# AgRoboticsResearch/headland_trajectory_planning

Measured on NVIDIA B200. Metric: warm_start_plans_per_sec, higher is better.
Workload: dtype f64

## Files before the change

headland_trajectory_planning_b200/_lib.py:

```python
import ctypes as C
import os
import threading

import numpy as np

HERE = os.path.dirname(os.path.abspath(__file__))
_LIB_NAME = "libheadland_b200.so"

ABI_VERSION = 4
HL_MAX_PRIMS = 16
HL_CAPSULE_VERTS = 66
HL_RS_CANDIDATES = 46
HL_RS_MAX_SEGS = 5

CHECK_OBSTACLES = 1
CHECK_BOUNDARY = 2
CHECK_AUX = 4
CHECK_LANE = 8

STATUS_NAMES = {0: "ok", 1: "start_goal_blocked", 2: "open_empty", 3: "max_nodes",
                4: "capacity", 5: "rs_assert"}


class HeadlandError(RuntimeError):
    pass


class HlEnvHost(C.Structure):
    _fields_ = [
        ("n_obs", C.c_int32), ("obs_xy", C.POINTER(C.c_double)),
        ("n_field", C.c_int32), ("field_xy", C.POINTER(C.c_double)),
        ("n_seg", C.c_int32), ("seg_xy", C.POINTER(C.c_double)),
        ("seg_poly", C.POINTER(C.c_double)), ("seg_len", C.POINTER(C.c_double)),
        ("n_crit", C.c_int32), ("crit_xy", C.POINTER(C.c_double)),
        ("n_guide", C.c_int32), ("guide", C.POINTER(C.c_double)),
        ("default_search_length", C.c_double),
        ("body_ext", C.c_double * 4),
        ("n_aux", C.c_int32), ("aux_ext", C.POINTER(C.c_double)),
    ]


class HlSearchParams(C.Structure):
    _fields_ = [
        ("plan_resolution", C.c_double), ("yaw_resolution", C.c_double),
        ("maxc", C.c_double), ("max_steer", C.c_double), ("wheel_base", C.c_double),
        ("n_prims", C.c_int32),
        ("prim_steer", C.c_double * HL_MAX_PRIMS), ("prim_dir", C.c_double * HL_MAX_PRIMS),
        ("prim_yaw_step", C.c_double * HL_MAX_PRIMS), ("prim_curv", C.c_double * HL_MAX_PRIMS),
        ("prim_steer_eff", C.c_double * HL_MAX_PRIMS),
        ("steps_default", C.c_int32), ("steps_large", C.c_int32),
        ("steer_cost", C.c_double), ("delta_steer_cost", C.c_double),
        ("direction_change_cost", C.c_double), ("reverse_cost", C.c_double),
        ("hybrid_cost", C.c_double), ("min_length_to_goal", C.c_double),
        ("max_nodes", C.c_int32), ("max_path_poses", C.c_int32),
        ("motion_type", C.c_int32), ("dubins_capacity", C.c_int32),
    ]


class HlGridField(C.Structure):
    _fields_ = [
        ("occ_offset", C.c_int64), ("out_offset", C.c_int64),
        ("w", C.c_int32), ("h", C.c_int32), ("gi", C.c_int32), ("gj", C.c_int32),
    ]


SCENARIO_DTYPE = np.dtype([("env_id", "<i4"), ("reserved", "<i4"),
                           ("start", "<f8", (3,)), ("goal", "<f8", (3,))])
RESULT_DTYPE = np.dtype([("status", "<i4"), ("counter", "<i4"), ("n_expanded", "<i4"),
                         ("arrival", "<i4"), ("path_len", "<i4"), ("rs_word", "<i4"),
                         ("path_offset", "<i8"), ("goal_cost", "<f8"),
                         ("n_pose_checks", "<i8"), ("n_exact", "<i8"), ("keys_offset", "<i8"),
                         ("cycles", "<i8"), ("n_pose_checks_ref", "<i8")])
RSWORD_DTYPE = np.dtype([("cand", "<i4"), ("n_seg", "<i4"), ("npts", "<i4"), ("collide", "<i4"),
                         ("L", "<f8"), ("cost", "<f8"), ("len", "<f8", (HL_RS_MAX_SEGS,)),
                         ("nlen", "<f8", (HL_RS_MAX_SEGS,))])
assert SCENARIO_DTYPE.itemsize == 56 and RESULT_DTYPE.itemsize == 80 and RSWORD_DTYPE.itemsize == 112

EXPORTS = [
    "hl_last_error", "hl_abi_version", "hl_ctx_create", "hl_ctx_destroy", "hl_ctx_sm_count", "hl_ctx_device",
    "hl_ctx_set_astar_variant", "hl_env_upload", "hl_env_free", "hl_env_count", "hl_env_device", "hl_collision_check", "hl_path_reduce",
    "hl_rs_all_paths", "hl_rs_sample", "hl_hybrid_astar_batch", "hl_hybrid_astar_workspace_bytes", "hl_astar_phase_cycles",
    "hl_distance_field", "hl_distance_field_batch", "hl_grid_pack", "hl_grid_footprint_check", "hl_measure_fp32_peak", "hl_ypark_paths", "hl_arc_paths", "hl_ref_path_count", "hl_ref_path_fill",
    "hl_dubins_count", "hl_dubins_knots", "hl_dubins_fill", "hl_min_boundary_distance", "hl_corridor_hits",
]



class _Missing:
    def __init__(self, name):
        self._name = name
        self.argtypes = None
        self.restype = None

    def __call__(self, *a, **k):
        raise HeadlandError(f"libheadland_b200.so does not export {self._name}: rebuild the library")


class _Tolerant:

    def __init__(self, cdll):
        self._cdll = cdll
        self._missing = {}

    def __getattr__(self, name):
        try:
            return getattr(self._cdll, name)
        except AttributeError:
            return self._missing.setdefault(name, _Missing(name))


_lib = None
_lock = threading.RLock()
_ctxs = {}


def library_path():
    return os.path.join(HERE, _LIB_NAME)


def load_library():
    global _lib
    with _lock:
        if _lib is not None:
            return _lib
        path = library_path()
        if not os.path.exists(path):
            raise HeadlandError(
                f"{path} is missing: build it with `python -c 'import __graft_entry__ as g; g.build()'` "
                "(there is no CPU fallback)")
        lib = _Tolerant(C.CDLL(path))
        vp, i32, i64, u32, dbl = C.c_void_p, C.c_int32, C.c_int64, C.c_uint32, C.c_double
        lib.hl_last_error.restype = C.c_char_p
        lib.hl_abi_version.restype = C.c_int
        lib.hl_ctx_create.argtypes = [C.POINTER(vp), C.c_int]
        lib.hl_ctx_destroy.argtypes = [vp]
        lib.hl_ctx_destroy.restype = None
        lib.hl_ctx_sm_count.argtypes = [vp]
        lib.hl_ctx_device.argtypes = [vp]
        lib.hl_ctx_set_astar_variant.argtypes = [vp, C.c_int]
        lib.hl_env_device.argtypes = [vp]
        lib.hl_env_upload.argtypes = [vp, C.POINTER(HlEnvHost), i32, C.POINTER(vp)]
        lib.hl_env_free.argtypes = [vp]
        lib.hl_env_free.restype = None
        lib.hl_env_count.argtypes = [vp]
        lib.hl_env_count.restype = i32
        lib.hl_collision_check.argtypes = [vp, vp, vp, vp, vp, i64, u32, vp, vp, vp]
        lib.hl_path_reduce.argtypes = [vp, vp, vp, i64, vp, vp]
        lib.hl_rs_all_paths.argtypes = [vp, vp, vp, vp, i64, dbl, dbl, dbl, u32, vp, vp, vp, vp]
        lib.hl_rs_sample.argtypes = [vp, vp, vp, i64, dbl, dbl, vp, vp, vp, vp, vp, vp, vp]
        lib.hl_hybrid_astar_batch.argtypes = [vp, vp, vp, i32, C.POINTER(HlSearchParams), vp, vp, i64, vp,
                                              vp, vp, vp, vp, vp, i64, vp, vp]
        lib.hl_hybrid_astar_workspace_bytes.argtypes = [vp, C.POINTER(HlSearchParams)]
        lib.hl_hybrid_astar_workspace_bytes.restype = i64
        lib.hl_astar_phase_cycles.argtypes = [vp, C.POINTER(C.c_uint64), i32, i32]
        lib.hl_distance_field.argtypes = [vp, vp, i32, i32, i32, i32, i32, vp, C.POINTER(i32), vp]
        lib.hl_distance_field_batch.argtypes = [vp, vp, i64, C.POINTER(HlGridField), i32, i32, vp, i64, C.POINTER(i32), vp]
        lib.hl_grid_pack.argtypes = [vp, vp, i32, i32, vp, vp]
        lib.hl_grid_footprint_check.argtypes = [vp, vp, i32, i32, dbl, vp, i64, C.POINTER(dbl), vp, vp]
        lib.hl_measure_fp32_peak.argtypes = [vp, C.POINTER(dbl)]
        lib.hl_ypark_paths.argtypes = [vp, vp, vp, i64, dbl, vp, vp]
        lib.hl_arc_paths.argtypes = [vp, vp, vp, i64, dbl, vp, vp]
        lib.hl_ref_path_count.argtypes = [vp, vp, vp, vp, vp, i64, dbl, vp, vp, vp]
        lib.hl_ref_path_fill.argtypes = [vp, vp, vp, vp, vp, vp, vp, i64, dbl, dbl, dbl, vp, vp, vp]
        lib.hl_dubins_count.argtypes = [vp, vp, i64, dbl, dbl, dbl, i32, vp, vp, vp, vp]
        lib.hl_dubins_knots.argtypes = [vp, vp, i64, dbl, dbl, dbl, i32, vp, vp, vp, vp, vp, vp]
        lib.hl_min_boundary_distance.argtypes = [vp, vp, vp, vp, vp, i64, i32, vp, vp]
        lib.hl_corridor_hits.argtypes = [vp, vp, vp, vp, vp, i64, dbl, vp, vp]
        lib.hl_dubins_fill.argtypes = [vp, i64, dbl, vp, vp, vp, vp, vp, vp]
        if lib.hl_abi_version() != ABI_VERSION:
            raise HeadlandError("libheadland_b200.so ABI version mismatch")
        _lib = lib
        return lib


def last_error():
    return load_library().hl_last_error().decode("utf-8", "replace")


def check(rc, what):
    if rc != 0:
        raise HeadlandError(f"{what}: {last_error()}")


def have_gpu():
    try:
        import torch
        return torch.cuda.is_available()
    except Exception:
        return False


def get_ctx(device=None):
    import torch
    lib = load_library()
    if not torch.cuda.is_available():
        raise HeadlandError("no CUDA device: headland_trajectory_planning_b200 has no CPU fallback")
    if device is None:
        device = torch.cuda.current_device()
    device = int(device)
    with _lock:
        if device in _ctxs:
            return _ctxs[device]
        h = C.c_void_p()
        rc = lib.hl_ctx_create(C.byref(h), device)
        msg = lib.hl_last_error().decode("utf-8", "replace") if rc != 0 else ""
        if rc == 0:
            _ctxs[device] = h
    if rc != 0:
        raise HeadlandError(f"hl_ctx_create: {msg}")
    return h


ASTAR_VARIANTS = {"spec": 0, "warp": 1, "level": 2}


def apply_astar_variant(ctx):
    v = os.environ.get("HL_ASTAR_VARIANT", "spec")
    check(load_library().hl_ctx_set_astar_variant(ctx, ASTAR_VARIANTS.get(v, 0)), "hl_ctx_set_astar_variant")


def ptr(t):
    if t is None:
        return None
    assert t.is_cuda and t.is_contiguous()
    return C.c_void_p(t.data_ptr())


def stream_ptr():
# ... 7 lines not shown
```

headland_trajectory_planning_b200/csrc/hl_astar.cu:

```cuda
#include <cstdlib>
#include <cstdio>
#include <mutex>
#include "hl_astar_common.cuh"

#ifndef AW_WARPS
#define AW_WARPS 12
#endif
#ifndef AW_MIN_CTAS
#define AW_MIN_CTAS 1
#endif
#ifndef AW_LOCKSTEP
#define AW_LOCKSTEP 1
#endif
#ifndef AW_MAX_PLANS
#define AW_MAX_PLANS 6
#endif

struct AwSmem {
    double start[3], goal[3];
    long long start_key, goal_key;
    int env, scen, state;
    int n_nodes, heap_n, counter, n_closed;
    int status, arrival, rs_word;
    double goal_cost;
// ... 6 lines not shown
            unsigned char rs_valid[HL_RS_CANDIDATES + 2], rs_accept[HL_RS_CANDIDATES + 2];
            RsPlan plans[AW_MAX_PLANS];
            RsPlan plan_tmp;
        };
        struct {
            double tx[HL_MAX_PRIMS][AS_ROLL], ty[HL_MAX_PRIMS][AS_ROLL], pyaw[HL_MAX_PRIMS][AS_ROLL];
            unsigned char pamb[HL_MAX_PRIMS][AS_ROLL];
            double pg[HL_MAX_PRIMS], pprio[HL_MAX_PRIMS];
            long long pkey[HL_MAX_PRIMS];
            int pkey_ok[HL_MAX_PRIMS], pslot[HL_MAX_PRIMS], ppos[HL_MAX_PRIMS], pneed[HL_MAX_PRIMS];
        };
    };
    RsProblem rs_prob;
    int rs_n, rs_pick;
    int dub_rows;
    int phit[HL_MAX_PRIMS];
    unsigned long long n_checks, n_exact, n_ref;
    long long t_last, t_phase[AS_N_PHASES];
    __align__(16) float envf[AS_ENV_FLOATS];
};

static_assert(sizeof(AwSmem) * AW_WARPS <= 227 * 1024, "per-CTA shared memory exceeds 227 KB");
#define TICK(ph) do { if (lane == 0) { long long _n = clock64(); S.t_phase[ph] += _n - S.t_last; S.t_last = _n; } } while (0)

__device__ __forceinline__ void finalize_scenario(AwSmem& S, const AsWs& W, const AsParams& P, const AsOut& O, int lane) {
    const RsPlan* plan = P.pawn ? nullptr : (S.rs_pick >= 0 && S.rs_pick < AW_MAX_PLANS ? &S.plans[S.rs_pick] : &S.plan_tmp);
    const AsWritten w = write_outputs(W, P, O, S.status, S.n_closed, S.cur, S.arrival, S.start_key, S.goal_key, plan,
                                      S.dub_rows, lane);
    if (lane == 0) {
        S.t_phase[PH_OUTPUT] += clock64() - S.t_last;
        long long tot = 0;
        for (int k = 0; k < AS_N_PHASES; ++k) tot += S.t_phase[k];
        write_record(O, S.scen, w, S.arrival, S.rs_word, S.goal_cost, S.counter, S.n_checks, S.n_exact, S.n_ref, tot);
        for (int k = 0; k < AS_N_PHASES; ++k) atomicAdd(O.phase_cycles + k, (unsigned long long)S.t_phase[k]);
    }
    for (int i = lane; i < S.n_nodes; i += 32) W.hkey[W.nhpos[i]] = KEY_EMPTY;
    __syncwarp();
}

__device__ __noinline__ void setup_scenario(AwSmem& S, const AsWs& W, const AsParams& P, const EnvBatchDev& eb,
                                            const EnvDesc& D, const EnvSmem& E, unsigned FLAGS, int lane) {
    const AsStart st = start_node(W, P, eb, D, E, S.start, S.goal, FLAGS, lane);
    if (lane == 0) {
        S.start_key = st.start_key; S.goal_key = st.goal_key; S.status = st.status;
        if (st.status < 0) { S.n_nodes = 1; heap_set(W, S.heap_n, 0, st.prio); }
    }
    __syncwarp();
}

__device__ __noinline__ void pawn_shot(AwSmem& S, const AsWs& W, const AsParams& P, const EnvBatchDev& eb, const EnvDesc& D,
                                       const EnvSmem& E, unsigned FLAGS, int lane) {
    const int cap = P.dub_cap;
    double* ts = W.dub; double* kx = ts + cap; double* ky = kx + cap; double* ks = ky + cap; double* dx = ks + cap;
    double* dy = dx + cap; double* cp = dy + cap; double* bx = cp + cap; double* by = bx + cap;
    double* rx = by + cap; double* ry = rx + cap; double* ryaw = ry + cap; double* rk = ryaw + cap;
    const double q0[3] = {S.cx, S.cy, S.cyaw};
    DubPath path;
    dub_shortest(q0, S.goal, xdiv(1.0, P.maxc), path);
    if (path.type < 0) { if (lane == 0) S.status = HL_STATUS_RS_ASSERT; __syncwarp(); return; }
    const long long n_s = dub_n_samples(dub_length(path), P.res);
    if (n_s + 1 > cap) { if (lane == 0) S.status = HL_STATUS_CAPACITY; __syncwarp(); return; }
    const int m = dub_course_knots(path, P.res, true, S.goal, n_s, ts, kx, ky, ks, lane);
    if (m < 2) { if (lane == 0) S.status = HL_STATUS_RS_ASSERT; __syncwarp(); return; }
    if (lane == 0) rp_derivs(ks, kx, ky, m, dx, dy, cp, bx, by);
    __syncwarp();
    const long long cnt = rp_count(ks[m - 1], P.res);
    if (cnt > cap) { if (lane == 0) S.status = HL_STATUS_CAPACITY; __syncwarp(); return; }
    for (long long i = lane; i < cnt; i += 32) {
        const double t = xmul((double)i, P.res);
        double x, x1, x2, y, y1, y2;
        rp_eval(ks, kx, dx, m, t, x, x1, x2);
        rp_eval(ks, ky, dy, m, t, y, y1, y2);
        const double q = x1 * x1 + y1 * y1;
        rx[i] = x; ry[i] = y; ryaw[i] = angle_wrap(m_atan2(y1, x1));
        rk[i] = (y2 * x1 - x2 * y1) / (q * sqrt(q));
    }
    __syncwarp();
    if (lane == 0) S.n_ref += (unsigned long long)cnt;
    int infeasible = 0;
    for (long long base = 0; base < cnt && !infeasible; base += 32) {
        const long long i = base + lane;
        int st = HL_FREE;
        unsigned amb = 0;
        if (i < cnt) st = pose_filter(D, E, rx[i], ry[i], ryaw[i], FLAGS, &amb);
        const unsigned livem = __ballot_sync(FULL, i < cnt);
        const unsigned hitm = __ballot_sync(FULL, st == HL_HIT);
        const unsigned ambm = __ballot_sync(FULL, st == HL_AMBIG);
        infeasible = hitm != 0;
        if (!infeasible && ambm) {
            int bad = 0;
            if (st == HL_AMBIG) bad = pose_exact(eb, D, rx[i], ry[i], ryaw[i], amb) ? 1 : 0;
            if (lane == 0) S.n_exact += (unsigned long long)__popc(ambm);
            infeasible = __any_sync(FULL, bad);
        }
        if (lane == 0) S.n_checks += (unsigned long long)__popc(livem);
    }
    if (!infeasible && lane == 0) {
        double len = 0.0, kmin = rk[0], kmax = rk[0];
        for (long long i = 0; i + 1 < cnt; ++i) {
            const double dsl = hypot_cr(xsub(rx[i + 1], rx[i]), xsub(ry[i + 1], ry[i]));
            len = (i == 0) ? dsl : xadd(len, dsl);
        }
        for (long long i = 1; i < cnt; ++i) { kmin = fmin(kmin, rk[i]); kmax = fmax(kmax, rk[i]); }
        if (len < P.min_len_goal) {
            S.arrival = 1; S.rs_word = path.type; S.dub_rows = (int)cnt;
            S.goal_cost = xadd(xadd(S.cg, len), xmul(angle_wrap(xsub(kmax, kmin)), P.steer_cost));
        }
    }
    __syncwarp();
}

__global__ void __launch_bounds__(AW_WARPS * 32, AW_MIN_CTAS)
k_hybrid_astar_w(EnvBatchDev eb, const HlScenario* __restrict__ scen, int n_scen, AsParams P, char* ws_base,
                 size_t ws_stride, unsigned int* work_counter, AsOut O) {
    extern __shared__ __align__(16) unsigned char smem_raw[];
    const int lane = threadIdx.x & 31, wid = threadIdx.x >> 5;
    AwSmem& S = reinterpret_cast<AwSmem*>(smem_raw)[wid];
    const AsWs W = as_carve(ws_base + ((size_t)blockIdx.x * AW_WARPS + wid) * ws_stride, P.cap_nodes, P.hash_size,
                            P.max_nodes, P.dub_cap);
    const int hmask = P.hash_size - 1;
    const unsigned FLAGS = HL_CHECK_OBSTACLES | HL_CHECK_BOUNDARY | HL_CHECK_LANE;

    for (int i = lane; i < P.hash_size; i += 32) W.hkey[i] = KEY_EMPTY;
    if (lane == 0) S.state = ST_IDLE;
    __syncwarp();

    EnvSmem E;
    E.n_obs = E.n_field = E.n_seg = E.all_rect = 0; E.eps = 0.f; E.reach = 0.f; E.obs = E.field = E.seg = nullptr;
    const EnvDesc* Dp = eb.desc;
    int iter = 0;
    (void)iter;

    while (true) {
        while (S.state == ST_IDLE) {
            int sc = 0;
            if (lane == 0) sc = (int)atomicAdd(work_counter, 1u);
            sc = __shfl_sync(FULL, sc, 0);
            if (sc >= n_scen) { if (lane == 0) S.state = ST_DONE; __syncwarp(); break; }
            if (lane == 0) {
                const HlScenario s = scen[sc];
                S.scen = sc; S.env = s.env_id;
                for (int k = 0; k < 3; ++k) { S.start[k] = s.start[k]; S.goal[k] = s.goal[k]; }
                S.n_nodes = 0; S.heap_n = 0; S.counter = 0; S.n_closed = 0;
                S.status = -1; S.arrival = 0; S.rs_word = -1; S.goal_cost = 0.0; S.rs_pick = -1;
                S.n_checks = 0; S.n_exact = 0; S.n_ref = 0;
                for (int k = 0; k < AS_N_PHASES; ++k) S.t_phase[k] = 0;
                S.t_last = clock64();
            }
            __syncwarp();
            Dp = eb.desc + S.env;
            stage_env_warp(eb, *Dp, S.envf, AS_ENV_FLOATS, E, lane);
            setup_scenario(S, W, P, eb, *Dp, E, FLAGS, lane);
            TICK(PH_SETUP);
            if (S.status >= 0) finalize_scenario(S, W, P, O, lane);
            else if (lane == 0) S.state = ST_SEARCH;
            __syncwarp();
        }
#if AW_LOCKSTEP == 3
        {
            if ((iter++ & 1) == 0) { if (__syncthreads_and(S.state == ST_DONE)) break; }
            else if (S.state == ST_DONE) {  }
        }
#elif AW_LOCKSTEP
        if (__syncthreads_and(S.state == ST_DONE)) break;
#else
        if (S.state == ST_DONE) break;
#endif
// ... 20 lines not shown
            __syncwarp();
            TICK(PH_POP);
        }
        if (live && S.status < 0 && P.pawn) {
            pawn_shot(S, W, P, eb, D, E, FLAGS, lane);
            TICK(PH_RS_SAMPLE);
        }
        if (live && S.status < 0 && !P.pawn) {
            const double q0[3] = {S.cx, S.cy, S.cyaw};
            for (int c = lane; c < HL_RS_CANDIDATES; c += 32) {
                double l[HL_RS_MAX_SEGS] = {0, 0, 0, 0, 0};
                bool ok = rs_candidate(c, S.rs_prob, l);
                S.rs_valid[c] = ok ? 1 : 0;
                for (int k = 0; k < HL_RS_MAX_SEGS; ++k) S.rs_lens[c][k] = l[k];
            }
            __syncwarp();
            TICK(PH_RS_CAND);
            if (lane < RS_N_GROUPS) rs_select_group(lane, S.rs_valid, S.rs_lens, S.rs_accept, S.rs_Lc);
            __syncwarp();
            {
                const int a0 = S.rs_accept[lane];
                const int a1 = (lane + 32 < HL_RS_CANDIDATES) ? S.rs_accept[lane + 32] : 0;
                const unsigned b0 = __ballot_sync(FULL, a0 == 1), b1 = __ballot_sync(FULL, a1 == 1);
                const unsigned bad = __ballot_sync(FULL, a0 == 2 || a1 == 2);
                const unsigned lt = (1u << lane) - 1u;
                const int n0 = __popc(b0);
                if (a0 == 1) { int k = __popc(b0 & lt); S.rs_acc[k] = lane; S.rs_L[k] = S.rs_Lc[lane]; }
                if (a1 == 1) { int k = n0 + __popc(b1 & lt); S.rs_acc[k] = lane + 32; S.rs_L[k] = S.rs_Lc[lane + 32]; }
                const int m = bad ? 0 : n0 + __popc(b1);
                __syncwarp();
                for (int k = lane; k < m; k += 32)
                    S.rs_prio[k] = rs_path_cost(S.cg, S.rs_acc[k], S.rs_lens[S.rs_acc[k]], P.max_steer,
                                                P.reverse_cost, P.dir_change_cost, P.steer_cost);
                __syncwarp();
                if (lane == 0) {
                    if (bad) S.status = HL_STATUS_RS_ASSERT;
                    S.rs_n = m;
                    if (m > 0) heapdict_order(S.rs_prio, m, S.rs_order);
                }
            }
            __syncwarp();
            TICK(PH_RS_SELECT);
        }
        if (live && S.status < 0) {
            const double q0[3] = {S.cx, S.cy, S.cyaw};
            const int m = P.pawn ? 0 : S.rs_n;
            const double stepn = xmul(P.res, P.maxc);
            const double cq = m_cos(-q0[2]), sq = m_sin(-q0[2]);
            if (lane < m && lane < AW_MAX_PLANS) {
                int c = S.rs_acc[S.rs_order[lane]];
                rs_make_plan(c, S.rs_lens[c], P.maxc, stepn, S.plans[lane]);
                rs_plan_world32(S.plans[lane], q0, cq, sq, D.origin);
            }
            __syncwarp();
            TICK(PH_RS_PLAN);
            EnvSmem Ers = E;
            Ers.eps = E.eps + 6e-5f;
            const float inv_maxc = (float)(1.0 / P.maxc);
            for (int r = 0; r < m; ++r) {
                const int k = S.rs_order[r];
                const int c = S.rs_acc[k];
                if (r >= AW_MAX_PLANS) {
                    __syncwarp();
                    if (lane == 0) {
                        rs_make_plan(c, S.rs_lens[c], P.maxc, stepn, S.plan_tmp);
                        rs_plan_world32(S.plan_tmp, q0, cq, sq, D.origin);
                    }
                    __syncwarp();
                }
                const RsPlan& plan = (r < AW_MAX_PLANS) ? S.plans[r] : S.plan_tmp;
                const int npts = plan.npts;
                if (lane == 0) S.n_ref += (unsigned long long)npts;
                int infeasible = 0;
                const int passes = (npts + 31) >> 5;
                for (int pass = 0; pass < passes && !infeasible; ++pass) {
                    const int j = lane * passes + pass;
                    int st = HL_FREE;
                    unsigned amb = 0;
                    if (j < npts) {
                        float fx, fy, fc, fs;
                        rs_sample_world32(plan, j, inv_maxc, fx, fy, fc, fs);
                        if (fabsf(fx) > Ers.reach || fabsf(fy) > Ers.reach) st = far_status(FLAGS, Ers.n_seg);
                        else if (!(fx == fx) || !(fy == fy) || !(fc == fc)) { st = HL_AMBIG; amb = FLAGS; }
                        else st = filter_part(Ers, fx, fy, fc, fs, Ers.ext, FLAGS, &amb);
                    }
                    const unsigned livem = __ballot_sync(FULL, j < npts);
                    const unsigned hitm = __ballot_sync(FULL, st == HL_HIT);
                    const unsigned ambm = __ballot_sync(FULL, st == HL_AMBIG);
                    infeasible = hitm != 0;
                    if (!infeasible && ambm) {
                        int bad = 0;
                        if (st == HL_AMBIG) {
                            double lx, ly, lyaw, wx, wy, wyaw;
                            int cs, dir;
                            rs_sample_local(plan, j, P.maxc, lx, ly, lyaw, cs, dir);
                            rs_to_world(q0, cq, sq, lx, ly, lyaw, wx, wy, wyaw);
                            bad = pose_exact(eb, D, wx, wy, wyaw, amb) ? 1 : 0;
                        }
                        if (lane == 0) S.n_exact += (unsigned long long)__popc(ambm);
                        infeasible = __any_sync(FULL, bad);
                    }
                    if (lane == 0) S.n_checks += (unsigned long long)__popc(livem);
                }
                const bool short_enough = xdiv(S.rs_L[k], P.maxc) < P.min_len_goal;
                if (!infeasible && short_enough) {
                    if (lane == 0) { S.rs_pick = r; S.arrival = 1; S.rs_word = c; S.goal_cost = S.rs_prio[k]; }
                    break;
                }
            }
            __syncwarp();
            TICK(PH_RS_SAMPLE);
            if (lane == 0) {
                double xd = fabs(xsub(S.cx, S.goal[0])), yd = fabs(xsub(S.cy, S.goal[1]));
                double wd = fabs(angle_wrap(xsub(S.cyaw, S.goal[2])));
                if (xd < P.res && yd < P.res && wd < P.yaw_res) { S.arrival = 2; S.goal_cost = S.cg; S.rs_word = -1; }
                if (S.arrival) S.status = HL_STATUS_OK;
                else {
                    int seg = exact_search_segment(eb, D, S.cx, S.cy);
                    double len = seg < 0 ? D.default_len : eb.seg_len[D.seg_off + seg];
                    S.nsteps = (int)rint(xdiv(len, P.res));
                    if (S.nsteps + 1 > HL_MAX_ROLLOUT || S.nsteps < 1) S.status = HL_STATUS_CAPACITY;
                }
            }
            if (lane < HL_MAX_PRIMS) S.phit[lane] = 0;
            __syncwarp();
            TICK(PH_ARRIVE);
        }
#if AW_LOCKSTEP == 1
        __syncthreads();
#endif
        if (live && S.status < 0) {
            const int n = S.nsteps, np1 = n + 1;
            const int total = P.n_prims * np1;
            for (int idx = lane; idx < total; idx += 32) {
                const int p = idx / np1, i = idx - p * np1;
                const double ys = P.yaw_step[p];
                const double init_yaw = angle_wrap(xadd(S.cyaw, ys));
                const double stop = xadd(init_yaw, xmul(ys, (double)(n + 1)));
                const double delta = xsub(stop, init_yaw);
                const double step = xdiv(delta, (double)(n + 1));
                const double yw = rollout_yaw(init_yaw, stop, step, delta, n + 1, i);
                S.tx[p][i] = xmul(xmul(P.res, m_cos(yw)), P.dir[p]);
                S.ty[p][i] = xmul(xmul(P.res, m_sin(yw)), P.dir[p]);
                S.pyaw[p][i] = rollout_yaw(init_yaw, stop, step, delta, n + 1, i + 1);
            }
            __syncwarp();
            if (lane < P.n_prims) {
                double ax = 0.0, ay = 0.0;
                for (int i = 0; i < np1; ++i) {
                    ax = (i == 0) ? S.tx[lane][0] : xadd(ax, S.tx[lane][i]);
                    ay = (i == 0) ? S.ty[lane][0] : xadd(ay, S.ty[lane][i]);
                    S.tx[lane][i] = xadd(S.cx, ax);
                    S.ty[lane][i] = xadd(S.cy, ay);
                }
            }
            __syncwarp();
            TICK(PH_ROLLOUT);
            for (int idx = lane; idx < total; idx += 32) {
                const int p = idx / np1, j = idx - p * np1;
                unsigned amb = 0;
                int st = pose_filter(D, E, S.tx[p][j], S.ty[p][j], S.pyaw[p][j], FLAGS, &amb);
                S.pamb[p][j] = (st == HL_AMBIG) ? (unsigned char)amb : 0;
                if (st == HL_HIT) atomicOr(&S.phit[p], 1);
            }
            if (lane == 0) { S.n_checks += (unsigned long long)total; S.n_ref += (unsigned long long)total; }
            __syncwarp();
            TICK(PH_FILTER);
            for (int idx = lane; idx < total; idx += 32) {
                const int p = idx / np1, j = idx - p * np1;
                if (S.pamb[p][j] && !S.phit[p]) {
                    atomicAdd(&S.n_exact, 1ULL);
                    if (pose_exact(eb, D, S.tx[p][j], S.ty[p][j], S.pyaw[p][j], S.pamb[p][j])) atomicOr(&S.phit[p], 2);
                }
            }
            __syncwarp();
            TICK(PH_EXACT);
            if (lane < HL_MAX_PRIMS) S.pneed[lane] = 1;
            __syncwarp();
            if (lane < P.n_prims && !S.phit[lane]) {
                const int p = lane;
                double len = 0.0;
                for (int i = 0; i + 1 < np1; ++i) {
                    double ds = hypot_cr(xsub(S.tx[p][i + 1], S.tx[p][i]), xsub(S.ty[p][i + 1], S.ty[p][i]));
                    len = (i == 0) ? ds : xadd(len, ds);
                }
                double cost = xadd(S.cg, len);
                if (P.dir[p] == -1.0) cost = xadd(cost, P.reverse_cost);
                cost = xadd(cost, xmul(P.steer[p], P.steer_cost));
                const double parent_steer = S.cprim < 0 ? 0.0 : P.steer_eff[S.cprim];
                cost = xadd(cost, xmul(fabs(xsub(P.steer[p], parent_steer)), P.delta_steer_cost));
                const double parent_dir = S.cprim < 0 ? 1.0 : P.dir[S.cprim];
                if (parent_dir != P.dir[p]) cost = xadd(cost, P.dir_change_cost);
                S.pg[p] = cost;
                int ix, iy, iw;
                long long key = 0;
                S.pkey_ok[p] = make_key(S.tx[p][n], S.ty[p][n], S.pyaw[p][n], P.res, P.yaw_res, ix, iy, iw, key) ? 1 : 0;
                S.pkey[p] = key;
                int pos = -1;
                const int slot = S.pkey_ok[p] ? hash_find(W, hmask, key, &pos) : -1;
                S.pslot[p] = slot;
                S.ppos[p] = pos;
                if (slot >= 0 && (W.nstate[slot] == 1 || !(cost < W.ng[slot]))) S.pneed[p] = 0;
            }
            __syncwarp();
            for (int p = 0; p < P.n_prims; ++p) {
                if (!S.phit[p] && S.pneed[p]) {
                    double h = warp_state_cost(eb, D, S.tx[p][n], S.ty[p][n], S.pyaw[p][n], lane);
                    if (lane == 0) S.pprio[p] = xmul(P.hybrid_cost, h);
                }
            }
            __syncwarp();
            TICK(PH_COST_HEUR);
            if (lane == 0) {
                for (int p = 0; p < P.n_prims; ++p) {
                    if (S.phit[p]) continue;
                    if (!S.pkey_ok[p]) { S.status = HL_STATUS_CAPACITY; break; }
                    int pos = S.ppos[p];
                    int slot = S.pslot[p];
                    if (slot < 0 ? (W.hkey[pos] != KEY_EMPTY) : false) slot = hash_find(W, hmask, S.pkey[p], &pos);
                    const double g = S.pg[p];
                    const double prio = (S.pprio[p] > g) ? S.pprio[p] : g;
                    if (slot >= 0) {
                        if (W.nstate[slot] == 1) continue;
                        if (!(g < W.ng[slot])) continue;
                        if (!S.pneed[p]) { S.status = HL_STATUS_CAPACITY; break; }
                    } else {
                        if (S.n_nodes >= P.cap_nodes) { S.status = HL_STATUS_CAPACITY; break; }
                        slot = S.n_nodes++;
                        W.hkey[pos] = S.pkey[p]; W.hval[pos] = slot; W.nhpos[slot] = pos;
                        W.nkey[slot] = S.pkey[p]; W.nstate[slot] = 0; W.nheap[slot] = -1;
                    }
                    W.nx[slot] = S.tx[p][n]; W.ny[slot] = S.ty[p][n]; W.nyaw[slot] = S.pyaw[p][n];
                    W.ng[slot] = g; W.nparent[slot] = S.cur; W.nprim[slot] = (signed char)p;
                    W.nsteps[slot] = (signed char)n;
                    heap_set(W, S.heap_n, slot, prio);
                }
            }
            __syncwarp();
            TICK(PH_MERGE);
        }
        if (live && S.status >= 0) {
            finalize_scenario(S, W, P, O, lane);
            if (lane == 0) S.state = ST_IDLE;
            __syncwarp();
// ... 313 lines not shown
```

headland_trajectory_planning_b200/csrc/hl_astar_common.cuh:

```cuda
#define HL_SHARED_CODE 1
#pragma once
#include <cstring>
#include "hl_geom.cuh"
#include "hl_rs.cuh"
#include "hl_dubins.cuh"

#define AS_ROLL (HL_MAX_ROLLOUT + 1)
#define AS_ENV_FLOATS 512
#define KEY_EMPTY (-1LL)
#define FULL 0xffffffffu
enum { ST_IDLE = 0, ST_SEARCH = 1, ST_DONE = 2 };
enum { PH_POP = 0, PH_RS_CAND, PH_RS_SELECT, PH_RS_PLAN, PH_RS_SAMPLE, PH_ARRIVE, PH_ROLLOUT, PH_FILTER, PH_EXACT,
       PH_COST_HEUR, PH_MERGE, PH_SETUP, PH_OUTPUT, AS_N_PHASES };

struct AsParams {
    double res, yaw_res, maxc, max_steer, wheel_base;
    int n_prims;
    double steer[HL_MAX_PRIMS], dir[HL_MAX_PRIMS], yaw_step[HL_MAX_PRIMS], curv[HL_MAX_PRIMS], steer_eff[HL_MAX_PRIMS];
    double steer_cost, delta_steer_cost, dir_change_cost, reverse_cost, hybrid_cost, min_len_goal;
    int max_nodes, max_path_poses;
    int cap_nodes, hash_size;
    int pawn;
    int dub_cap;
};
// ... 75 lines not shown
}

__device__ __forceinline__ unsigned hash_key(long long k) {
    unsigned long long z = (unsigned long long)k * 0x9E3779B97F4A7C15ULL;
    return (unsigned)(z >> 40);
}

__device__ __noinline__ int hash_find(const AsWs& w, int hmask, long long key, int* pos) {
    unsigned h = hash_key(key) & hmask;
    while (true) {
        long long k = w.hkey[h];
        if (k == key) { *pos = (int)h; return w.hval[h]; }
        if (k == KEY_EMPTY) { *pos = (int)h; return -1; }
        h = (h + 1) & hmask;
    }
}

template <int HS> struct HeapRef {
    const AsWs& w; double* sp; int* ss;
    __device__ __forceinline__ double prio(int i) const { return (HS > 0 && i < HS) ? sp[i] : w.hprio[i]; }
    __device__ __forceinline__ int slot(int i) const { return (HS > 0 && i < HS) ? ss[i] : w.hslot[i]; }
    __device__ __forceinline__ void put(int i, double p, int s) const {
        if (HS > 0 && i < HS) { sp[i] = p; ss[i] = s; } else { w.hprio[i] = p; w.hslot[i] = s; }
        w.nheap[s] = i;
    }
};

template <int HS> __device__ __forceinline__ void heap_up_t(const HeapRef<HS>& H, int i, double prio, int slot, bool always) {
    while (i) {
        const int parent = (i - 1) >> 1;
        const double pp = H.prio(parent);
        if (!always && pp < prio) break;
        H.put(i, pp, H.slot(parent));
        i = parent;
    }
    H.put(i, prio, slot);
}

template <int HS> __device__ __forceinline__ int heap_popitem_t(const HeapRef<HS>& H, int& n) {
    const int top = H.slot(0);
    --n;
    if (n > 0) {
        const double prio = H.prio(n);
        const int slot = H.slot(n);
        int i = 0;
        while (true) {
            const int l = (i << 1) + 1, r = l + 1;
            int low = i;
            double lowp = prio;
            if (l < n) {
                const double pl = H.prio(l);
                const double pr = (r < n) ? H.prio(r) : 0.0;
                if (pl < lowp) { low = l; lowp = pl; }
                if (r < n && pr < lowp) { low = r; lowp = pr; }
            }
            if (low == i) break;
            H.put(i, lowp, H.slot(low));
            i = low;
        }
        H.put(i, prio, slot);
    }
    H.w.nheap[top] = -1;
    return top;
}

template <int HS> __device__ __forceinline__ void heap_set_t(const HeapRef<HS>& H, int& n, int slot, double prio) {
    const int at = H.w.nheap[slot];
    if (at >= 0) {
        heap_up_t<HS>(H, at, 0.0, slot, true);
        heap_popitem_t<HS>(H, n);
    }
    heap_up_t<HS>(H, n++, prio, slot, false);
}

__device__ __noinline__ int heap_popitem(const AsWs& w, int& n) {
    const HeapRef<0> H{w, nullptr, nullptr};
    return heap_popitem_t<0>(H, n);
}
__device__ __noinline__ void heap_set(const AsWs& w, int& n, int slot, double prio) {
    const HeapRef<0> H{w, nullptr, nullptr};
    heap_set_t<0>(H, n, slot, prio);
}

__device__ HL_CODE int pose_filter(const EnvDesc& D, const EnvSmem& E, double x, double y, double yaw,
                                           unsigned flags, unsigned* amb) {
    float px = (float)(x - D.origin[0]), py = (float)(y - D.origin[1]);
    if (fabsf(px) > E.reach || fabsf(py) > E.reach) return far_status(flags, E.n_seg);
    if (!(fabs(yaw) < 1e6) || !(px == px) || !(py == py)) { *amb = flags; return HL_AMBIG; }
    float sf, cf;
    sincosf((float)yaw, &sf, &cf);
    return filter_part(E, px, py, cf, sf, E.ext, flags, amb);
}

__device__ __noinline__ bool pose_exact(const EnvBatchDev& eb, const EnvDesc& D, double x, double y, double yaw,
                                           unsigned amb) {
    Pose64 p;
    p.x = x; p.y = y; p.c = m_cos(yaw); p.s = m_sin(yaw);
    return exact_part_check(p, D.body_ext, eb, D, amb);
}

__device__ __noinline__ void stage_env_warp(const EnvBatchDev& eb, const EnvDesc& D, float* sm, int cap_floats,
                                            EnvSmem& E, int lane) {
    const int n_o = D.n_obs * HL_OBS32_STRIDE, n_f = D.n_field * HL_FIELD32_STRIDE, n_s = D.n_seg * 4;
    E.n_obs = D.n_obs; E.n_field = D.n_field; E.n_seg = D.n_seg; E.all_rect = D.all_rect;
    E.eps = D.eps; E.reach = D.reach;
    for (int k = 0; k < 4; ++k) E.ext[k] = (float)D.body_ext[k];
    const float* g_obs = eb.obs32 + (size_t)HL_OBS32_STRIDE * D.obs_off;
    const float* g_field = eb.field32 + HL_FIELD32_STRIDE * (size_t)D.field_off;
    const float* g_seg = eb.seg32 + 4 * (size_t)D.seg_off;
    if (n_o + n_f + n_s <= cap_floats) {
        float* s_obs = sm;
        float* s_field = s_obs + n_o;
        float* s_seg = s_field + n_f;
        for (int i = lane; i < n_o; i += 32) s_obs[i] = g_obs[i];
        for (int i = lane; i < n_f; i += 32) s_field[i] = g_field[i];
        for (int i = lane; i < n_s; i += 32) s_seg[i] = g_seg[i];
        E.obs = s_obs; E.field = s_field; E.seg = s_seg;
    } else {
        E.obs = g_obs; E.field = g_field; E.seg = g_seg;
    }
    __syncwarp();
}

__device__ __noinline__ double warp_state_cost(const EnvBatchDev& eb, const EnvDesc& D, double x, double y, double yaw, int lane) {
    const double* gx = eb.guide_x + D.guide_off;
    const double* gy = eb.guide_y + D.guide_off;
    const int n = D.n_guide;
    if (n <= 0) return 0.0;
    double best = INFINITY;
#pragma unroll 1
    for (int i = lane; i < n; i += 32) {
        double dx = gx[i] - x, dy = gy[i] - y;
        best = fmin(best, dx * dx + dy * dy);
    }
    for (int o = 16; o; o >>= 1) best = fmin(best, __shfl_xor_sync(0xffffffffu, best, o));
    const double thr = best * (1.0 + 1e-9) + 1e-300;
    double bh = INFINITY;
    int bi = 0x7fffffff;
#pragma unroll 1
    for (int i = lane; i < n; i += 32) {
        double dx = xsub(gx[i], x), dy = xsub(gy[i], y);
        if (dx * dx + dy * dy <= thr) {
            double h = hypot_cr(dx, dy);
            if (h < bh || (h == bh && i < bi)) { bh = h; bi = i; }
        }
    }
    for (int o = 16; o; o >>= 1) {
        double oh = __shfl_xor_sync(0xffffffffu, bh, o);
        int oi = __shfl_xor_sync(0xffffffffu, bi, o);
        if (oh < bh || (oh == bh && oi < bi)) { bh = oh; bi = oi; }
    }
    double dist = xmul(bh, 100.0);
    double yaw_diff = fabs(angle_wrap(xsub(eb.guide_yaw[D.guide_off + bi], yaw)));
    if (dist > 2.0) dist = 100.0;
    double to_goal = xsub(eb.guide_s[D.guide_off + n - 1], eb.guide_s[D.guide_off + bi]);
    return xadd(xadd(dist, xmul(yaw_diff, 0.2)), xmul(to_goal, 5.0));
}

__device__ HL_TINY double rollout_yaw(double init_yaw, double stop, double step, double delta, int div, int i) {
    double v;
    if (i == div) v = stop;
    else if (step != 0.0) v = xadd(xmul((double)i, step), init_yaw);
    else v = xadd(xmul(xdiv((double)i, (double)div), delta), init_yaw);
    return angle_wrap(v);
}



struct AsStart { int status; long long start_key, goal_key; double prio; };

__device__ __forceinline__ AsStart start_node(const AsWs& W, const AsParams& P, const EnvBatchDev& eb, const EnvDesc& D,
                                           const EnvSmem& E, const double* start, const double* goal, unsigned flags,
                                           int lane) {
    int bad = 0;
    if (lane < 2) {
        const double* q = lane == 0 ? start : goal;
        unsigned amb = flags;
        int r = pose_filter(D, E, q[0], q[1], q[2], flags, &amb);
        bad = (r == HL_HIT) || (r == HL_AMBIG && pose_exact(eb, D, q[0], q[1], q[2], amb));
    }
    bad = __any_sync(FULL, bad);
    const double h = warp_state_cost(eb, D, start[0], start[1], start[2], lane);
    AsStart s;
    s.status = -1; s.start_key = 0; s.goal_key = 0; s.prio = 0.0;
    if (lane == 0) {
        int ix, iy, iw;
        bool ok = make_key(start[0], start[1], start[2], P.res, P.yaw_res, ix, iy, iw, s.start_key);
        ok = make_key(goal[0], goal[1], goal[2], P.res, P.yaw_res, ix, iy, iw, s.goal_key) && ok;
        if (!ok) s.status = HL_STATUS_CAPACITY;
        else if (bad) s.status = HL_STATUS_START_GOAL_BLOCKED;
        else {
            W.nx[0] = start[0]; W.ny[0] = start[1]; W.nyaw[0] = start[2]; W.ng[0] = 0.0;
            W.nkey[0] = s.start_key; W.nparent[0] = 0; W.nprim[0] = -1; W.nsteps[0] = 0; W.nstate[0] = 0;
            W.nheap[0] = -1;
            int pos;
            hash_find(W, P.hash_size - 1, s.start_key, &pos);
            W.hkey[pos] = s.start_key; W.hval[pos] = 0; W.nhpos[0] = pos;
            s.prio = xmul(P.hybrid_cost, h);
            s.prio = (s.prio > 0.0) ? s.prio : 0.0;
        }
    }
    return s;
}

struct AsWritten { int status, n_keys; long long keys_off; int path_len; long long path_off; };

__device__ __noinline__ AsWritten write_outputs(const AsWs& W, const AsParams& P, const AsOut& O, int status, int n_closed,
                                                int end, int arrival, long long start_key, long long goal_key,
                                                const RsPlan* plan, int dub_rows, int lane) {
    AsWritten w;
    long long koff = 0;
    if (lane == 0 && n_closed > 0) {
        koff = (long long)atomicAdd(O.keys_cursor, (unsigned long long)n_closed);
        if (koff + n_closed > O.keys_capacity) koff = -1;
    }
    koff = __shfl_sync(FULL, koff, 0);
    w.n_keys = n_closed;
    if (koff < 0) { status = HL_STATUS_CAPACITY; w.n_keys = 0; koff = 0; }
    w.keys_off = koff;
    int32_t* ek = O.expanded_keys + (size_t)koff * 3;
    for (int i = lane; i < w.n_keys; i += 32) {
        int ix, iy, iw;
        unpack_key(W.nkey[W.corder[i]], ix, iy, iw);
        ek[3 * i] = ix; ek[3 * i + 1] = iy; ek[3 * i + 2] = iw;
    }
    const int ext_rows = arrival != 1 ? 0 : (plan ? plan->npts : dub_rows);
    int len = 0, path_len = 0;
    long long path_off = 0;
    if (lane == 0 && status == HL_STATUS_OK) {
        int poses = 0;
        bool ok = true;
        if (goal_key != start_key) {
            for (int node = end; node != 0; node = W.nparent[node]) {
                if (len >= P.cap_nodes) { ok = false; break; }
                W.hslot[len++] = node;
                poses += W.nsteps[node] + 1;
            }
            poses += ext_rows;
        }
        path_len = poses;
        if (!ok || path_len > P.max_path_poses) { status = HL_STATUS_CAPACITY; path_len = 0; }
        else if (path_len > 0) {
            unsigned long long off = atomicAdd(O.path_cursor, (unsigned long long)path_len);
            if ((long long)(off + path_len) > O.path_capacity) { status = HL_STATUS_CAPACITY; path_len = 0; }
            path_off = (long long)off;
        }
    }
    __syncwarp();
    w.status = __shfl_sync(FULL, status, 0);
    w.path_len = __shfl_sync(FULL, path_len, 0);
    w.path_off = __shfl_sync(FULL, path_off, 0);
    len = __shfl_sync(FULL, len, 0);
    if (w.status == HL_STATUS_OK && w.path_len > 0) {
        for (int c = lane; c < len; c += 32) {
            const int node = W.hslot[len - 1 - c];
            long long off = w.path_off;
            for (int q = 0; q < c; ++q) off += W.nsteps[W.hslot[len - 1 - q]] + 1;
            const int par = W.nparent[node];
            const int p = W.nprim[node], n = W.nsteps[node];
            const double ys = P.yaw_step[p];
            const double init_yaw = angle_wrap(xadd(W.nyaw[par], ys));
// ... 64 lines not shown
```

headland_trajectory_planning_b200/csrc/hl_astar_level.cuh:

```cuda
#pragma once
#include "hl_astar_common.cuh"

#define LS_ROLL_STRIDE (AS_ROLL + 1)
#define LS_MAX_BATCH 8192
#define LS_CHUNK 32
#define LS_GRID_MULT 4
#define LS_THREADS 256

struct LsScn {
    double start[3], goal[3];
    long long start_key, goal_key;
    int env, status, arrival, has_cur;
    int n_nodes, heap_n, counter, n_closed;
    int cur, cprim, nsteps, rs_n;
    double cx, cy, cyaw, cg;
    double goal_cost;
    int rs_pick, rs_word, rs_bad, pad0;
    RsProblem rs_prob;
    unsigned long long checks, exact, ref;
};

struct LsPrim {
    double dtx[AS_ROLL], dty[AS_ROLL];
    double tx[AS_ROLL], ty[AS_ROLL], pyaw[AS_ROLL];
// ... 202 lines not shown
    const int n_act = C.n_act[parity];
    const int* act = C.act[parity];
    for (int a = warp; a < n_act; a += n_warps) {
        const int sc = act[a];
        LsScn& S = C.scn[sc];
        LsShot& T = C.shot[sc];
        if (lane < RS_N_GROUPS) rs_select_group(lane, T.rs_valid, T.rs_lens, T.rs_accept, T.rs_Lc);
        __syncwarp();
        const int a0 = T.rs_accept[lane];
        const int a1 = (lane + 32 < HL_RS_CANDIDATES) ? T.rs_accept[lane + 32] : 0;
        const unsigned b0 = __ballot_sync(FULL, a0 == 1), b1 = __ballot_sync(FULL, a1 == 1);
        const unsigned bad = __ballot_sync(FULL, a0 == 2 || a1 == 2);
        const unsigned lt = (1u << lane) - 1u;
        const int n0 = __popc(b0);
        if (a0 == 1) { int k = __popc(b0 & lt); T.rs_acc[k] = lane; T.rs_L[k] = T.rs_Lc[lane]; }
        if (a1 == 1) { int k = n0 + __popc(b1 & lt); T.rs_acc[k] = lane + 32; T.rs_L[k] = T.rs_Lc[lane + 32]; }
        const int m = bad ? 0 : n0 + __popc(b1);
        __syncwarp();
        const double sg = S.cg;
        for (int k = lane; k < m; k += 32)
            T.rs_prio[k] = rs_path_cost(sg, T.rs_acc[k], T.rs_lens[T.rs_acc[k]], P.max_steer, P.reverse_cost,
                                        P.dir_change_cost, P.steer_cost);
        __syncwarp();
        int base = 0;
        if (lane == 0) {
            S.rs_n = m; S.rs_bad = bad ? 1 : 0;
            if (m > 0) {
                double prio[HL_RS_CANDIDATES];
                int order[HL_RS_CANDIDATES];
                for (int k = 0; k < m; ++k) prio[k] = T.rs_prio[k];
                heapdict_order(prio, m, order);
                for (int k = 0; k < m; ++k) T.rs_order[k] = order[k];
                base = atomicAdd(C.n_words, m);
            }
        }
        base = __shfl_sync(FULL, base, 0);
        for (int r = lane; r < m; r += 32) { C.words[base + r] = make_int2(sc, r); T.word_bad[r] = 1; }
        __syncwarp();
    }
}

__global__ void __launch_bounds__(LS_THREADS) ls_sample(const LsCall* __restrict__ Cp) {
    __shared__ RsPlan s_plan[LS_THREADS / 32];
    const LsCall& C = *Cp;
    const int lane = threadIdx.x & 31, wib = threadIdx.x >> 5;
    const int warp = (blockIdx.x * blockDim.x + threadIdx.x) >> 5, n_warps = (gridDim.x * blockDim.x) >> 5;
    const AsParams& P = C.P;
    const int n_words = *C.n_words;
    const float inv_maxc = (float)(1.0 / P.maxc);
    const double stepn = xmul(P.res, P.maxc);
    RsPlan& plan = s_plan[wib];
    for (int w = warp; w < n_words; w += n_warps) {
        const int2 item = C.words[w];
        const int sc = item.x, r = item.y;
        LsScn& S = C.scn[sc];
        LsShot& T = C.shot[sc];
        const EnvDesc& D = C.eb.desc[S.env];
        EnvSmem E;
        global_env(C.eb, D, E);
        E.eps += 6e-5f;
        const int k = T.rs_order[r];
        const int c = T.rs_acc[k];
        const double q0[3] = {S.cx, S.cy, S.cyaw};
        const double cq = m_cos(-q0[2]), sq = m_sin(-q0[2]);
        __syncwarp();
        if (lane == 0) {
            rs_make_plan(c, T.rs_lens[c], P.maxc, stepn, plan);
            rs_plan_world32(plan, q0, cq, sq, D.origin);
        }
        __syncwarp();
        const int npts = plan.npts;
        int infeasible = 0;
        const int passes = (npts + 31) >> 5;
        unsigned long long checks = 0, exact = 0;
        for (int pass = 0; pass < passes && !infeasible; ++pass) {
            const int j = lane * passes + pass;
            int st2 = HL_FREE;
            unsigned amb = 0;
            if (j < npts) {
                float fx, fy, fc, fs;
                rs_sample_world32(plan, j, inv_maxc, fx, fy, fc, fs);
                if (fabsf(fx) > E.reach || fabsf(fy) > E.reach) st2 = far_status(LS_FLAGS, E.n_seg);
                else if (!(fx == fx) || !(fy == fy) || !(fc == fc)) { st2 = HL_AMBIG; amb = LS_FLAGS; }
                else st2 = filter_part(E, fx, fy, fc, fs, E.ext, LS_FLAGS, &amb);
            }
            const unsigned livem = __ballot_sync(FULL, j < npts);
            const unsigned hitm = __ballot_sync(FULL, st2 == HL_HIT);
            const unsigned ambm = __ballot_sync(FULL, st2 == HL_AMBIG);
            infeasible = hitm != 0;
            if (!infeasible && ambm) {
                int bad2 = 0;
                if (st2 == HL_AMBIG) {
                    double lx, ly, lyaw, wx, wy, wyaw;
                    int cs, dir;
                    rs_sample_local(plan, j, P.maxc, lx, ly, lyaw, cs, dir);
                    rs_to_world(q0, cq, sq, lx, ly, lyaw, wx, wy, wyaw);
                    bad2 = pose_exact(C.eb, D, wx, wy, wyaw, amb) ? 1 : 0;
                }
                exact += (unsigned long long)__popc(ambm);
                infeasible = __any_sync(FULL, bad2);
            }
            checks += (unsigned long long)__popc(livem);
        }
        if (lane == 0) {
            T.word_npts[r] = npts;
            T.word_bad[r] = infeasible ? 1 : 0;
            atomicAdd(&S.checks, checks);
            if (exact) atomicAdd(&S.exact, exact);
        }
        __syncwarp();
    }
}

__global__ void __launch_bounds__(LS_THREADS) ls_rollout(const LsCall* __restrict__ Cp, int parity) {
    const LsCall& C = *Cp;
    const AsParams& P = C.P;
    const int per_scn = P.n_prims * LS_ROLL_STRIDE;
    const int n_items = C.n_act[parity] * per_scn;
    const int* act = C.act[parity];
    if (blockIdx.x == 0 && threadIdx.x == 0) C.n_act[parity ^ 1] = 0;
    for (int it = blockIdx.x * blockDim.x + threadIdx.x; it < n_items; it += gridDim.x * blockDim.x) {
        const int a = it / per_scn, rem = it - a * per_scn;
        const int p = rem / LS_ROLL_STRIDE, i = rem - p * LS_ROLL_STRIDE;
        const int sc = act[a];
        const LsScn& S = C.scn[sc];
        const int n = S.nsteps, np1 = n + 1;
        if (i > np1) continue;
        LsPrim& R = C.prim[(size_t)sc * P.n_prims + p];
        const double ys = P.yaw_step[p];
        const double init_yaw = angle_wrap(xadd(S.cyaw, ys));
        const double stop = xadd(init_yaw, xmul(ys, (double)(n + 1)));
        const double delta = xsub(stop, init_yaw);
        const double step = xdiv(delta, (double)(n + 1));
        const double yw = rollout_yaw(init_yaw, stop, step, delta, n + 1, i);
        if (i >= 1) R.pyaw[i - 1] = yw;
        if (i <= n) {
            double sn, cs;
            m_sincos(yw, &sn, &cs);
            R.dtx[i] = xmul(xmul(P.res, cs), P.dir[p]);
            R.dty[i] = xmul(xmul(P.res, sn), P.dir[p]);
        }
        if (i == 0) { R.phit = 0; R.pneed = 1; }
    }
}

__global__ void __launch_bounds__(LS_THREADS) ls_filter(const LsCall* __restrict__ Cp, int parity) {
    const LsCall& C = *Cp;
    const AsParams& P = C.P;
    const int per_scn = P.n_prims * AS_ROLL;
    const int n_items = C.n_act[parity] * per_scn;
    const int* act = C.act[parity];
    for (int it = blockIdx.x * blockDim.x + threadIdx.x; it < n_items; it += gridDim.x * blockDim.x) {
        const int a = it / per_scn, rem = it - a * per_scn;
        const int p = rem / AS_ROLL, j = rem - p * AS_ROLL;
        const int sc = act[a];
        LsScn& S = C.scn[sc];
        const int np1 = S.nsteps + 1;
        if (j >= np1) continue;
        LsPrim& R = C.prim[(size_t)sc * P.n_prims + p];
        double ax = R.dtx[0], ay = R.dty[0];
        for (int i = 1; i <= j; ++i) { ax = xadd(ax, R.dtx[i]); ay = xadd(ay, R.dty[i]); }
        const double x = xadd(S.cx, ax), y = xadd(S.cy, ay);
        R.tx[j] = x; R.ty[j] = y;
        const EnvDesc& D = C.eb.desc[S.env];
        EnvSmem E;
        global_env(C.eb, D, E);
        unsigned amb = 0;
        const int st = pose_filter(D, E, x, y, R.pyaw[j], LS_FLAGS, &amb);
        R.pamb[j] = (st == HL_AMBIG) ? (unsigned char)amb : 0;
        if (st == HL_HIT) atomicOr(&R.phit, 1);
        if (j == 0 && p == 0) atomicAdd(&S.checks, (unsigned long long)(P.n_prims * np1));
    }
}

__global__ void __launch_bounds__(LS_THREADS) ls_cost(const LsCall* __restrict__ Cp, int parity) {
    const LsCall& C = *Cp;
    const int lane = threadIdx.x & 31;
    const int warp = (blockIdx.x * blockDim.x + threadIdx.x) >> 5, n_warps = (gridDim.x * blockDim.x) >> 5;
    const AsParams& P = C.P;
    const int hmask = P.hash_size - 1;
    const int n_items = C.n_act[parity] * P.n_prims;
    const int* act = C.act[parity];
    for (int it = warp; it < n_items; it += n_warps) {
        const int a = it / P.n_prims, p = it - a * P.n_prims;
        const int sc = act[a];
        LsScn& S = C.scn[sc];
        LsPrim& R = C.prim[(size_t)sc * P.n_prims + p];
        const EnvDesc& D = C.eb.desc[S.env];
        const int n = S.nsteps, np1 = n + 1;
        int hit = R.phit;
        if (!hit) {
            int bad = 0;
            const int am = lane < np1 ? R.pamb[lane] : 0;
            if (am) bad = pose_exact(C.eb, D, R.tx[lane], R.ty[lane], R.pyaw[lane], am) ? 1 : 0;
            const unsigned ambm = __ballot_sync(FULL, am != 0);
            if (ambm && lane == 0) atomicAdd(&S.exact, (unsigned long long)__popc(ambm));
            if (__any_sync(FULL, bad)) hit = 2;
        }
        if (hit) { if (lane == 0) R.phit = hit; __syncwarp(); continue; }
        double ds = 0.0;
        if (lane < n) ds = hypot_cr(xsub(R.tx[lane + 1], R.tx[lane]), xsub(R.ty[lane + 1], R.ty[lane]));
        double len = __shfl_sync(FULL, ds, 0);
        for (int i = 1; i < n; ++i) len = xadd(len, __shfl_sync(FULL, ds, i));
        if (n < 1) len = 0.0;
        int need = 1, key_ok = 0;
        if (lane == 0) {
            const AsWs W = ls_ws(C, sc);
            double cost = xadd(S.cg, len);
            if (P.dir[p] == -1.0) cost = xadd(cost, P.reverse_cost);
            cost = xadd(cost, xmul(P.steer[p], P.steer_cost));
            const int cprim = S.cprim;
            const double parent_steer = cprim < 0 ? 0.0 : P.steer_eff[cprim];
            cost = xadd(cost, xmul(fabs(xsub(P.steer[p], parent_steer)), P.delta_steer_cost));
            const double parent_dir = cprim < 0 ? 1.0 : P.dir[cprim];
            if (parent_dir != P.dir[p]) cost = xadd(cost, P.dir_change_cost);
            R.pg = cost;
            int ix, iy, iw;
            long long key = 0;
            key_ok = make_key(R.tx[n], R.ty[n], R.pyaw[n], P.res, P.yaw_res, ix, iy, iw, key) ? 1 : 0;
            R.pkey_ok = key_ok;
            R.pkey = key;
            int pos = -1;
            const int slot2 = key_ok ? hash_find(W, hmask, key, &pos) : -1;
            R.pslot = slot2;
            R.ppos = pos;
            if (slot2 >= 0 && (W.nstate[slot2] == 1 || !(cost < W.ng[slot2]))) need = 0;
            R.pneed = need;
            R.phit = 0;
        }
        need = __shfl_sync(FULL, need, 0);
        key_ok = __shfl_sync(FULL, key_ok, 0);
        if (need && key_ok) {
            const double h = warp_state_cost(C.eb, D, R.tx[n], R.ty[n], R.pyaw[n], lane);
            if (lane == 0) R.pprio = xmul(P.hybrid_cost, h);
        }
        __syncwarp();
    }
}

__global__ void __launch_bounds__(LS_THREADS) ls_finalize(const LsCall* __restrict__ Cp) {
    __shared__ RsPlan s_plan[LS_THREADS / 32];
    const LsCall& C = *Cp;
    const int lane = threadIdx.x & 31, wib = threadIdx.x >> 5;
    const int warp = (blockIdx.x * blockDim.x + threadIdx.x) >> 5, n_warps = (gridDim.x * blockDim.x) >> 5;
    const AsParams& P = C.P;
    RsPlan& plan = s_plan[wib];
    for (int sc = warp; sc < C.n_scen; sc += n_warps) {
        const LsScn& S = C.scn[sc];
        const AsWs W = ls_ws(C, sc);
        const int status = S.status < 0 ? HL_STATUS_CAPACITY : S.status;
        if (lane == 0 && S.arrival == 1)
// ... 11 lines not shown
```

headland_trajectory_planning_b200/csrc/hl_astar_spec.cuh:

```cuda
#pragma once
#include "hl_astar_common.cuh"

#ifndef AQ_EXPANDERS
#define AQ_EXPANDERS 2
#endif
#ifndef AQ_SLOTS
#define AQ_SLOTS (AQ_EXPANDERS > 1 ? 5 : 6)
#endif
#define AQ_MAX_PLANS 6
#ifndef AQ_SHOOTERS
#define AQ_SHOOTERS 1
#endif
#define AQ_WARPS_PER_SLOT (AQ_EXPANDERS + AQ_SHOOTERS)
#ifndef AQ_HEAP_SM
#define AQ_HEAP_SM 1023
#endif
#ifndef AQ_GUIDE_CAP
#define AQ_GUIDE_CAP 192
#endif
#ifndef AQ_GD_UNROLL
#define AQ_GD_UNROLL 4
#endif
#define AQ_PRAGMA_(x) _Pragma(#x)
#define AQ_PRAGMA_UNROLL(n) AQ_PRAGMA_(unroll n)
// ... 139 lines not shown
    const HeapRef<AQ_HEAP_SM> H{w, S.hp_prio, S.hp_slot};
#else
    const HeapRef<0> H{w, nullptr, nullptr};
#endif
    const int i = S.heap_n;
    const int depth = 31 - __clz(i + 1);
    const bool mine = lane >= 1 && lane <= depth;
    const int a = ((i + 1) >> lane) - 1;
    double ap = 0.0;
    int as = 0;
    if (mine) { ap = H.prio(a); as = H.slot(a); }
    const unsigned stopm = __ballot_sync(FULL, mine && ap < prio);
    const int stop = stopm ? (__ffs(stopm) - 1) : depth + 1;
    __syncwarp();
    if (mine && lane < stop) H.put(((i + 1) >> (lane - 1)) - 1, ap, as);
    if (lane == 0) { H.put(((i + 1) >> (stop - 1)) - 1, prio, slot); S.heap_n = i + 1; }
    __syncwarp();
}

__device__ __noinline__ void team_state_costs(AqSmem& S, const EnvBatchDev& eb, const EnvDesc& D, const AsParams& P,
                                              int nst, int tl, int lane) {
    const unsigned needm = __ballot_sync(FULL, lane < P.n_prims && !S.phit[lane] && S.pneed[lane]);
    const int slot = tl / AQ_SUB, sub = tl - slot * AQ_SUB;
    const int p = slot < __popc(needm) ? (int)__fns(needm, 0, slot + 1) : -1;
    const int n = D.n_guide;
    const double* gx = S.gx;
    const double* gy = S.gy;
    const double x = p >= 0 ? S.tx[p][nst] : 0.0, y = p >= 0 ? S.ty[p][nst] : 0.0;
    double best = INFINITY;
AQ_PRAGMA_UNROLL(AQ_GD_UNROLL)
    for (int i = sub; i < n; i += AQ_SUB) {
        const double dx = gx[i] - x, dy = gy[i] - y;
        const double d2 = dx * dx + dy * dy;
        best = d2 < best ? d2 : best;
    }
#pragma unroll
    for (int o = AQ_SUB / 2; o; o >>= 1) best = fmin(best, __shfl_xor_sync(FULL, best, o));
    const double thr = best * (1.0 + 1e-9) + 1e-300;
    double bh = INFINITY;
    int bi = 0x7fffffff;
#pragma unroll 1
    for (int i = sub; i < n; i += AQ_SUB) {
        const double dx = xsub(gx[i], x), dy = xsub(gy[i], y);
        if (dx * dx + dy * dy <= thr) {
            const double h = hypot_cr(dx, dy);
            if (h < bh || (h == bh && i < bi)) { bh = h; bi = i; }
        }
    }
#pragma unroll
    for (int o = AQ_SUB / 2; o; o >>= 1) {
        const double oh = __shfl_xor_sync(FULL, bh, o);
        const int oi = __shfl_xor_sync(FULL, bi, o);
        if (oh < bh || (oh == bh && oi < bi)) { bh = oh; bi = oi; }
    }
    if (p >= 0 && sub == 0) {
        double h = 0.0;
        if (n > 0) {
            double dist = xmul(bh, 100.0);
            const double yaw_diff = fabs(angle_wrap(xsub(S.gyaw[bi], S.pyaw[p][nst])));
            if (dist > 2.0) dist = 100.0;
            const double to_goal = xsub(S.gs[n - 1], S.gs[bi]);
            h = xadd(xadd(dist, xmul(yaw_diff, 0.2)), xmul(to_goal, 5.0));
        }
        S.pprio[p] = xmul(P.hybrid_cost, h);
    }
}

__device__ __noinline__ bool aq_word_collides(const EnvSmem& Ers, const EnvBatchDev& eb, const EnvDesc& D, const RsPlan& plan,
                                              const double* q0, double cq, double sq, double maxc, float inv_maxc,
                                              unsigned FLAGS, AqShot& T, int lane) {
    const int npts = plan.npts;
    int infeasible = 0;
    const int passes = (npts + 31) >> 5;
#pragma unroll 1
    for (int pass = 0; pass < passes && !infeasible; ++pass) {
        const int j = lane * passes + pass;
        int st2 = HL_FREE;
        unsigned amb = 0;
        if (j < npts) {
            float fx, fy, fc, fs;
            rs_sample_world32(plan, j, inv_maxc, fx, fy, fc, fs);
            if (fabsf(fx) > Ers.reach || fabsf(fy) > Ers.reach) st2 = far_status(FLAGS, Ers.n_seg);
            else if (!(fx == fx) || !(fy == fy) || !(fc == fc)) { st2 = HL_AMBIG; amb = FLAGS; }
            else st2 = filter_part(Ers, fx, fy, fc, fs, Ers.ext, FLAGS, &amb);
        }
        const unsigned livem = __ballot_sync(FULL, j < npts);
        const unsigned hitm = __ballot_sync(FULL, st2 == HL_HIT);
        const unsigned ambm = __ballot_sync(FULL, st2 == HL_AMBIG);
        infeasible = hitm != 0;
        if (!infeasible && ambm) {
            int bad2 = 0;
            if (st2 == HL_AMBIG) {
                double lx, ly, lyaw, wx, wy, wyaw;
                int cs, dir;
                rs_sample_local(plan, j, maxc, lx, ly, lyaw, cs, dir);
                rs_to_world(q0, cq, sq, lx, ly, lyaw, wx, wy, wyaw);
                bad2 = pose_exact(eb, D, wx, wy, wyaw, amb) ? 1 : 0;
            }
            if (lane == 0) T.s_exact += (unsigned long long)__popc(ambm);
            infeasible = __any_sync(FULL, bad2);
        }
        if (lane == 0) T.s_checks += (unsigned long long)__popc(livem);
    }
    return infeasible != 0;
}

__device__ __forceinline__ void finalize_spec(AqSmem& S, const AsWs& W, const AsParams& P, const AsOut& O, int lane) {
    const int n_closed = S.fin_closed;
    const int end = (n_closed > 0) ? W.corder[n_closed - 1] : 0;
    const AqShot& T = S.sh[S.win];
    const AsWritten w = write_outputs(W, P, O, S.status, n_closed, end, S.arrival, S.start_key, S.goal_key, &T.plan_tmp,
                                      0, lane);
    if (lane == 0) {
        unsigned long long checks = S.e_checks, exact = S.e_exact, ref = 0;
        for (int k = 0; k < AQ_SHOOTERS; ++k) { checks += S.sh[k].s_checks; exact += S.sh[k].s_exact; ref += S.sh[k].s_ref; }
        const bool shot_won = (S.arrival == 1) || (w.status == HL_STATUS_RS_ASSERT);
        ref += (shot_won && n_closed > 0) ? (unsigned long long)W.cref[n_closed - 1] : S.e_ref;
        write_record(O, S.scen, w, S.arrival, T.rs_word, S.goal_cost, S.fin_counter, checks, exact, ref, clock64() - S.t0);
        for (int k = 0; k < AS_N_PHASES; ++k) {
            const long long v = S.te[k] + S.ts[k];
            if (v) atomicAdd(O.phase_cycles + k, (unsigned long long)v);
        }
    }
    for (int i = lane; i < S.n_nodes; i += 32) W.hkey[W.nhpos[i]] = KEY_EMPTY;
    __syncwarp();
}

__global__ void __launch_bounds__(AQ_SLOTS * AQ_WARPS_PER_SLOT * 32, 1)
k_hybrid_astar_s(EnvBatchDev eb, const HlScenario* __restrict__ scen, int n_scen, AsParams P, char* ws_base,
                 size_t ws_stride, unsigned int* work_counter, AsOut O) {
    extern __shared__ __align__(16) unsigned char smem_raw[];
    const int lane = threadIdx.x & 31, wid = threadIdx.x >> 5;
#if AQ_WARP_MAP == 1 && AQ_SLOTS == 5 && AQ_WARPS_PER_SLOT == 3
    const int slot = (wid & 3) == 3 ? 4 : wid >> 2;
    const int wrole = (wid & 3) == 3 ? (wid == 3 ? 2 : (wid == 7 ? 0 : 1)) : ((wid & 3) == 0 ? 2 : (wid & 3) - 1);
#else
    const int slot = wid / AQ_WARPS_PER_SLOT;
    const int wrole = wid % AQ_WARPS_PER_SLOT;
#endif
    const int ew = wrole;
    const int role = wrole < AQ_EXPANDERS ? 0 : wrole - AQ_EXPANDERS + 1;
    const int tl = ew * 32 + lane;
    AqSmem& S = reinterpret_cast<AqSmem*>(smem_raw)[slot];
    const AsWs W = as_carve(ws_base + ((size_t)blockIdx.x * AQ_SLOTS + slot) * ws_stride, P.cap_nodes, P.hash_size,
                            P.max_nodes);
    const int hmask = P.hash_size - 1;
    const unsigned FLAGS = HL_CHECK_OBSTACLES | HL_CHECK_BOUNDARY | HL_CHECK_LANE;
    if (role == 0 && ew == 0) {
#pragma unroll 1
        for (int i = lane; i < P.hash_size; i += 32) W.hkey[i] = KEY_EMPTY;
        if (lane == 0) {
            S.x_expanding = 0; S.x_finished = 0; S.need_seg = 0;
            S.state = ST_IDLE; S.epoch = 0; S.popped = 0; S.ew_done = 0; S.shot_best = AQ_NO_HIT;
            for (int k = 0; k < AQ_SHOOTERS; ++k) S.sh[k].done_epoch = 0;
        }
    }
    __syncthreads();

    EnvSmem E;
    E.n_obs = E.n_field = E.n_seg = E.all_rect = 0; E.eps = 0.f; E.reach = 0.f; E.obs = E.field = E.seg = nullptr;

    if (role >= 1) {
        const int shooter = role - 1;
        AqShot& T = S.sh[shooter];
        int my_epoch = 0;
        int i = 0;
        bool active = false;
// ... 55 lines not shown
                    break;
                }
                if (!have) { __nanosleep(100); break; }
                __threadfence_block();
                if (lane == 0) {
                    const int cur = W.corder[i];
                    T.s_cur = cur; T.sx = W.nx[cur]; T.sy = W.ny[cur]; T.syaw = W.nyaw[cur]; T.sg = W.ng[cur];
                }
                __syncwarp();
                q0[0] = T.sx; q0[1] = T.sy; q0[2] = T.syaw;
                {
                    const double phi = xsub(S.goal[2], q0[2]);
                    double sn, cs;
                    m_sincos(lane == 1 ? phi : q0[2], &sn, &cs);
                    const double c0 = __shfl_sync(FULL, cs, 0), s0 = __shfl_sync(FULL, sn, 0);
                    const double cp = __shfl_sync(FULL, cs, 1), sp = __shfl_sync(FULL, sn, 1);
                    cq = c0; sq = -s0;
                    if (lane == 0) {
                        RsProblem Pr;
                        const double dx = xsub(S.goal[0], q0[0]), dy = xsub(S.goal[1], q0[1]);
                        Pr.phi = phi;
                        Pr.x = xmul(xadd(xmul(c0, dx), xmul(s0, dy)), P.maxc);
                        Pr.y = xmul(xadd(xmul(-s0, dx), xmul(c0, dy)), P.maxc);
                        Pr.sp = sp; Pr.cp = cp;
                        Pr.xb = xadd(xmul(Pr.x, cp), xmul(Pr.y, sp));
                        Pr.yb = xsub(xmul(Pr.x, sp), xmul(Pr.y, cp));
                        T.rs_prob = Pr;
                    }
                    __syncwarp();
                }
                rs_candidates_warp(T.rs_prob, T.rs_valid, T.rs_lens, lane);
                STICK(PH_RS_CAND);
                if (lane < RS_N_GROUPS) rs_select_group(lane, T.rs_valid, T.rs_lens, T.rs_accept, T.rs_Lc);
                __syncwarp();
                {
                    const int a0 = T.rs_accept[lane];
                    const int a1 = (lane + 32 < HL_RS_CANDIDATES) ? T.rs_accept[lane + 32] : 0;
                    const unsigned b0 = __ballot_sync(FULL, a0 == 1), b1 = __ballot_sync(FULL, a1 == 1);
                    const unsigned bad = __ballot_sync(FULL, a0 == 2 || a1 == 2);
                    const unsigned lt = (1u << lane) - 1u;
                    const int n0 = __popc(b0);
                    if (a0 == 1) { int k = __popc(b0 & lt); T.rs_acc[k] = lane; T.rs_L[k] = T.rs_Lc[lane]; }
                    if (a1 == 1) { int k = n0 + __popc(b1 & lt); T.rs_acc[k] = lane + 32; T.rs_L[k] = T.rs_Lc[lane + 32]; }
                    m = bad ? 0 : n0 + __popc(b1);
                    __syncwarp();
                    if (lane == 0) { if (bad) T.rs_assert = 1; T.rs_n = m; }
                    __syncwarp();
                    if (bad) success = true;
                }
                STICK(PH_RS_SELECT);
                shooting = true;
            }
            } while (0);
#if AQ_MID >= 1
            role_sync(1, AQ_SLOTS * AQ_SHOOTERS * 32);
            if (shooting) STICK(PH_OUTPUT);
#endif
            if (!shooting) continue;
            const EnvDesc& D = *Dp;
            {
                int first_free = -1;
                unsigned long long ref_all = 0;
#pragma unroll 1
                for (int k0 = 0; k0 < m && first_free < 0; k0 += AQ_MAX_PLANS) {
                    const int nw = (m - k0) < AQ_MAX_PLANS ? (m - k0) : AQ_MAX_PLANS;
                    rs_make_plans_warp(T.rs_acc, T.rs_lens, T.rs_npts, k0, nw, T.plans, q0, cq, sq, D.origin, P.maxc, stepn, lane);
                    STICK(PH_RS_PLAN);
                    unsigned dead = 0;
#if AQ_COARSE
                    if (nw >= 2) {
                        const int per = 32 / nw;
                        const int r = lane / per, q = lane - r * per;
                        int st2 = HL_FREE;
                        if (r < nw) {
                            const RsPlan& plan = T.plans[r];
                            const int npts = plan.npts;
                            const int j = (int)(((long long)(2 * q + 1) * npts) / (2 * per));
                            if (j < npts) {
                                float fx, fy, fc, fs;
                                unsigned amb = 0;
                                rs_sample_world32(plan, j, inv_maxc, fx, fy, fc, fs);
                                if (fabsf(fx) > Ers.reach || fabsf(fy) > Ers.reach) st2 = far_status(FLAGS, Ers.n_seg);
                                else if (!(fx == fx) || !(fy == fy) || !(fc == fc)) st2 = HL_AMBIG;
                                else st2 = filter_part(Ers, fx, fy, fc, fs, Ers.ext, FLAGS, &amb);
                            }
                        }
                        const unsigned hitm = __ballot_sync(FULL, st2 == HL_HIT);
                        const unsigned livem = __ballot_sync(FULL, r < nw);
                        for (int w = 0; w < nw; ++w)
                            if (hitm & (((per >= 32) ? 0xffffffffu : ((1u << per) - 1u)) << (w * per))) dead |= 1u << w;
                        if (lane == 0) T.s_checks += (unsigned long long)__popc(livem);
                    }
#endif
#pragma unroll 1
                    for (int w = 0; w < nw; ++w) {
                        const RsPlan& plan = T.plans[w];
                        ref_all += (unsigned long long)plan.npts;
                        if (dead & (1u << w)) continue;
                        const bool hit = aq_word_collides(Ers, eb, D, plan, q0, cq, sq, P.maxc, inv_maxc, FLAGS, T, lane);
                        if (!hit && xdiv(T.rs_L[k0 + w], P.maxc) < P.min_len_goal) { first_free = k0 + w; break; }
                    }
                    STICK(PH_RS_SAMPLE);
                }
                if (first_free < 0) {
                    if (lane == 0) T.s_ref += ref_all;
                } else {
                    __syncwarp();
#pragma unroll 1
                    for (int k = lane; k < m; k += 32)
                        T.rs_prio[k] = rs_path_cost(T.sg, T.rs_acc[k], T.rs_lens[T.rs_acc[k]], P.max_steer,
                                                    P.reverse_cost, P.dir_change_cost, P.steer_cost);
                    __syncwarp();
                    if (lane == 0) heapdict_order(T.rs_prio, m, T.rs_order);
                    __syncwarp();
                    unsigned long long tally = 0;
                    int winner = -1;
#pragma unroll 1
                    for (int r = 0; r < m && winner < 0; ++r) {
                        const int k = T.rs_order[r];
                        if (k < first_free) { tally += (unsigned long long)T.rs_npts[k]; continue; }
                        if (k == first_free) { tally += (unsigned long long)T.rs_npts[k]; winner = k; break; }
                        rs_make_plans_warp(T.rs_acc, T.rs_lens, T.rs_npts, k, 1, &T.plan_tmp, q0, cq, sq, D.origin, P.maxc, stepn, lane);
                        const RsPlan& plan = T.plan_tmp;
                        tally += (unsigned long long)plan.npts;
                        const bool hit = aq_word_collides(Ers, eb, D, plan, q0, cq, sq, P.maxc, inv_maxc, FLAGS, T, lane);
                        if (!hit && xdiv(T.rs_L[k], P.maxc) < P.min_len_goal) winner = k;
                    }
                    __syncwarp();
                    rs_make_plans_warp(T.rs_acc, T.rs_lens, T.rs_npts, winner, 1, &T.plan_tmp, q0, cq, sq, D.origin, P.maxc, stepn, lane);
                    if (lane == 0) {
                        T.s_ref += tally;
                        T.rs_word = T.rs_acc[winner]; T.rs_goal_cost = T.rs_prio[winner];
                    }
                    success = true;
                }
                __syncwarp();
                STICK(PH_RS_SAMPLE);
            }
            if (success) {
                if (lane == 0) { __threadfence_block(); atomicMin(&S.shot_best, i); __threadfence_block(); T.done_epoch = my_epoch; }
                __syncwarp();
                active = false;
            } else i += AQ_SHOOTERS;
        }
        return;
    }

    int mode = 0;
    bool finished = false;
    int my_epoch = 0;
    const EnvDesc* Dp = eb.desc;
    unsigned e_iter = 0;
    int helper_epoch = 0;
    while (true) {
        if ((e_iter++ % AQ_EVERY_E) == 0 && role_barrier_all(2, AQ_SLOTS * AQ_TEAM, finished)) break;
        bool expanding = false;
        if (ew == 0) {
        do {
        if (finished) break;
        ETICK(PH_SETUP);
        if (mode == 0) {
        int sc = 0;
        if (lane == 0) {
            sc = (int)atomicAdd(work_counter, 1u);
            const int n_eff = O.order_count ? *O.order_count : n_scen;
            sc = sc < n_eff ? (O.order ? O.order[sc] : sc) : -1;
        }
// ... 81 lines not shown
                if (lane == 0) {
                    const int seg = inm ? 31 - __clz(inm) : -1;
                    const double len = seg < 0 ? D.default_len : eb.seg_len[D.seg_off + seg];
                    S.nsteps = (int)rint(xdiv(len, P.res));
                    if (S.nsteps + 1 > HL_MAX_ROLLOUT || S.nsteps < 1) S.ew_status = HL_STATUS_CAPACITY;
                    S.need_seg = 0;
                }
            }
            if (lane < HL_MAX_PRIMS) { S.phit[lane] = 0; S.pneed[lane] = 1; }
            __syncwarp();
            if (O.first_only && S.ew_status < 0) {
                if (lane == 0) S.ew_status = AQ_STATUS_DEFER;
                __syncwarp();
            }
            ETICK(PH_POP);
            if (S.ew_status >= 0) mode = 2; else expanding = true;
        }
        } while (0);
        }
#if AQ_EXPANDERS > 1
        if (ew == 0 && lane == 0) { S.x_expanding = expanding ? 1 : 0; S.x_finished = finished ? 1 : 0; }
        team_sync(slot);
        if (ew != 0) {
            expanding = S.x_expanding != 0; finished = S.x_finished != 0;
            const int ep = S.epoch;
            if (expanding && ep != helper_epoch) {
                helper_epoch = ep;
                Dp = eb.desc + S.env;
                const EnvDesc& D0 = *Dp;
                const int n_o = D0.n_obs * HL_OBS32_STRIDE, n_f = D0.n_field * HL_FIELD32_STRIDE, n_s = D0.n_seg * 4;
                E.n_obs = D0.n_obs; E.n_field = D0.n_field; E.n_seg = D0.n_seg; E.all_rect = D0.all_rect;
                E.eps = D0.eps; E.reach = D0.reach;
                for (int k = 0; k < 4; ++k) E.ext[k] = (float)D0.body_ext[k];
                if (n_o + n_f + n_s <= AS_ENV_FLOATS) { E.obs = S.envf; E.field = S.envf + n_o; E.seg = S.envf + n_o + n_f; }
                else {
                    E.obs = eb.obs32 + (size_t)HL_OBS32_STRIDE * D0.obs_off;
                    E.field = eb.field32 + HL_FIELD32_STRIDE * (size_t)D0.field_off;
                    E.seg = eb.seg32 + 4 * (size_t)D0.seg_off;
                }
            }
        }
#endif
        const EnvDesc& D = *Dp;
        if (expanding) {
            {
            const int n = S.nsteps, np1 = n + 1;
            const int total = P.n_prims * np1;
#pragma unroll 1
            for (int idx = tl; idx < P.n_prims * (np1 + 1); idx += AQ_TEAM) {
                const int p = idx / (np1 + 1), i = idx - p * (np1 + 1);
                const double ys = P.yaw_step[p];
                const double init_yaw = angle_wrap(xadd(S.cyaw, ys));
                const double stop = xadd(init_yaw, xmul(ys, (double)(n + 1)));
                const double delta = xsub(stop, init_yaw);
                const double step = xdiv(delta, (double)(n + 1));
                const double yw = rollout_yaw(init_yaw, stop, step, delta, n + 1, i);
                if (i >= 1) S.pyaw[p][i - 1] = yw;
                if (i <= n) {
                    double sn, cs;
                    m_sincos(yw, &sn, &cs);
                    S.tx[p][i] = xmul(xmul(P.res, cs), P.dir[p]);
                    S.ty[p][i] = xmul(xmul(P.res, sn), P.dir[p]);
                }
            }
            team_sync(slot);
            if (tl < P.n_prims) {
                double ax = 0.0, ay = 0.0;
#pragma unroll 1
                for (int i = 0; i < np1; ++i) {
                    ax = (i == 0) ? S.tx[lane][0] : xadd(ax, S.tx[lane][i]);
                    ay = (i == 0) ? S.ty[lane][0] : xadd(ay, S.ty[lane][i]);
                    S.tx[lane][i] = xadd(S.cx, ax);
                    S.ty[lane][i] = xadd(S.cy, ay);
                }
            }
            team_sync(slot);
            if (ew == 0) ETICK(PH_ROLLOUT);
            {
                const int far_cnt = np1 < AQ_FAR ? np1 : AQ_FAR;
#pragma unroll 1
                for (int idx = tl; idx < P.n_prims * far_cnt; idx += AQ_TEAM) {
                    const int p = idx / far_cnt, j = n - (idx - p * far_cnt);
                    unsigned amb = 0;
                    int st = pose_filter(D, E, S.tx[p][j], S.ty[p][j], S.pyaw[p][j], FLAGS, &amb);
                    S.pamb[p][j] = (st == HL_AMBIG) ? (unsigned char)amb : 0;
                    if (st == HL_HIT) atomicOr(&S.phit[p], 1);
                }
                team_sync(slot);
                const unsigned live = __ballot_sync(FULL, lane < P.n_prims && S.phit[lane] == 0);
                const int rem = np1 - far_cnt;
                const int total2 = __popc(live) * rem;
#pragma unroll 1
                for (int idx = tl; idx < total2; idx += AQ_TEAM) {
                    const int q = idx / rem, j = idx - q * rem;
                    const int p = __fns(live, 0, q + 1);
                    unsigned amb = 0;
                    int st = pose_filter(D, E, S.tx[p][j], S.ty[p][j], S.pyaw[p][j], FLAGS, &amb);
                    S.pamb[p][j] = (st == HL_AMBIG) ? (unsigned char)amb : 0;
                    if (st == HL_HIT) atomicOr(&S.phit[p], 1);
                }
                if (tl == 0) { S.e_checks += (unsigned long long)(P.n_prims * far_cnt + total2); S.e_ref += (unsigned long long)total; }
            }
            team_sync(slot);
            if (ew == 0) ETICK(PH_FILTER);
#pragma unroll 1
            for (int idx = tl; idx < total; idx += AQ_TEAM) {
                const int p = idx / np1, j = idx - p * np1;
                if (S.pamb[p][j] && !S.phit[p]) {
                    atomicAdd(&S.e_exact, 1ULL);
                    if (pose_exact(eb, D, S.tx[p][j], S.ty[p][j], S.pyaw[p][j], S.pamb[p][j])) atomicOr(&S.phit[p], 2);
                }
            }
            team_sync(slot);
            if (ew == 0) ETICK(PH_EXACT);
            }
        }
        if (expanding) {
            {
            const int n = S.nsteps, np1 = n + 1;
#pragma unroll 1
            for (int idx = tl; idx < P.n_prims * n; idx += AQ_TEAM) {
                const int p = idx / n, i = idx - p * n;
                if (!S.phit[p]) S.pds[p][i] = hypot_cr(xsub(S.tx[p][i + 1], S.tx[p][i]), xsub(S.ty[p][i + 1], S.ty[p][i]));
            }
            team_sync(slot);
            if (tl < P.n_prims && !S.phit[lane]) {
                const int p = lane;
                double len = 0.0;
#pragma unroll 1
                for (int i = 0; i + 1 < np1; ++i) len = (i == 0) ? S.pds[p][0] : xadd(len, S.pds[p][i]);
                double cost = xadd(S.cg, len);
                if (P.dir[p] == -1.0) cost = xadd(cost, P.reverse_cost);
                cost = xadd(cost, xmul(P.steer[p], P.steer_cost));
                const double parent_steer = S.cprim < 0 ? 0.0 : P.steer_eff[S.cprim];
                cost = xadd(cost, xmul(fabs(xsub(P.steer[p], parent_steer)), P.delta_steer_cost));
                const double parent_dir = S.cprim < 0 ? 1.0 : P.dir[S.cprim];
                if (parent_dir != P.dir[p]) cost = xadd(cost, P.dir_change_cost);
                S.pg[p] = cost;
                int ix, iy, iw;
                long long key = 0;
                S.pkey_ok[p] = make_key(S.tx[p][n], S.ty[p][n], S.pyaw[p][n], P.res, P.yaw_res, ix, iy, iw, key) ? 1 : 0;
                S.pkey[p] = key;
                int pos = -1;
                const int slot2 = S.pkey_ok[p] ? hash_find(W, hmask, key, &pos) : -1;
                S.pslot[p] = slot2;
                S.ppos[p] = pos;
                if (slot2 >= 0 && (W.nstate[slot2] == 1 || !(cost < W.ng[slot2]))) S.pneed[p] = 0;
            }
            team_sync(slot);
            if (ew == 0) ETICK(PH_ARRIVE);
            if (S.guide_staged) team_state_costs(S, eb, D, P, n, tl, lane);
            else {
                int q = 0;
#pragma unroll 1
                for (int p = 0; p < P.n_prims; ++p) {
                    if (!S.phit[p] && S.pneed[p]) {
                        if ((q % AQ_EXPANDERS) == ew) {
                            const double h = warp_state_cost(eb, D, S.tx[p][n], S.ty[p][n], S.pyaw[p][n], lane);
                            if (lane == 0) S.pprio[p] = xmul(P.hybrid_cost, h);
                        }
                        ++q;
                    }
                }
            }
            team_sync(slot);
            if (ew == 0) ETICK(PH_COST_HEUR);
            if (ew == 0) {
                const bool live = lane < P.n_prims && !S.phit[lane];
                const int my_pos = live ? S.ppos[lane] : -1, my_slot = live ? S.pslot[lane] : -1;
                bool meet = live && !S.pkey_ok[lane];
                if (live) {
#pragma unroll 1
                    for (int q = 0; q < lane; ++q) {
                        if (S.phit[q]) continue;
                        if (my_slot < 0 ? (S.pslot[q] < 0 && S.ppos[q] == my_pos) : (S.pslot[q] == my_slot)) meet = true;
                    }
                }
                const unsigned newm = __ballot_sync(FULL, live && my_slot < 0);
                const bool slow = __any_sync(FULL, meet) || S.n_nodes + __popc(newm) > P.cap_nodes;
                unsigned todo = __ballot_sync(FULL, live);
// ... 123 lines not shown
```

headland_trajectory_planning_b200/csrc/hl_collision.cu:

```cuda
#include "hl_geom.cuh"

#ifndef K1_WARPS
#define K1_WARPS 8
#endif
#define K1_THREADS (K1_WARPS * 32)
#define K1_TILE (K1_WARPS * 128)
#define K1_PER_THREAD (K1_TILE / K1_THREADS)
#define K1_SLICE (K1_TILE / K1_WARPS)
#define K1_ENV_FLOATS 1024
#define K1_PAIR_CAP 2048
#define K1_QBITS 11
#ifndef K1_MIN_CTAS
#define K1_MIN_CTAS 4
#endif
#ifndef K1_UNROLL_OBS
#define K1_UNROLL_OBS 2
#endif
#ifndef K1_UNROLL_FLD
#define K1_UNROLL_FLD 2
#endif
#define K1_PRAGMA(x) _Pragma(#x)
#define K1_UNROLL(n) K1_PRAGMA(unroll n)

__device__ __forceinline__ unsigned smem_u32(const void* p) { return (unsigned)__cvta_generic_to_shared(p); }
// ... 264 lines not shown
        const float delta = fabsf(q - (k + 0.5f) * step);
        g = g * cosf(delta) * 1.0012061467251643f;
    }
    if (g <= (float)HL_LANE_R - eps) return 1;
    if (g > (float)HL_LANE_R + eps) return 0;
    return 2;
}

__device__ __forceinline__ int k1_lane_corners(const K1Env& E, const K1Rect& R, float4 P) {
    const float eps = E.eps;
    const float px = P.x, py = P.y, c = P.z, s = P.w;
    const float rin = (float)HL_LANE_RIN - eps;
    float rx[4], ry[4];
    const float lx[4] = {R.x0, R.x0, R.x1, R.x1};
    const float ly[4] = {R.y1, R.y0, R.y0, R.y1};
#pragma unroll
    for (int j = 0; j < 4; ++j) {
        rx[j] = fmaf(c, lx[j], fmaf(-s, ly[j], px));
        ry[j] = fmaf(s, lx[j], fmaf(c, ly[j], py));
    }
    bool one_holds_all = false;
    unsigned maybe = 0;
#pragma unroll 1
    for (int i = 0; i < E.n_seg; ++i) {
        const float4 sg = lds4(E.seg_a + 4 * i), sd = lds4(E.segd_a + 4 * i);
        bool all_in = true;
#pragma unroll
        for (int j = 0; j < 4; ++j) {
            const int st = k1_corner_in_capsule(sg, sd, rx[j], ry[j], eps);
            all_in = all_in && (st == 1);
            if (st != 0) maybe |= 1u << j;
        }
        if (all_in) one_holds_all = true;
    }
    if (one_holds_all) return HL_FREE;
    if (maybe != 0xFu) return HL_HIT;
    unsigned prev = 0;
    bool covered = true;
#pragma unroll 1
    for (int q = 0; q <= 4 && covered; ++q) {
        const float lxq = R.x0 + 0.25f * (float)q * (R.x1 - R.x0);
        unsigned m = 0xFFFFu;
#pragma unroll
        for (int side = 0; side < 2; ++side) {
            const float lyq = side ? R.y1 : R.y0;
            const float wx = fmaf(c, lxq, fmaf(-s, lyq, px)), wy = fmaf(s, lxq, fmaf(c, lyq, py));
            unsigned in = 0;
            for (int i = 0; i < E.n_seg; ++i) {
                const float4 sg = lds4(E.seg_a + 4 * i), sd = lds4(E.segd_a + 4 * i);
                const float qx = wx - sg.x, qy = wy - sg.y;
                const float t = fminf(fmaxf(fmaf(qx, sd.x, qy * sd.y) * sd.z, 0.f), 1.f);
                const float ddx = fmaf(-t, sd.x, qx), ddy = fmaf(-t, sd.y, qy);
                if (fmaf(ddx, ddx, ddy * ddy) <= rin * rin) in |= 1u << i;
            }
            m &= in;
        }
        if (q > 0 && (prev & m) == 0) covered = false;
        prev = m;
    }
    return covered ? HL_FREE : HL_AMBIG;
}

__device__ __noinline__ void k1_slow_slice(const EnvBatchDev& eb, const int32_t* env_id, const double* poses,
                                           const int32_t* pose_idx, long long n, long long base, unsigned flags,
                                           uint8_t* out, unsigned long long* n_exact, int lane) {
    for (int j = 0; j < (K1_SLICE / 32); ++j) {
        const long long i = base + j * 32 + lane;
        const bool active = i < n;
        const int e = active ? (env_id ? env_id[i] : 0) : 0;
        const EnvDesc& D = eb.desc[e];
        EnvSmem E;
        global_env(eb, D, E);
        double x = 0.0, y = 0.0, yaw = 0.0;
        if (active) { x = poses[3 * i]; y = poses[3 * i + 1]; yaw = poses[3 * i + 2]; }
        const bool with_aux = active && (pose_idx ? ((pose_idx[i] & 1) == 0) : true);
        const float px = (float)(x - D.origin[0]), py = (float)(y - D.origin[1]);
        const bool beyond = fabsf(px) > E.reach || fabsf(py) > E.reach;
        const bool far = !beyond && (!(fabs(yaw) < 1e6) || !(px == px) || !(py == py));
        float sf, cf;
        sincosf((float)yaw, &sf, &cf);
        bool bad = false;
        unsigned amb = flags;
        int r = HL_FREE;
        if (active) r = beyond ? far_status(flags, E.n_seg) : (far ? HL_AMBIG : filter_part(E, px, py, cf, sf, E.ext, flags, &amb));
        if (r == HL_HIT) bad = true;
        warp_resolve(r == HL_AMBIG, x, y, yaw, e, D.body_ext, amb, bad, eb, n_exact, lane);
        if (flags & HL_CHECK_AUX) {
            const unsigned aflags = flags & (HL_CHECK_OBSTACLES | HL_CHECK_BOUNDARY);
            const int na = (active && with_aux && !beyond) ? D.n_aux : 0;
            int na_max = na;
            for (int o = 16; o; o >>= 1) na_max = max(na_max, __shfl_xor_sync(0xffffffffu, na_max, o));
            for (int a = 0; a < na_max; ++a) {
                const bool mine = a < na && !bad;
                const double* ext64 = eb.aux64 + 4 * (size_t)(D.aux_off + (a < D.n_aux ? a : 0));
                unsigned amb2 = aflags;
                int r2 = HL_FREE;
                if (mine) {
                    float ext32[4] = {(float)ext64[0], (float)ext64[1], (float)ext64[2], (float)ext64[3]};
                    r2 = far ? HL_AMBIG : filter_part(E, px, py, cf, sf, ext32, aflags, &amb2);
                    if (r2 == HL_HIT) bad = true;
                }
                bool bad2 = false;
                warp_resolve(r2 == HL_AMBIG, x, y, yaw, e, D.n_aux > 0 ? ext64 : D.body_ext, amb2, bad2, eb, n_exact, lane);
                bad = bad || bad2;
            }
        }
        if (active) out[i] = bad ? 1 : 0;
    }
}

__global__ void __launch_bounds__(K1_THREADS, K1_MIN_CTAS)
k_collision(EnvBatchDev eb, const int32_t* __restrict__ env_id, const double* __restrict__ poses,
            const int32_t* __restrict__ pose_idx, long long n, unsigned flags,
            uint8_t* __restrict__ out, unsigned long long* n_exact, int use_tma) {
    extern __shared__ __align__(16) unsigned char k1_smem[];
    K1Cta& S = *reinterpret_cast<K1Cta*>(k1_smem);
    const int tid = threadIdx.x, lane = tid & 31, warp = tid >> 5;
    const unsigned rbar = smem_u32(&S.bar_raw), ebar = smem_u32(&S.bar_env);
    const long long n_tiles = (n + K1_TILE - 1) / K1_TILE;
    if (tid == 0) { mbar_init(rbar, 1); mbar_init(ebar, 1); S.dq_cnt = 0; }
    asm volatile("fence.mbarrier_init.release.cluster;" ::: "memory");
    __syncthreads();
    unsigned rphase = 0, ephase = 0;
    int staged_env = -1;
    bool env_ok = false;
    K1Env E;
    E.obs_a = E.field_a = E.seg_a = S.env; E.segd_a = reinterpret_cast<const float*>(S.segd);
    E.fld_a = reinterpret_cast<const float*>(S.fld);
    E.n_obs = E.n_field = E.n_seg = 0; E.eps = 0.f;

    auto tile_tma = [&](long long tile) -> bool { return use_tma && tile < n_tiles && (tile + 1) * K1_TILE <= n; };
    auto issue_tile = [&](long long tile) {
        if (tid == 0 && tile_tma(tile)) {
            mbar_expect_tx(rbar, K1_TILE * 24);
            bulk_g2s(smem_u32(S.raw), poses + 3 * tile * K1_TILE, K1_TILE * 24, rbar);
        }
    };
    auto drain_queue = [&]() {
        const int nq = min(S.dq_cnt, K1_DEFER_CAP);
#pragma unroll 1
        for (int e = warp; e < nq; e += K1_WARPS) {
            const K1Defer d = S.dq[e];
            const EnvDesc& D = eb.desc[d.env];
            const double* ext64 = d.rect == 0 ? D.body_ext : eb.aux64 + 4 * (size_t)(D.aux_off + d.rect - 1);
            Pose64 p;
            p.x = poses[3 * d.i]; p.y = poses[3 * d.i + 1];
            const double yaw = poses[3 * d.i + 2];
            p.c = cos(yaw); p.s = sin(yaw);
            double e4[4];
#pragma unroll
            for (int k = 0; k < 4; ++k) e4[k] = ext64[k];
            const bool res = warp_exact_part_check(p, e4, eb, D, d.amb, lane);
            if (lane == 0) {
                if (res) out[d.i] = 1;
                if (n_exact) atomicAdd(n_exact, 1ULL);
            }
        }
    };
    issue_tile(blockIdx.x);

    for (long long tile = blockIdx.x; tile < n_tiles; tile += gridDim.x) {
        const long long base = tile * K1_TILE;
        const int e0 = env_id ? env_id[base] : 0;
        if (e0 != staged_env) {
            __syncthreads();
            const EnvDesc& D0 = eb.desc[e0];
            const int n_o = D0.n_obs * HL_OBS32_STRIDE, n_f = D0.n_field * HL_FIELD32_STRIDE, n_s = D0.n_seg * 4;
// ... 355 lines not shown
```

headland_trajectory_planning_b200/csrc/hl_common.cuh:

```cuda
#pragma once
#include <cuda_runtime.h>
#include <stdint.h>
#include <math.h>
#include "../../include/headland_b200.h"

#define HL_MAX_SEGS 16
#define HL_OBS32_STRIDE 28
#define HL_FIELD32_STRIDE 12
#define HL_PI 3.141592653589793

struct EnvDesc {
    int n_obs, obs_off;
    int n_field, field_off;
    int n_seg, seg_off;
    int n_crit, crit_off;
    int n_guide, guide_off;
    int n_aux, aux_off;
    int all_rect, pad0;
    float eps;
    float reach;
    double origin[2];
    double default_len;
    double body_ext[4];
};

struct EnvBatchDev {
    const EnvDesc* desc;
    const float* obs32;
    const double* obs64;
    const float* field32;
    const double* field64;
    const float* seg32;
    const double* seg64;
    const double* seg_len;
    const double* seg_poly;
    const double* crit64;
    const double* guide_x;
    const double* guide_y;
    const double* guide_yaw;
    const double* guide_s;
    const double* aux64;
    int n_env;
};

struct hl_ctx;
struct hl_env_batch {
    EnvBatchDev dev;
    void* allocs[20];
    int n_allocs;
    int device;
    hl_ctx* owner;
    size_t block_bytes;
};

struct hl_ctx {
    int device;
    int sm_count;
    int max_smem_optin;
    void* astar_ws;
    size_t astar_ws_bytes;
    unsigned int* d_counters;
    void* stage;
    size_t stage_bytes;
    void* env_cache[2];
    size_t env_cache_bytes[2];
    void* copy_stream;
    void* mu;
    void* ws_mu;
    void* ls_state;
    void (*ls_free)(void*);
    int* astar_defer;
    size_t astar_defer_cap;
    int astar_variant;
    void* astar_done;
};
#define HL_ASTAR_SPEC 0
#define HL_ASTAR_WARP 1
#define HL_ASTAR_LEVEL 2

void hl_set_error(const char* fmt, ...);
int hl_enter(const hl_ctx* ctx, const hl_env_batch* envs, const void* probe, const char* what);
#define HL_CUDA_OK(call)                                                            \
    do {                                                                            \
        cudaError_t _e = (call);                                                    \
        if (_e != cudaSuccess) {                                                    \
            hl_set_error("%s failed: %s (%s:%d)", #call, cudaGetErrorString(_e),    \
                         __FILE__, __LINE__);                                       \
            return 1;                                                               \
        }                                                                           \
    } while (0)

#ifdef __CUDACC__
#ifdef HL_SHARED_CODE
#define HL_LOOP _Pragma("unroll 1")
#else
#define HL_LOOP
#endif
#ifndef HL_TINY
#define HL_TINY __forceinline__
#endif
#ifdef HL_SHARED_CODE
#define HL_CODE __noinline__
#else
#define HL_CODE __forceinline__
#endif
static __device__ HL_CODE double m_sin(double x) { return sin(x); }
static __device__ HL_CODE double m_cos(double x) { return cos(x); }
static __device__ HL_CODE double m_tan(double x) { return tan(x); }
static __device__ HL_CODE double m_atan2(double y, double x) { return atan2(y, x); }
static __device__ HL_CODE double m_asin(double x) { return asin(x); }
static __device__ HL_CODE double m_acos(double x) { return acos(x); }
static __device__ HL_CODE double m_fmod(double a, double b) { return fmod(a, b); }
static __device__ HL_CODE void m_sincos(double x, double* s, double* c) { sincos(x, s, c); }
static __device__ HL_CODE double m_fmod_pos(double a, double m) {
    const double aa = fabs(a);
    if (aa < m) return a;
    if (aa < 2.0 * m) return (a > 0.0) ? __dadd_rn(a, -m) : __dadd_rn(a, m);
    return fmod(a, m);
}
__device__ __forceinline__ double xmul(double a, double b) { return __dmul_rn(a, b); }
__device__ __forceinline__ double xadd(double a, double b) { return __dadd_rn(a, b); }
__device__ __forceinline__ double xsub(double a, double b) { return __dadd_rn(a, -b); }
static __device__ HL_TINY double xdiv(double a, double b) { return __ddiv_rn(a, b); }

// ... 39 lines not shown
```

headland_trajectory_planning_b200/csrc/hl_ctx.cu:

```cuda
#include <cstdarg>
#include <cstdio>
#include <cstring>
#include <vector>
#include <cstdlib>
#include <thread>
#include <mutex>
#include <cmath>
#include "hl_common.cuh"

static thread_local char g_err[512] = "";

void hl_set_error(const char* fmt, ...) {
    va_list ap;
    va_start(ap, fmt);
    vsnprintf(g_err, sizeof(g_err), fmt, ap);
    va_end(ap);
}

extern "C" const char* hl_last_error(void) { return g_err; }
extern "C" int hl_abi_version(void) { return HL_ABI_VERSION; }

extern "C" int hl_ctx_create(hl_ctx** out, int device) {
    if (!out) { hl_set_error("hl_ctx_create: out is NULL"); return 1; }
    int n = 0;
    cudaError_t e = cudaGetDeviceCount(&n);
    if (e != cudaSuccess || n == 0) {
        hl_set_error("hl_ctx_create: no CUDA device (%s); this library has no CPU fallback",
                     e == cudaSuccess ? "device count 0" : cudaGetErrorString(e));
        return 1;
    }
    if (device < 0 || device >= n) { hl_set_error("hl_ctx_create: bad device %d of %d", device, n); return 1; }
    HL_CUDA_OK(cudaSetDevice(device));
    cudaDeviceProp prop;
    HL_CUDA_OK(cudaGetDeviceProperties(&prop, device));
    if (prop.major != 10) {
        hl_set_error("hl_ctx_create: device %d is sm_%d%d; this library is built for sm_100a only",
                     device, prop.major, prop.minor);
        return 1;
    }
    hl_ctx* c = new hl_ctx();
    c->device = device;
    c->sm_count = prop.multiProcessorCount;
    c->max_smem_optin = (int)prop.sharedMemPerBlockOptin;
    c->astar_ws = nullptr;
    c->astar_ws_bytes = 0;
    c->astar_defer = nullptr;
    c->astar_defer_cap = 0;
    c->d_counters = nullptr;
    c->stage = nullptr;
    c->stage_bytes = 0;
    c->env_cache[0] = c->env_cache[1] = nullptr;
    c->env_cache_bytes[0] = c->env_cache_bytes[1] = 0;
    c->ls_state = nullptr;
    c->ls_free = nullptr;
    c->copy_stream = nullptr;
    c->mu = new std::recursive_mutex();
    c->ws_mu = new std::recursive_mutex();
    {
        cudaStream_t cs = nullptr;
        if (cudaStreamCreateWithFlags(&cs, cudaStreamNonBlocking) == cudaSuccess) c->copy_stream = cs;
    }
    c->astar_variant = HL_ASTAR_SPEC;
    if (const char* var = getenv("HL_ASTAR_VARIANT")) {
        if (strcmp(var, "warp") == 0) c->astar_variant = HL_ASTAR_WARP;
        else if (strcmp(var, "level") == 0) c->astar_variant = HL_ASTAR_LEVEL;
    }
    c->astar_done = nullptr;
    {
        cudaEvent_t ev = nullptr;
        if (cudaEventCreateWithFlags(&ev, cudaEventDisableTiming) == cudaSuccess) c->astar_done = ev;
    }
    if (!c->astar_done || cudaMalloc(&c->d_counters, 256 * sizeof(unsigned int)) != cudaSuccess) {
        hl_set_error("hl_ctx_create: cudaMalloc / cudaEventCreate failed: %s", cudaGetErrorString(cudaGetLastError()));
        if (c->astar_done) cudaEventDestroy((cudaEvent_t)c->astar_done);
        if (c->copy_stream) cudaStreamDestroy((cudaStream_t)c->copy_stream);
        delete (std::recursive_mutex*)c->mu;
        delete (std::recursive_mutex*)c->ws_mu;
        delete c;
        return 1;
    }
    cudaMemset(c->d_counters, 0, 256 * sizeof(unsigned int));
    *out = c;
    return 0;
}

extern "C" int hl_ctx_device(const hl_ctx* ctx) { return ctx ? ctx->device : -1; }
extern "C" int hl_env_device(const hl_env_batch* envs) { return envs ? envs->device : -1; }

extern "C" int hl_ctx_set_astar_variant(hl_ctx* ctx, int variant) {
    if (!ctx || variant < HL_ASTAR_SPEC || variant > HL_ASTAR_LEVEL) { hl_set_error("hl_ctx_set_astar_variant: bad arguments"); return 1; }
    std::lock_guard<std::recursive_mutex> lock(*(std::recursive_mutex*)ctx->ws_mu);
    ctx->astar_variant = variant;
    return 0;
}

int hl_enter(const hl_ctx* ctx, const hl_env_batch* envs, const void* probe, const char* what) {
    if (!ctx) { hl_set_error("%s: ctx is NULL", what); return 1; }
    if (envs && envs->device != ctx->device) {
        hl_set_error("%s: the environment batch lives on device %d but the context is for device %d "
                     "(upload it through the context of the device that runs the kernels)", what, envs->device, ctx->device);
        return 1;
    }
    if (envs && envs->owner != ctx) { hl_set_error("%s: the environment batch belongs to another context", what); return 1; }
    cudaError_t e = cudaSetDevice(ctx->device);
    if (e != cudaSuccess) { hl_set_error("%s: cudaSetDevice(%d) failed: %s", what, ctx->device, cudaGetErrorString(e)); return 1; }
    if (probe) {
        cudaPointerAttributes a;
        e = cudaPointerGetAttributes(&a, probe);
        if (e != cudaSuccess) { cudaGetLastError(); hl_set_error("%s: cudaPointerGetAttributes failed: %s", what, cudaGetErrorString(e)); return 1; }
        if (a.type != cudaMemoryTypeDevice && a.type != cudaMemoryTypeManaged) {
            hl_set_error("%s: a d_* argument is not device memory (host pointer passed?)", what); return 1;
        }
        if (a.type == cudaMemoryTypeDevice && a.device != ctx->device) {
            hl_set_error("%s: a d_* argument lives on device %d but the context is for device %d", what, a.device, ctx->device);
            return 1;
        }
    }
    return 0;
}

extern "C" void hl_ctx_destroy(hl_ctx* ctx) {
    if (!ctx) return;
    cudaSetDevice(ctx->device);
    if (ctx->astar_ws) cudaFree(ctx->astar_ws);
    if (ctx->astar_defer) cudaFree(ctx->astar_defer);
    if (ctx->d_counters) cudaFree(ctx->d_counters);
    if (ctx->stage) cudaFreeHost(ctx->stage);
    for (int k = 0; k < 2; ++k) if (ctx->env_cache[k]) cudaFree(ctx->env_cache[k]);
    if (ctx->ls_state && ctx->ls_free) ctx->ls_free(ctx->ls_state);
    if (ctx->copy_stream) cudaStreamDestroy((cudaStream_t)ctx->copy_stream);
    if (ctx->astar_done) cudaEventDestroy((cudaEvent_t)ctx->astar_done);
    delete (std::recursive_mutex*)ctx->mu;
    delete (std::recursive_mutex*)ctx->ws_mu;
    delete ctx;
}

extern "C" int hl_ctx_sm_count(const hl_ctx* ctx) { return ctx ? ctx->sm_count : 0; }

extern "C" void hl_env_free(hl_env_batch* envs) {
    if (!envs) return;
    cudaSetDevice(envs->device);
    hl_ctx* c = envs->owner;
    std::unique_lock<std::recursive_mutex> lock;
    if (c && c->mu) lock = std::unique_lock<std::recursive_mutex>(*(std::recursive_mutex*)c->mu);
    for (int i = 0; i < envs->n_allocs; ++i) {
        int slot = -1;
        if (i == 0 && c) {
            if (!c->env_cache[0]) slot = 0;
            else if (!c->env_cache[1]) slot = 1;
            else {
                const int small = c->env_cache_bytes[0] <= c->env_cache_bytes[1] ? 0 : 1;
                if (envs->block_bytes > c->env_cache_bytes[small]) slot = small;
            }
        }
        if (slot >= 0) {
            cudaDeviceSynchronize();
            if (c->env_cache[slot]) cudaFree(c->env_cache[slot]);
            c->env_cache[slot] = envs->allocs[0]; c->env_cache_bytes[slot] = envs->block_bytes;
        } else cudaFree(envs->allocs[i]);
    }
    delete envs;
}

extern "C" int32_t hl_env_count(const hl_env_batch* envs) { return envs ? envs->dev.n_env : 0; }

enum { P_DESC = 0, P_OBS64, P_FIELD64, P_SEG64, P_SEGLEN, P_SEGPOLY, P_CRIT64, P_AUX64, P_GUIDE_AOS,
       P_OBS32, P_FIELD32, P_SEG32, P_GX, P_GY, P_GYAW, P_GS, P_COUNT };
#define P_HOST_POOLS P_OBS32
struct PoolLayout {
    size_t off[P_COUNT];
    size_t host_bytes;
    size_t total;
};
static inline size_t al256(size_t x) { return (x + 255) & ~(size_t)255; }

struct EnvDerive {
    EnvDesc* desc;
    const double* obs64; const double* field64; const double* seg64; const double* aux64; const double* guide_aos;
    float* obs32; float* field32; float* seg32;
    double* gx; double* gy; double* gyaw; double* gs;
};

__global__ void __launch_bounds__(128) k_env_derive(EnvDerive A, int n_env) {
    const int e = blockIdx.x;
    if (e >= n_env) return;
    EnvDesc& D = A.desc[e];
    const int t = threadIdx.x, nt = blockDim.x;
    __shared__ double s_lo[2][128], s_hi[2][128];
    __shared__ double s_origin[2], s_orient;
    __shared__ int s_all_rect;
    const double* obs = A.obs64 + 8 * (size_t)D.obs_off;
    const double* fld = A.field64 + 2 * (size_t)D.field_off;
    const double* seg = A.seg64 + 4 * (size_t)D.seg_off;
    double lo[2] = {1e300, 1e300}, hi[2] = {-1e300, -1e300};
    for (int i = t; i < 4 * D.n_obs; i += nt)
        for (int c = 0; c < 2; ++c) { lo[c] = fmin(lo[c], obs[2 * i + c]); hi[c] = fmax(hi[c], obs[2 * i + c]); }
    for (int i = t; i < D.n_field; i += nt)
        for (int c = 0; c < 2; ++c) { lo[c] = fmin(lo[c], fld[2 * i + c]); hi[c] = fmax(hi[c], fld[2 * i + c]); }
    for (int i = t; i < 2 * D.n_seg; i += nt)
        for (int c = 0; c < 2; ++c) { lo[c] = fmin(lo[c], seg[2 * i + c]); hi[c] = fmax(hi[c], seg[2 * i + c]); }
    for (int c = 0; c < 2; ++c) { s_lo[c][t] = lo[c]; s_hi[c][t] = hi[c]; }
    if (t == 0) s_all_rect = 1;
    __syncthreads();
    for (int w = nt / 2; w > 0; w >>= 1) {
        if (t < w)
            for (int c = 0; c < 2; ++c) { s_lo[c][t] = fmin(s_lo[c][t], s_lo[c][t + w]); s_hi[c][t] = fmax(s_hi[c][t], s_hi[c][t + w]); }
        __syncthreads();
    }
    if (t == 0) {
        double l0 = s_lo[0][0], l1 = s_lo[1][0], h0 = s_hi[0][0], h1 = s_hi[1][0];
        if (l0 > h0) { l0 = l1 = h0 = h1 = 0.0; }
        const double ox = xmul(0.5, xadd(l0, h0)), oy = xmul(0.5, xadd(l1, h1));
        s_origin[0] = ox; s_origin[1] = oy;
        D.origin[0] = ox; D.origin[1] = oy;
        const double extent = xmul(xmul(0.5, fmax(xsub(h0, l0), xsub(h1, l1))), 1.4142135623730951);
        double foot = hypot_cr(fmax(fabs(D.body_ext[0]), fabs(D.body_ext[1])), fmax(fabs(D.body_ext[2]), fabs(D.body_ext[3])));
        for (int a = 0; a < D.n_aux; ++a) {
            const double* x = A.aux64 + 4 * (size_t)(D.aux_off + a);
            foot = fmax(foot, hypot_cr(fmax(fabs(x[0]), fabs(x[1])), fmax(fabs(x[2]), fabs(x[3]))));
        }
        const double reach = xadd(xadd(xadd(extent, 6.0), foot), 4.0);
        D.reach = (float)reach;
        D.eps = (float)xmul(xmul(32.0, 1.1920929e-07), fmax(reach, 8.0));
        double area2 = 0.0;
        for (int i = 0; i < D.n_field; ++i) {
            const int j = (i + 1 == D.n_field) ? 0 : i + 1;
            area2 = xadd(area2, xsub(xmul(fld[2 * i], fld[2 * j + 1]), xmul(fld[2 * j], fld[2 * i + 1])));
        }
        s_orient = area2 < 0 ? -1.0 : 1.0;
    }
    __syncthreads();
    const double ox = s_origin[0], oy = s_origin[1];
    for (int k = t; k < D.n_obs; k += nt) {
        const double* V = obs + 8 * k;
        float* o = A.obs32 + HL_OBS32_STRIDE * (size_t)(D.obs_off + k);
        for (int i = 0; i < 4; ++i) {
            o[2 * i] = (float)xsub(V[2 * i], ox);
            o[2 * i + 1] = (float)xsub(V[2 * i + 1], oy);
        }
        for (int i = 0; i < 4; ++i) {
            const int j = (i + 1) & 3;
            const double ex = xsub(V[2 * j], V[2 * i]), ey = xsub(V[2 * j + 1], V[2 * i + 1]);
            const double ln = sqrt(xadd(xmul(ex, ex), xmul(ey, ey)));
            const double nx = ln > 0 ? xdiv(ey, ln) : 0.0, ny = ln > 0 ? xdiv(-ex, ln) : 0.0;
            const double cc = xadd(xmul(nx, xsub(V[2 * i], ox)), xmul(ny, xsub(V[2 * i + 1], oy)));
            o[8 + 3 * i] = (float)nx; o[9 + 3 * i] = (float)ny; o[10 + 3 * i] = (float)cc;
        }
        const double e0x = xsub(V[2], V[0]), e0y = xsub(V[3], V[1]), e1x = xsub(V[4], V[2]), e1y = xsub(V[5], V[3]);
        const double e2x = xsub(V[6], V[4]), e2y = xsub(V[7], V[5]), e3x = xsub(V[0], V[6]), e3y = xsub(V[1], V[7]);
        const double l0 = sqrt(xadd(xmul(e0x, e0x), xmul(e0y, e0y))), l1 = sqrt(xadd(xmul(e1x, e1x), xmul(e1y, e1y)));
        const double scale = fmax(l0, l1);
        const bool para = xadd(xadd(xadd(fabs(xadd(e0x, e2x)), fabs(xadd(e0y, e2y))), fabs(xadd(e1x, e3x))), fabs(xadd(e1y, e3y))) <= xmul(1e-9, scale);
        const bool perp = l0 > 0 && l1 > 0 && fabs(xadd(xmul(e0x, e1x), xmul(e0y, e1y))) <= xmul(xmul(1e-9, l0), l1);
        const bool is_rect = para && perp;
        if (!is_rect) s_all_rect = 0;
        o[20] = is_rect ? 1.0f : 0.0f;
        o[21] = (float)xsub(xmul(0.25, xadd(xadd(xadd(V[0], V[2]), V[4]), V[6])), ox);
        o[22] = (float)xsub(xmul(0.25, xadd(xadd(xadd(V[1], V[3]), V[5]), V[7])), oy);
        o[23] = (float)(is_rect ? xdiv(e0x, l0) : 1.0); o[24] = (float)(is_rect ? xdiv(e0y, l0) : 0.0);
        o[25] = (float)xmul(0.5, l0); o[26] = (float)xmul(0.5, l1); o[27] = 0.0f;
    }
    {
        const double orient = s_orient;
        for (int i = t; i < D.n_field; i += nt) {
            const int j = (i + 1 == D.n_field) ? 0 : i + 1;
            const double Ax = xsub(fld[2 * i], ox), Ay = xsub(fld[2 * i + 1], oy);
            const double Bx = xsub(fld[2 * j], ox), By = xsub(fld[2 * j + 1], oy);
            const double ex = xsub(Bx, Ax), ey = xsub(By, Ay), ln = sqrt(xadd(xmul(ex, ex), xmul(ey, ey)));
            const double nx = ln > 0 ? xdiv(xmul(orient, ey), ln) : 0.0, ny = ln > 0 ? xdiv(xmul(-orient, ex), ln) : 0.0;
            float* f = A.field32 + HL_FIELD32_STRIDE * (size_t)(D.field_off + i);
            f[0] = (float)Ax; f[1] = (float)Ay; f[2] = (float)xsub(Bx, Ax); f[3] = (float)xsub(By, Ay);
            f[4] = (float)nx; f[5] = (float)ny; f[6] = (float)xadd(xmul(nx, Ax), xmul(ny, Ay));
            f[7] = (float)By;
            f[8] = (float)xadd(xmul(-ny, Ax), xmul(nx, Ay)); f[9] = (float)xadd(xmul(-ny, Bx), xmul(nx, By));
            f[10] = 0.0f; f[11] = 0.0f;
        }
    }
    for (int i = t; i < 4 * D.n_seg; i += nt)
        A.seg32[4 * (size_t)D.seg_off + i] = (float)xsub(seg[i], (i & 1) ? oy : ox);
    {
        const double* g = A.guide_aos + 4 * (size_t)D.guide_off;
        const size_t go = (size_t)D.guide_off;
        for (int i = t; i < D.n_guide; i += nt) {
            A.gx[go + i] = g[4 * i]; A.gy[go + i] = g[4 * i + 1]; A.gyaw[go + i] = g[4 * i + 2]; A.gs[go + i] = g[4 * i + 3];
        }
    }
    __syncthreads();
    if (t == 0) { D.all_rect = s_all_rect; D.pad0 = 0; }
}

extern "C" int hl_env_upload(hl_ctx* ctx, const HlEnvHost* h, int32_t n_env, hl_env_batch** out) {
    if (!ctx || !h || !out || n_env <= 0) { hl_set_error("hl_env_upload: bad arguments"); return 1; }
    if (hl_enter(ctx, nullptr, nullptr, "hl_env_upload")) return 1;
    std::lock_guard<std::recursive_mutex> lock(*(std::recursive_mutex*)ctx->mu);
    size_t n_obs = 0, n_field = 0, n_seg = 0, n_crit = 0, n_guide = 0, n_aux = 0;
    std::vector<size_t> offs(6 * (size_t)n_env);
    for (int e = 0; e < n_env; ++e) {
        const HlEnvHost& E = h[e];
        size_t* o6 = &offs[6 * (size_t)e];
        o6[0] = n_obs; o6[1] = n_field; o6[2] = n_seg; o6[3] = n_crit; o6[4] = n_guide; o6[5] = n_aux;
        if (E.n_seg > HL_MAX_SEGS) { hl_set_error("hl_env_upload: env %d has %d lane segments (max %d)", e, E.n_seg, HL_MAX_SEGS); return 1; }
        if (E.n_obs < 0 || E.n_field < 0 || E.n_seg < 0 || E.n_guide < 0 || E.n_aux < 0 || E.n_crit < 0) {
            hl_set_error("hl_env_upload: env %d has a negative count", e); return 1;
        }
        n_obs += E.n_obs; n_field += E.n_field; n_seg += E.n_seg; n_crit += E.n_crit; n_guide += E.n_guide; n_aux += E.n_aux;
    }
    size_t bytes[P_COUNT];
    bytes[P_DESC] = sizeof(EnvDesc) * (size_t)n_env;
    bytes[P_OBS64] = sizeof(double) * 8 * n_obs;       bytes[P_FIELD64] = sizeof(double) * 2 * n_field;
    bytes[P_SEG64] = sizeof(double) * 4 * n_seg;       bytes[P_SEGLEN] = sizeof(double) * n_seg;
    bytes[P_SEGPOLY] = sizeof(double) * 2 * HL_CAPSULE_VERTS * n_seg;
    bytes[P_CRIT64] = sizeof(double) * 2 * n_crit;     bytes[P_AUX64] = sizeof(double) * 4 * n_aux;
    bytes[P_GUIDE_AOS] = sizeof(double) * 4 * n_guide;
    bytes[P_OBS32] = sizeof(float) * HL_OBS32_STRIDE * n_obs;
    bytes[P_FIELD32] = sizeof(float) * HL_FIELD32_STRIDE * n_field;
    bytes[P_SEG32] = sizeof(float) * 4 * n_seg;
    bytes[P_GX] = bytes[P_GY] = bytes[P_GYAW] = bytes[P_GS] = sizeof(double) * n_guide;
    PoolLayout L;
    L.total = 0;
    for (int k = 0; k < P_COUNT; ++k) {
        if (k == P_HOST_POOLS) L.host_bytes = L.total;
        L.off[k] = L.total; L.total += al256(bytes[k] ? bytes[k] : 1);
    }
    if (L.host_bytes > ctx->stage_bytes) {
        if (ctx->stage) cudaFreeHost(ctx->stage);
        ctx->stage = nullptr; ctx->stage_bytes = 0;
        HL_CUDA_OK(cudaMallocHost(&ctx->stage, L.host_bytes));
        ctx->stage_bytes = L.host_bytes;
    }
    char* S = (char*)ctx->stage;
    EnvDesc* desc = (EnvDesc*)(S + L.off[P_DESC]);
    double* obs64 = (double*)(S + L.off[P_OBS64]);     double* field64 = (double*)(S + L.off[P_FIELD64]);
    double* seg64 = (double*)(S + L.off[P_SEG64]);     double* seg_len = (double*)(S + L.off[P_SEGLEN]);
    double* seg_poly = (double*)(S + L.off[P_SEGPOLY]); double* crit64 = (double*)(S + L.off[P_CRIT64]);
    double* aux64 = (double*)(S + L.off[P_AUX64]);     double* guide = (double*)(S + L.off[P_GUIDE_AOS]);
    auto fill = [&](int e_lo, int e_hi) {
    for (int e = e_lo; e < e_hi; ++e) {
        const HlEnvHost& E = h[e];
        EnvDesc& D = desc[e];
        const size_t* o6 = &offs[6 * (size_t)e];
        const size_t c_obs = o6[0], c_field = o6[1], c_seg = o6[2], c_crit = o6[3], c_guide = o6[4], c_aux = o6[5];
        D.n_obs = E.n_obs;     D.obs_off = (int)c_obs;
        D.n_field = E.n_field; D.field_off = (int)c_field;
        D.n_seg = E.n_seg;     D.seg_off = (int)c_seg;
        D.n_crit = E.n_crit;   D.crit_off = (int)c_crit;
        D.n_guide = E.n_guide; D.guide_off = (int)c_guide;
        D.n_aux = E.n_aux;     D.aux_off = (int)c_aux;
        D.default_len = E.default_search_length;
        for (int k = 0; k < 4; ++k) D.body_ext[k] = E.body_ext[k];
        D.origin[0] = D.origin[1] = 0.0; D.reach = 0.f; D.eps = 0.f; D.all_rect = 1; D.pad0 = 0;
        if (E.n_obs) memcpy(obs64 + 8 * c_obs, E.obs_xy, sizeof(double) * 8 * E.n_obs);
        if (E.n_field) memcpy(field64 + 2 * c_field, E.field_xy, sizeof(double) * 2 * E.n_field);
        if (E.n_seg) {
            memcpy(seg64 + 4 * c_seg, E.seg_xy, sizeof(double) * 4 * E.n_seg);
            memcpy(seg_len + c_seg, E.seg_len, sizeof(double) * E.n_seg);
            memcpy(seg_poly + 2 * HL_CAPSULE_VERTS * c_seg, E.seg_poly, sizeof(double) * 2 * HL_CAPSULE_VERTS * E.n_seg);
        }
        if (E.n_crit) memcpy(crit64 + 2 * c_crit, E.crit_xy, sizeof(double) * 2 * E.n_crit);
        if (E.n_guide) memcpy(guide + 4 * c_guide, E.guide, sizeof(double) * 4 * E.n_guide);
        if (E.n_aux) memcpy(aux64 + 4 * c_aux, E.aux_ext, sizeof(double) * 4 * E.n_aux);
    }
    };
    {
        int nt = (int)std::thread::hardware_concurrency();
        const char* lws = getenv("LOCAL_WORLD_SIZE");
        const int ranks = lws ? atoi(lws) : 1;
        if (ranks > 1) nt /= ranks;
        nt = nt < 1 ? 1 : (nt > 4 ? 4 : nt);
        if (n_env < 1024) nt = 1;
        std::vector<std::thread> th;
        for (int t = 1; t < nt; ++t) th.emplace_back(fill, (int)((long long)n_env * t / nt), (int)((long long)n_env * (t + 1) / nt));
        fill(0, (int)((long long)n_env / nt));
        for (auto& x : th) x.join();
    }
    hl_env_batch* b = new hl_env_batch();
    b->n_allocs = 0;
    b->device = ctx->device;
    b->dev.n_env = n_env;
    char* d = nullptr;
    b->owner = ctx;
    b->block_bytes = L.total;
    int pick = -1;
    for (int k = 0; k < 2; ++k)
        if (ctx->env_cache[k] && ctx->env_cache_bytes[k] >= L.total &&
            (pick < 0 || ctx->env_cache_bytes[k] < ctx->env_cache_bytes[pick])) pick = k;
    if (pick >= 0) {
        d = (char*)ctx->env_cache[pick]; b->block_bytes = ctx->env_cache_bytes[pick];
        ctx->env_cache[pick] = nullptr; ctx->env_cache_bytes[pick] = 0;
    } else if (cudaMalloc(&d, L.total) != cudaSuccess) { delete b; hl_set_error("hl_env_upload: cudaMalloc(%zu) failed", L.total); return 1; }
    b->allocs[b->n_allocs++] = d;
    cudaStream_t cs = (cudaStream_t)ctx->copy_stream;
    EnvDerive A;
    A.desc = (EnvDesc*)(d + L.off[P_DESC]);
    A.obs64 = (const double*)(d + L.off[P_OBS64]);     A.field64 = (const double*)(d + L.off[P_FIELD64]);
    A.seg64 = (const double*)(d + L.off[P_SEG64]);     A.aux64 = (const double*)(d + L.off[P_AUX64]);
    A.guide_aos = (const double*)(d + L.off[P_GUIDE_AOS]);
    A.obs32 = (float*)(d + L.off[P_OBS32]); A.field32 = (float*)(d + L.off[P_FIELD32]); A.seg32 = (float*)(d + L.off[P_SEG32]);
    A.gx = (double*)(d + L.off[P_GX]); A.gy = (double*)(d + L.off[P_GY]); A.gyaw = (double*)(d + L.off[P_GYAW]); A.gs = (double*)(d + L.off[P_GS]);
    cudaError_t ce = cudaMemcpyAsync(d, S, L.host_bytes, cudaMemcpyHostToDevice, cs);
    if (ce == cudaSuccess) {
        k_env_derive<<<n_env, 128, 0, cs>>>(A, n_env);
        ce = cudaGetLastError();
    }
    if (ce == cudaSuccess) ce = cudaStreamSynchronize(cs);
    if (ce != cudaSuccess) {
        hl_env_free(b); hl_set_error("hl_env_upload: copy / k_env_derive failed: %s", cudaGetErrorString(ce)); return 1;
    }
    b->dev.desc = A.desc;
    b->dev.obs32 = A.obs32;     b->dev.obs64 = A.obs64;
    b->dev.field32 = A.field32; b->dev.field64 = A.field64;
    b->dev.seg32 = A.seg32;     b->dev.seg64 = A.seg64;
    b->dev.seg_len = (const double*)(d + L.off[P_SEGLEN]); b->dev.seg_poly = (const double*)(d + L.off[P_SEGPOLY]);
    b->dev.crit64 = (const double*)(d + L.off[P_CRIT64]);
    b->dev.guide_x = A.gx; b->dev.guide_y = A.gy; b->dev.guide_yaw = A.gyaw; b->dev.guide_s = A.gs;
    b->dev.aux64 = A.aux64;
    *out = b;
    return 0;
}
```

headland_trajectory_planning_b200/csrc/hl_geom.cuh:

```cuda
#pragma once
#include "hl_common.cuh"

enum { HL_FREE = 0, HL_HIT = 1, HL_AMBIG = 2 };

__device__ __forceinline__ int far_status(unsigned flags, int n_seg) {
    return ((flags & HL_CHECK_BOUNDARY) || ((flags & HL_CHECK_LANE) && n_seg > 0)) ? HL_HIT : HL_FREE;
}

#define HL_LANE_R 6.0
#define HL_LANE_RIN 5.992771509254837
#define HL_BAND_IN (HL_LANE_RIN - 1e-6)
#define HL_BAND_OUT (HL_LANE_R + 1e-6)

struct Pose64 {
    double x, y, c, s;
};

__device__ __forceinline__ void exact_corners(const Pose64& p, const double* ext, double* cx, double* cy) {
    const double lx[4] = {ext[0], ext[0], ext[1], ext[1]};
    const double ly[4] = {ext[3], ext[2], ext[2], ext[3]};
#pragma unroll
    for (int k = 0; k < 4; ++k) {
        cx[k] = xadd(xsub(xmul(p.c, lx[k]), xmul(p.s, ly[k])), p.x);
        cy[k] = xadd(xadd(xmul(p.s, lx[k]), xmul(p.c, ly[k])), p.y);
// ... 243 lines not shown
                const double tc = xdiv(g0, xsub(g0, g1));
                if (g0 > 0.0) lo = fmax(lo, tc); else hi = fmin(hi, tc);
            }
            dead = __any_sync(0xffffffffu, dead);
            lo = warp_max(lo);
            hi = warp_min(hi);
            if (!dead && lo <= hi) {
                int q = ni++;
                while (q > 0 && (lo_s[q - 1] > lo || (lo_s[q - 1] == lo && hi_s[q - 1] > hi))) {
                    lo_s[q] = lo_s[q - 1]; hi_s[q] = hi_s[q - 1]; --q;
                }
                lo_s[q] = lo; hi_s[q] = hi;
            }
        }
        double cover = 0.0;
        for (int q = 0; q < ni; ++q) {
            if (lo_s[q] > cover) return false;
            cover = fmax(cover, hi_s[q]);
        }
        if (cover < 1.0) return false;
    }
    const double* crit = eb.crit64 + 2 * (size_t)e.crit_off;
    int inside = 0;
    for (int q = lane; q < e.n_crit; q += 32) {
        double u, w;
        exact_local(p, crit[2 * q], crit[2 * q + 1], u, w);
        if (u > ext[0] && u < ext[1] && w > ext[2] && w < ext[3]) inside = 1;
    }
    return !__any_sync(0xffffffffu, inside);
}

static __device__ __noinline__ bool warp_exact_part_check(const Pose64& p, const double* ext, const EnvBatchDev& eb,
                                                          const EnvDesc& e, unsigned flags, int lane) {
    double cx[4], cy[4];
    exact_corners(p, ext, cx, cy);
    if (flags & HL_CHECK_OBSTACLES) {
        const double* V = eb.obs64 + 8 * (size_t)e.obs_off;
        int hit = 0;
        for (int k = lane; k < e.n_obs; k += 32)
            if (exact_rect_hits_quad(p, ext, cx, cy, V + 8 * k)) hit = 1;
        if (__any_sync(0xffffffffu, hit)) return true;
    }
    if (flags & HL_CHECK_BOUNDARY) {
        const double* poly = eb.field64 + 2 * (size_t)e.field_off;
        const int n = e.n_field;
        unsigned par = 0, on = 0;
        int cut = 0;
        for (int i = lane; i < n; i += 32) {
            const int j = (i + 1 == n) ? 0 : i + 1;
            const double ax = poly[2 * i], ay = poly[2 * i + 1], bx = poly[2 * j], by = poly[2 * j + 1];
#pragma unroll
            for (int k = 0; k < 4; ++k) {
                const double px = cx[k], py = cy[k];
                const double cross = xsub(xmul(xsub(bx, ax), xsub(py, ay)), xmul(xsub(by, ay), xsub(px, ax)));
                if (cross == 0.0 && px >= fmin(ax, bx) && px <= fmax(ax, bx) && py >= fmin(ay, by) && py <= fmax(ay, by))
                    on |= 1u << k;
                if ((ay > py) != (by > py)) {
                    const double xint = xadd(xdiv(xmul(xsub(bx, ax), xsub(py, ay)), xsub(by, ay)), ax);
                    if (px < xint) par ^= 1u << k;
                }
            }
            double ua, wa, ub, wb;
            exact_local(p, ax, ay, ua, wa);
            exact_local(p, bx, by, ub, wb);
            if (exact_seg_meets_open_rect(ua, wa, ub, wb, ext)) cut = 1;
        }
        for (int o = 16; o; o >>= 1) { par ^= __shfl_xor_sync(0xffffffffu, par, o); on |= __shfl_xor_sync(0xffffffffu, on, o); }
        if (((par | on) & 0xFu) != 0xFu) return true;
        if (__any_sync(0xffffffffu, cut)) return true;
    }
    if ((flags & HL_CHECK_LANE) && e.n_seg > 0)
        if (!warp_exact_rect_in_lane(p, ext, cx, cy, eb, e, lane)) return true;
    return false;
}

struct EnvSmem {
    int n_obs, n_field, n_seg, all_rect;
    float eps, reach;
    float ext[4];
    const float* obs;
    const float* field;
    const float* seg;
};

__device__ __forceinline__ float f_rcp(float x) { return __fdividef(1.0f, x); }
__device__ __forceinline__ float f_sqrt(float x) { return x > 0.0f ? x * rsqrtf(x) : 0.0f; }

static __device__ HL_CODE int corner_in_capsule(const float* sg, float wx, float wy, float eps) {
    const float ex = sg[2] - sg[0], ey = sg[3] - sg[1];
    const float len2 = fmaf(ex, ex, ey * ey);
    const float qx = wx - sg[0], qy = wy - sg[1];
    const float tt = fmaf(qx, ex, qy * ey) * f_rcp(len2);
    const float t = fminf(fmaxf(tt, 0.f), 1.f);
    const float ddx = fmaf(-t, ex, qx), ddy = fmaf(-t, ey, qy);
    const float d2 = fmaf(ddx, ddx, ddy * ddy);
    const float rin = (float)HL_LANE_RIN - eps, rout = (float)HL_LANE_R + eps;
    if (d2 <= rin * rin) return 1;
    if (d2 > rout * rout) return 0;
    float g = f_sqrt(d2);
    if (tt < 0.f || tt > 1.f) {
        const float il = rsqrtf(len2);
        const float along = fabsf(fmaf(ddx, ex, ddy * ey)) * il, across = fabsf(fmaf(ddy, ex, -ddx * ey)) * il;
        const float phi = atan2f(across, along);
        const float q = 1.5707963267948966f - phi;
        const float step = 0.09817477042468103f;
        const float k = floorf(q / step);
        const float delta = fabsf(q - (k + 0.5f) * step);
        g = g * cosf(delta) * 1.0012061467251643f;
    }
    if (g <= (float)HL_LANE_R - eps) return 1;
    if (g > (float)HL_LANE_R + eps) return 0;
    return 2;
}

struct FiltState {
    unsigned near_mask;
    unsigned amb;
    bool hit, inside, overflow;
};

static __device__ __forceinline__ void filt_stage1(const EnvSmem& E, float px, float py, float c, float s,
                                                   const float* ext, unsigned flags, FiltState& F) {
    const float eps = E.eps;
    const float hx = 0.5f * (ext[1] - ext[0]), hy = 0.5f * (ext[3] - ext[2]);
    const float mx = 0.5f * (ext[1] + ext[0]), my = 0.5f * (ext[3] + ext[2]);
    const float Cx = fmaf(c, mx, fmaf(-s, my, px)), Cy = fmaf(s, mx, fmaf(c, my, py));
    unsigned amb = 0;
    bool hit = false;
    if (flags & HL_CHECK_OBSTACLES) {
        bool a_obs = false;
        if (E.all_rect) {
            HL_LOOP
            for (int k = 0; k < E.n_obs; ++k) {
                const float* o = E.obs + HL_OBS32_STRIDE * k;
                const float4 b0 = *reinterpret_cast<const float4*>(o + 20);
                const float4 b1 = *reinterpret_cast<const float4*>(o + 24);
                const float dx = b0.y - Cx, dy = b0.z - Cy;
                const float ax = b0.w, ay = b1.x, ha = b1.y, hb = b1.z;
                const float p = fabsf(fmaf(ax, c, ay * s)), q = fabsf(fmaf(ay, c, -ax * s));
                const float du = fabsf(fmaf(dx, c, dy * s)), dv = fabsf(fmaf(dy, c, -dx * s));
                const float da = fabsf(fmaf(dx, ax, dy * ay)), db = fabsf(fmaf(dy, ax, -dx * ay));
                const float sep = fmaxf(fmaxf(du - fmaf(ha, p, fmaf(hb, q, hx)), dv - fmaf(ha, q, fmaf(hb, p, hy))),
                                        fmaxf(da - fmaf(hx, p, fmaf(hy, q, ha)), db - fmaf(hx, q, fmaf(hy, p, hb))));
                hit |= sep < -eps;
                a_obs |= fabsf(sep) <= eps;
            }
        } else {
            float rx[4], ry[4];
            const float lx[4] = {ext[0], ext[0], ext[1], ext[1]};
            const float ly[4] = {ext[3], ext[2], ext[2], ext[3]};
#pragma unroll
            for (int j = 0; j < 4; ++j) {
                rx[j] = fmaf(c, lx[j], fmaf(-s, ly[j], px));
                ry[j] = fmaf(s, lx[j], fmaf(c, ly[j], py));
            }
            HL_LOOP
            for (int k = 0; k < E.n_obs; ++k) {
                const float* o = E.obs + HL_OBS32_STRIDE * k;
                float sep = -INFINITY;
#pragma unroll
                for (int i = 0; i < 4; ++i) {
                    float nx = o[8 + 3 * i], ny = o[9 + 3 * i], cc = o[10 + 3 * i];
                    float m = fminf(fminf(fmaf(nx, rx[0], ny * ry[0]), fmaf(nx, rx[1], ny * ry[1])),
                                    fminf(fmaf(nx, rx[2], ny * ry[2]), fmaf(nx, rx[3], ny * ry[3])));
                    sep = fmaxf(sep, m - cc);
                }
                float umin = INFINITY, umax = -INFINITY, wmin = INFINITY, wmax = -INFINITY;
#pragma unroll
                for (int v = 0; v < 4; ++v) {
                    float dx = o[2 * v] - px, dy = o[2 * v + 1] - py;
                    float u = fmaf(c, dx, s * dy), w = fmaf(c, dy, -s * dx);
                    umin = fminf(umin, u); umax = fmaxf(umax, u);
                    wmin = fminf(wmin, w); wmax = fmaxf(wmax, w);
                }
                sep = fmaxf(sep, fmaxf(fmaxf(umin - ext[1], ext[0] - umax), fmaxf(wmin - ext[3], ext[2] - wmax)));
                hit |= sep < -eps;
                a_obs |= fabsf(sep) <= eps;
            }
        }
        if (a_obs) amb |= HL_CHECK_OBSTACLES;
    }
    bool inside = false, overflow = false;
    unsigned near_mask = 0;
    if (flags & HL_CHECK_BOUNDARY) {
        const int n = E.n_field;
        const float rho_eps = sqrtf(fmaf(hx, hx, hy * hy)) + eps;
        HL_LOOP
        for (int i = 0; i < n; ++i) {
            const float* e = E.field + HL_FIELD32_STRIDE * i;
            const float4 r0 = *reinterpret_cast<const float4*>(e);
            const float4 r1 = *reinterpret_cast<const float4*>(e + 4);
            const float dyc = Cy - r0.y;
            const bool straddle = (r0.y > Cy) != (r1.w > Cy);
            const float lhs = (Cx - r0.x) * r0.w, rhs = r0.z * dyc;
            inside ^= straddle && ((r0.w > 0.0f) ? (lhs < rhs) : (lhs > rhs));
            const float sd = fmaf(r1.x, Cx, fmaf(r1.y, Cy, -r1.z));
            if (!(fabsf(sd) > rho_eps)) {
                const float nu = fmaf(r1.x, c, r1.y * s), nv = fmaf(r1.y, c, -r1.x * s);
                const float rn = fmaf(hx, fabsf(nu), hy * fabsf(nv));
                if (!(fabsf(sd) > rn + eps)) { if (i < 32) near_mask |= 1u << i; else overflow = true; }
            }
        }
    }
    F.near_mask = near_mask; F.amb = amb; F.hit = hit; F.inside = inside; F.overflow = overflow;
}

static __device__ __forceinline__ void filt_field2(const EnvSmem& E, float px, float py, float c, float s,
                                                   const float* ext, FiltState& F) {
    const float eps = E.eps;
    const float hx = 0.5f * (ext[1] - ext[0]), hy = 0.5f * (ext[3] - ext[2]);
    const float mx = 0.5f * (ext[1] + ext[0]), my = 0.5f * (ext[3] + ext[2]);
    const float Cx = fmaf(c, mx, fmaf(-s, my, px)), Cy = fmaf(s, mx, fmaf(c, my, py));
    unsigned near_mask = F.near_mask;
    bool all_clear = !F.overflow, cut = false;
    while (near_mask) {
        const int i = __ffs(near_mask) - 1;
        near_mask &= near_mask - 1;
        const float* e = E.field + HL_FIELD32_STRIDE * i;
        const float Ax = e[0], Ay = e[1], Bx = Ax + e[2], By = e[7], nx = e[4], ny = e[5];
        const float nu = fmaf(nx, c, ny * s), nv = fmaf(ny, c, -nx * s);
        const float ct = fmaf(-ny, Cx, nx * Cy);
        const float rt = fmaf(hx, fabsf(nv), hy * fabsf(nu));
        if (ct - rt > fmaxf(e[8], e[9]) + eps || ct + rt < fminf(e[8], e[9]) - eps) continue;
        float dxa = Ax - px, dya = Ay - py, dxb = Bx - px, dyb = By - py;
        float ua = fmaf(c, dxa, s * dya), wa = fmaf(c, dya, -s * dxa);
        float ub = fmaf(c, dxb, s * dyb), wb = fmaf(c, dyb, -s * dxb);
        if ((fminf(ua, ub) > ext[1] + eps) || (fmaxf(ua, ub) < ext[0] - eps) ||
            (fminf(wa, wb) > ext[3] + eps) || (fmaxf(wa, wb) < ext[2] - eps)) continue;
        all_clear = false;
        float t0 = 0.f, t1 = 1.f;
        bool dead = false;
        const float a2[2] = {ua, wa}, d2v[2] = {ub - ua, wb - wa};
        const float lo2[2] = {ext[0] + eps, ext[2] + eps}, hi2[2] = {ext[1] - eps, ext[3] - eps};
#pragma unroll
        for (int ax = 0; ax < 2; ++ax) {
            if (fabsf(d2v[ax]) < 1e-12f) {
                if (a2[ax] <= lo2[ax] || a2[ax] >= hi2[ax]) dead = true;
            } else {
                float inv = f_rcp(d2v[ax]);
                float tl = (lo2[ax] - a2[ax]) * inv, th = (hi2[ax] - a2[ax]) * inv;
                t0 = fmaxf(t0, fminf(tl, th));
                t1 = fminf(t1, fmaxf(tl, th));
            }
        }
        if (!dead && (t1 - t0) * f_sqrt(fmaf(d2v[0], d2v[0], d2v[1] * d2v[1])) > 8.0f * eps) { cut = true; break; }
    }
    if (cut) F.hit = true;
    else if (all_clear) { if (!F.inside) F.hit = true; }
    else F.amb |= HL_CHECK_BOUNDARY;
}

static __device__ __forceinline__ int filt_lane(const EnvSmem& E, float px, float py, float c, float s,
                                                const float* ext, bool* lane_amb) {
    const float eps = E.eps;
    const float hx = 0.5f * (ext[1] - ext[0]), hy = 0.5f * (ext[3] - ext[2]);
    const float mx = 0.5f * (ext[1] + ext[0]), my = 0.5f * (ext[3] + ext[2]);
    const float Cx = fmaf(c, mx, fmaf(-s, my, px)), Cy = fmaf(s, mx, fmaf(c, my, py));
    *lane_amb = false;
    const float rho = sqrtf(fmaf(hx, hx, hy * hy));
    const float rin = (float)HL_LANE_RIN - eps, rout = (float)HL_LANE_R + eps;
    bool accepted = false, need_corners = false;
    HL_LOOP
    for (int i = 0; i < E.n_seg && !accepted; ++i) {
        const float* sg = E.seg + 4 * i;
        float ex = sg[2] - sg[0], ey = sg[3] - sg[1];
        float inv = f_rcp(fmaf(ex, ex, ey * ey));
        float qx = Cx - sg[0], qy = Cy - sg[1];
        float t = fminf(fmaxf(fmaf(qx, ex, qy * ey) * inv, 0.f), 1.f);
        float ddx = fmaf(-t, ex, qx), ddy = fmaf(-t, ey, qy);
        float d = f_sqrt(fmaf(ddx, ddx, ddy * ddy));
        if (d + rho <= rin) accepted = true;
        else if (d - rho <= rout) need_corners = true;
    }
    if (accepted) return HL_FREE;
    if (!need_corners) return HL_HIT;
    float rx[4], ry[4];
    const float lx[4] = {ext[0], ext[0], ext[1], ext[1]};
    const float ly[4] = {ext[3], ext[2], ext[2], ext[3]};
#pragma unroll
    for (int j = 0; j < 4; ++j) {
        rx[j] = fmaf(c, lx[j], fmaf(-s, ly[j], px));
        ry[j] = fmaf(s, lx[j], fmaf(c, ly[j], py));
    }
    bool one_holds_all = false;
    unsigned maybe = 0;
    HL_LOOP
    for (int i = 0; i < E.n_seg; ++i) {
        const float* sg = E.seg + 4 * i;
        bool all_in = true;
#pragma unroll
        for (int j = 0; j < 4; ++j) {
            const int st = corner_in_capsule(sg, rx[j], ry[j], eps);
            all_in = all_in && (st == 1);
            if (st != 0) maybe |= 1u << j;
        }
        if (all_in) one_holds_all = true;
    }
    if (one_holds_all) return HL_FREE;
    if (maybe != 0xFu) return HL_HIT;
    unsigned prev = 0;
    bool covered = true;
#pragma unroll 1
    for (int q = 0; q <= 4 && covered; ++q) {
        const float lxq = ext[0] + 0.25f * (float)q * (ext[1] - ext[0]);
        unsigned m = 0xFFFFu;
#pragma unroll
        for (int side = 0; side < 2; ++side) {
            const float lyq = side ? ext[3] : ext[2];
            const float wx = fmaf(c, lxq, fmaf(-s, lyq, px)), wy = fmaf(s, lxq, fmaf(c, lyq, py));
            unsigned in = 0;
            HL_LOOP
            for (int i = 0; i < E.n_seg; ++i) {
                const float* sg = E.seg + 4 * i;
                float ex = sg[2] - sg[0], ey = sg[3] - sg[1];
                float inv = f_rcp(fmaf(ex, ex, ey * ey));
                float qx = wx - sg[0], qy = wy - sg[1];
                float t = fminf(fmaxf(fmaf(qx, ex, qy * ey) * inv, 0.f), 1.f);
                float ddx = fmaf(-t, ex, qx), ddy = fmaf(-t, ey, qy);
                if (fmaf(ddx, ddx, ddy * ddy) <= rin * rin) in |= 1u << i;
            }
            m &= in;
        }
        if (q > 0 && (prev & m) == 0) covered = false;
        prev = m;
    }
    if (!covered) *lane_amb = true;
    return HL_FREE;
}

static __device__ HL_CODE int filter_part(const EnvSmem& E, float px, float py, float c, float s,
                                           const float* ext, unsigned flags, unsigned* which_ambig) {
    FiltState F;
    filt_stage1(E, px, py, c, s, ext, flags, F);
    if (flags & HL_CHECK_BOUNDARY) filt_field2(E, px, py, c, s, ext, F);
    if (F.hit) return HL_HIT;
    unsigned amb = F.amb;
    if ((flags & HL_CHECK_LANE) && E.n_seg > 0) {
        bool lane_amb;
        if (filt_lane(E, px, py, c, s, ext, &lane_amb) == HL_HIT) return HL_HIT;
        if (lane_amb) amb |= HL_CHECK_LANE;
    }
    if (amb) { if (which_ambig) *which_ambig = amb; return HL_AMBIG; }
    return HL_FREE;
}

static __device__ bool pose_infeasible(const EnvBatchDev& eb, const EnvDesc& D, const EnvSmem& E,
                                double x, double y, double yaw, bool with_aux, unsigned flags,
                                unsigned long long* n_exact) {
    float px = (float)(x - D.origin[0]), py = (float)(y - D.origin[1]);
    if (fabsf(px) > E.reach || fabsf(py) > E.reach) return far_status(flags, E.n_seg) == HL_HIT;
    bool far = !(fabs(yaw) < 1e6) || !(px == px) || !(py == py);
    float sf, cf;
    sincosf((float)yaw, &sf, &cf);
    unsigned amb = flags;
    int r = far ? HL_AMBIG : filter_part(E, px, py, cf, sf, E.ext, flags, &amb);
    if (r == HL_HIT) return true;
    bool bad = false;
    Pose64 p;
    bool have64 = false;
    if (r == HL_AMBIG) {
        p.x = x; p.y = y; p.c = m_cos(yaw); p.s = m_sin(yaw);
        have64 = true;
        if (n_exact) atomicAdd(n_exact, 1ULL);
        bad = exact_part_check(p, D.body_ext, eb, D, amb);
        if (bad) return true;
    }
    if (with_aux && (flags & HL_CHECK_AUX)) {
        unsigned aflags = flags & (HL_CHECK_OBSTACLES | HL_CHECK_BOUNDARY);
        for (int a = 0; a < D.n_aux; ++a) {
            const double* ext64 = eb.aux64 + 4 * (size_t)(D.aux_off + a);
            float ext32[4] = {(float)ext64[0], (float)ext64[1], (float)ext64[2], (float)ext64[3]};
            unsigned amb2 = aflags;
            int r2 = far ? HL_AMBIG : filter_part(E, px, py, cf, sf, ext32, aflags, &amb2);
            if (r2 == HL_HIT) return true;
            if (r2 == HL_AMBIG) {
                if (!have64) { p.x = x; p.y = y; p.c = m_cos(yaw); p.s = m_sin(yaw); have64 = true; }
                if (n_exact) atomicAdd(n_exact, 1ULL);
                if (exact_part_check(p, ext64, eb, D, amb2)) return true;
            }
        }
    }
    return false;
}

__device__ __forceinline__ void global_env(const EnvBatchDev& eb, const EnvDesc& D, EnvSmem& E) {
    E.n_obs = D.n_obs; E.n_field = D.n_field; E.n_seg = D.n_seg; E.all_rect = D.all_rect;
    E.eps = D.eps; E.reach = D.reach;
    for (int k = 0; k < 4; ++k) E.ext[k] = (float)D.body_ext[k];
    E.obs = eb.obs32 + (size_t)HL_OBS32_STRIDE * D.obs_off;
    E.field = eb.field32 + HL_FIELD32_STRIDE * (size_t)D.field_off;
    E.seg = eb.seg32 + 4 * (size_t)D.seg_off;
}
```

headland_trajectory_planning_b200/csrc/hl_rs.cu:

```cuda
#define HL_SHARED_CODE 1
#include <cstring>
#include "hl_geom.cuh"
#include "hl_rs.cuh"

#define RS_WARPS 4
#define RS_PLANS 6

struct RsWarpSmem {
    double lens[HL_RS_CANDIDATES][HL_RS_MAX_SEGS];
    double L[HL_RS_CANDIDATES], Lc[HL_RS_CANDIDATES];
    double prio[HL_RS_CANDIDATES];
    int acc[HL_RS_CANDIDATES];
    int order[HL_RS_CANDIDATES];
    unsigned char valid[HL_RS_CANDIDATES + 2], accept[HL_RS_CANDIDATES + 2];
    RsProblem prob;
    RsPlan plans[RS_PLANS];
};

__global__ void __launch_bounds__(RS_WARPS * 32)
k_rs_all_paths(EnvBatchDev eb, int have_env, const int32_t* __restrict__ env_id,
               const double* __restrict__ sg, long long n, double maxc, double step, double max_steer,
               unsigned flags, HlRsWord* __restrict__ words, int32_t* __restrict__ count,
               int32_t* __restrict__ order_out) {
    extern __shared__ __align__(16) unsigned char rs_smem_raw[];
    RsWarpSmem* sm = reinterpret_cast<RsWarpSmem*>(rs_smem_raw);
    const int lane = threadIdx.x & 31, wid = threadIdx.x >> 5;
    RsWarpSmem& W = sm[wid];
    const long long n_warps = (long long)gridDim.x * RS_WARPS;
    const double stepn = xmul(step, maxc);
    const float inv_maxc = (float)(1.0 / maxc);
    const bool body_only = !(flags & HL_CHECK_AUX);
    for (long long i = (long long)blockIdx.x * RS_WARPS + wid; i < n; i += n_warps) {
        double q0[3] = {sg[6 * i], sg[6 * i + 1], sg[6 * i + 2]};
        double q1[3] = {sg[6 * i + 3], sg[6 * i + 4], sg[6 * i + 5]};
        double cq, sq;
        {
            const double phi = xsub(q1[2], q0[2]);
            double sn, cs;
            m_sincos(lane == 1 ? phi : q0[2], &sn, &cs);
            const double c0 = __shfl_sync(0xffffffffu, cs, 0), s0 = __shfl_sync(0xffffffffu, sn, 0);
            const double cp = __shfl_sync(0xffffffffu, cs, 1), sp = __shfl_sync(0xffffffffu, sn, 1);
            cq = c0; sq = -s0;
            if (lane == 0) {
                RsProblem Pr;
                const double dx = xsub(q1[0], q0[0]), dy = xsub(q1[1], q0[1]);
                Pr.phi = phi;
                Pr.x = xmul(xadd(xmul(c0, dx), xmul(s0, dy)), maxc);
                Pr.y = xmul(xadd(xmul(-s0, dx), xmul(c0, dy)), maxc);
                Pr.sp = sp; Pr.cp = cp;
                Pr.xb = xadd(xmul(Pr.x, cp), xmul(Pr.y, sp));
                Pr.yb = xsub(xmul(Pr.x, sp), xmul(Pr.y, cp));
                W.prob = Pr;
            }
            __syncwarp();
        }
        rs_candidates_warp(W.prob, W.valid, W.lens, lane);
        if (lane < RS_N_GROUPS) rs_select_group(lane, W.valid, W.lens, W.accept, W.Lc);
        __syncwarp();
        int m;
        {
            const int a0 = W.accept[lane];
            const int a1 = (lane + 32 < HL_RS_CANDIDATES) ? W.accept[lane + 32] : 0;
            const unsigned b0 = __ballot_sync(0xffffffffu, a0 == 1), b1 = __ballot_sync(0xffffffffu, a1 == 1);
            const unsigned bad = __ballot_sync(0xffffffffu, a0 == 2 || a1 == 2);
            const unsigned lt = (1u << lane) - 1u;
            const int n0 = __popc(b0);
            if (a0 == 1) { int k = __popc(b0 & lt); W.acc[k] = lane; W.L[k] = W.Lc[lane]; }
            if (a1 == 1) { int k = n0 + __popc(b1 & lt); W.acc[k] = lane + 32; W.L[k] = W.Lc[lane + 32]; }
            m = bad ? -1 : n0 + __popc(b1);
        }
        __syncwarp();
        const int mm = m < 0 ? 0 : m;
        for (int k = lane; k < mm; k += 32)
            W.prio[k] = rs_path_cost(0.0, W.acc[k], W.lens[W.acc[k]], max_steer, 5000.0, 1000.0, 1.0);
        __syncwarp();
        if (lane == 0) {
            if (mm > 0) heapdict_order(W.prio, mm, W.order);
            count[i] = m;
        }
        __syncwarp();
        HlRsWord* out = words + (size_t)i * HL_RS_CANDIDATES;
        if (order_out)
            for (int k = lane; k < HL_RS_CANDIDATES; k += 32)
                order_out[(size_t)i * HL_RS_CANDIDATES + k] = (k < mm) ? W.order[k] : -1;
        const int e = (have_env && env_id) ? env_id[i] : 0;
        const EnvDesc* Dp = have_env ? &eb.desc[e] : nullptr;
        EnvSmem E;
        if (have_env && mm > 0) {
            global_env(eb, *Dp, E);
            E.eps += 6e-5f;
        }
        HL_LOOP
        for (int k0 = 0; k0 < mm; k0 += RS_PLANS) {
            const int nk = (mm - k0) < RS_PLANS ? (mm - k0) : RS_PLANS;
            __syncwarp();
            rs_make_plans_warp(W.acc, W.lens, nullptr, k0, nk, W.plans, q0, cq, sq, have_env ? Dp->origin : nullptr, maxc, stepn, lane);
            if (lane < nk) {
                const int k = k0 + lane;
                const int c = W.acc[k];
                const RsPlan& plan = W.plans[lane];
                HlRsWord w;
                w.cand = c; w.n_seg = plan.nseg; w.npts = plan.npts; w.collide = -1;
                w.L = xdiv(W.L[k], maxc);
                w.cost = W.prio[k];
                for (int s = 0; s < HL_RS_MAX_SEGS; ++s) {
                    w.len[s] = (s < plan.nseg) ? xdiv(W.lens[c][s], maxc) : 0.0;
                    w.nlen[s] = (s < plan.nseg) ? W.lens[c][s] : 0.0;
                }
                out[k] = w;
            }
            __syncwarp();
            if (!have_env) continue;
            const EnvDesc& D = *Dp;
            HL_LOOP
            for (int r = 0; r < nk; ++r) {
                const RsPlan& plan = W.plans[r];
                const int npts = plan.npts;
                int hit = 0;
                if (body_only) {
                    const int passes = (npts + 31) >> 5;
                    for (int pass = 0; pass < passes && !hit; ++pass) {
                        const int j = lane * passes + pass;
                        int st = HL_FREE;
                        unsigned amb = 0;
                        if (j < npts) {
                            float fx, fy, fc, fs;
                            rs_sample_world32(plan, j, inv_maxc, fx, fy, fc, fs);
                            if (fabsf(fx) > E.reach || fabsf(fy) > E.reach) st = far_status(flags, E.n_seg);
                            else if (!(fx == fx) || !(fy == fy) || !(fc == fc)) { st = HL_AMBIG; amb = flags; }
                            else st = filter_part(E, fx, fy, fc, fs, E.ext, flags, &amb);
                        }
                        hit = __any_sync(0xffffffffu, st == HL_HIT);
                        if (!hit && __any_sync(0xffffffffu, st == HL_AMBIG)) {
                            int bad = 0;
                            if (st == HL_AMBIG) {
                                double lx, ly, lyaw, wx, wy, wyaw;
                                int cs, dir;
                                rs_sample_local(plan, j, maxc, lx, ly, lyaw, cs, dir);
                                rs_to_world(q0, cq, sq, lx, ly, lyaw, wx, wy, wyaw);
                                Pose64 p64;
                                p64.x = wx; p64.y = wy; p64.c = m_cos(wyaw); p64.s = m_sin(wyaw);
                                bad = exact_part_check(p64, D.body_ext, eb, D, amb) ? 1 : 0;
                            }
                            hit = __any_sync(0xffffffffu, bad);
                        }
                    }
                } else {
                    EnvSmem E0 = E;
                    E0.eps = D.eps;
                    for (int base = 0; base < npts && !hit; base += 32) {
                        const int j = base + lane;
                        int bad = 0;
                        if (j < npts) {
                            double lx, ly, lyaw, wx, wy, wyaw;
                            int cs, dir;
                            rs_sample_local(plan, j, maxc, lx, ly, lyaw, cs, dir);
                            rs_to_world(q0, cq, sq, lx, ly, lyaw, wx, wy, wyaw);
                            bad = pose_infeasible(eb, D, E0, wx, wy, wyaw, (j & 1) == 0, flags, nullptr) ? 1 : 0;
                        }
                        hit = __any_sync(0xffffffffu, bad);
                    }
                }
                if (lane == 0) out[k0 + r].collide = hit ? 1 : 0;
            }
        }
        __syncwarp();
    }
}

__global__ void __launch_bounds__(RS_WARPS * 32)
k_rs_sample(const double* __restrict__ start, const HlRsWord* __restrict__ words, long long m, double maxc,
            double step, const long long* __restrict__ offset, double* __restrict__ ox, double* __restrict__ oy,
            double* __restrict__ oyaw, double* __restrict__ ocs, int8_t* __restrict__ odir) {
    __shared__ RsPlan plans[RS_WARPS];
    const int lane = threadIdx.x & 31, wid = threadIdx.x >> 5;
    const long long n_warps = (long long)gridDim.x * RS_WARPS;
    for (long long i = (long long)blockIdx.x * RS_WARPS + wid; i < m; i += n_warps) {
        const HlRsWord w = words[i];
        double q0[3] = {start[3 * i], start[3 * i + 1], start[3 * i + 2]};
        __syncwarp();
        if (lane == 0) {
            double lens[HL_RS_MAX_SEGS];
            for (int s = 0; s < HL_RS_MAX_SEGS; ++s) lens[s] = w.nlen[s];
            rs_make_plan(w.cand, lens, maxc, xmul(step, maxc), plans[wid]);
        }
        __syncwarp();
        const RsPlan& P = plans[wid];
        const long long o = offset[i];
        const long long cap = offset[i + 1] - o;
        const double cq = cos(-q0[2]), sq = sin(-q0[2]);
        for (int j = lane; j < P.npts && j < cap; j += 32) {
            double lx, ly, lyaw, wx, wy, wyaw;
            int cs, dir;
            rs_sample_local(P, j, maxc, lx, ly, lyaw, cs, dir);
            rs_to_world(q0, cq, sq, lx, ly, lyaw, wx, wy, wyaw);
            ox[o + j] = wx; oy[o + j] = wy; oyaw[o + j] = wyaw;
            ocs[o + j] = cs == 0 ? 0.0 : (cs > 0 ? maxc : -maxc);
            odir[o + j] = (int8_t)dir;
        }
    }
}

extern "C" int hl_rs_all_paths(hl_ctx* ctx, const hl_env_batch* envs, const int32_t* d_env_id,
                               const double* d_start_goal, int64_t n, double maxc, double step,
                               double max_steer, uint32_t flags, HlRsWord* d_words, int32_t* d_count,
                               int32_t* d_order, void* stream) {
    if (!ctx || !d_start_goal || !d_words || !d_count || n < 0) { hl_set_error("hl_rs_all_paths: bad arguments"); return 1; }
    if (n == 0) return 0;
    if (hl_enter(ctx, envs, d_words, "hl_rs_all_paths")) return 1;
    long long blocks = (n + RS_WARPS - 1) / RS_WARPS;
    long long cap = (long long)ctx->sm_count * 8;
    int grid = (int)(blocks < cap ? blocks : cap);
    EnvBatchDev eb;
    memset(&eb, 0, sizeof(eb));
    if (envs) eb = envs->dev;
    k_rs_all_paths<<<grid, RS_WARPS * 32, sizeof(RsWarpSmem) * RS_WARPS, (cudaStream_t)stream>>>(
        eb, envs ? 1 : 0, d_env_id, d_start_goal, (long long)n, maxc, step, max_steer, flags, d_words,
        d_count, d_order);
    HL_CUDA_OK(cudaGetLastError());
    return 0;
}

extern "C" int hl_rs_sample(hl_ctx* ctx, const double* d_start, const HlRsWord* d_words, int64_t m,
                            double maxc, double step, const int64_t* d_offset, double* d_x, double* d_y,
                            double* d_yaw, double* d_cs, int8_t* d_dir, void* stream) {
    if (!ctx || !d_start || !d_words || !d_offset || !d_x || !d_y || !d_yaw || !d_cs || !d_dir || m < 0) {
        hl_set_error("hl_rs_sample: bad arguments"); return 1;
    }
    if (m == 0) return 0;
    if (hl_enter(ctx, nullptr, d_x, "hl_rs_sample")) return 1;
    long long blocks = (m + RS_WARPS - 1) / RS_WARPS;
    long long cap = (long long)ctx->sm_count * 8;
    int grid = (int)(blocks < cap ? blocks : cap);
    k_rs_sample<<<grid, RS_WARPS * 32, 0, (cudaStream_t)stream>>>(
        d_start, d_words, (long long)m, maxc, step, (const long long*)d_offset, d_x, d_y, d_yaw, d_cs, d_dir);
    HL_CUDA_OK(cudaGetLastError());
    return 0;
}
```

headland_trajectory_planning_b200/ops.py:

```python
import ctypes as C

import numpy as np

from . import _lib
from ._lib import CHECK_AUX, CHECK_BOUNDARY, CHECK_LANE, CHECK_OBSTACLES


def _torch():
    import torch
    return torch


def _device(envs=None, *tensors):
    import torch
    if not torch.cuda.is_available():
        raise _lib.HeadlandError("no CUDA device: headland_trajectory_planning_b200 has no CPU fallback")
    cur = torch.cuda.current_device()
    if envs is not None and getattr(envs, "device", cur) != cur:
        raise _lib.HeadlandError(f"environment batch was uploaded to cuda:{envs.device} but the current device of this "
                                 f"thread is cuda:{cur} (torch.cuda.set_device / EnvBatch(device=...))")
    for t in tensors:
        if torch.is_tensor(t) and (not t.is_cuda or t.device.index != cur):
            raise _lib.HeadlandError(f"tensor on {t.device} passed to an op running on cuda:{cur}")
    return torch.device("cuda", cur)


def collision_check(envs, poses, env_id=None, pose_idx=None, flags=CHECK_OBSTACLES | CHECK_BOUNDARY,
                    count_exact=False):
    torch = _torch()
    lib = _lib.load_library()
    dev = _device(envs, poses, env_id, pose_idx)
    if not torch.is_tensor(poses):
        poses = torch.from_numpy(np.ascontiguousarray(np.asarray(poses, dtype=np.float64)[:, :3])).to(dev)
    poses = poses.contiguous()
    n = poses.shape[0]
    if env_id is not None and not torch.is_tensor(env_id):
        env_id = torch.from_numpy(np.ascontiguousarray(env_id, dtype=np.int32)).to(dev)
    if pose_idx is not None and not torch.is_tensor(pose_idx):
        pose_idx = torch.from_numpy(np.ascontiguousarray(pose_idx, dtype=np.int32)).to(dev)
    out = torch.empty(n, dtype=torch.uint8, device=dev)
    n_exact = torch.zeros(1, dtype=torch.int64, device=dev) if count_exact else None
    if n == 0:
        return (out, n_exact) if count_exact else out
    _lib.check(lib.hl_collision_check(envs.ctx, envs.handle, _lib.ptr(env_id), _lib.ptr(poses),
                                      _lib.ptr(pose_idx), n, flags, _lib.ptr(out), _lib.ptr(n_exact),
                                      _lib.stream_ptr()), "hl_collision_check")
    if count_exact:
        return out, n_exact
    return out


def path_reduce(envs, pose_bad, path_start):
    torch = _torch()
    lib = _lib.load_library()
    n_paths = path_start.shape[0] - 1
    out = torch.empty(n_paths, dtype=torch.uint8, device=pose_bad.device)
    _lib.check(lib.hl_path_reduce(envs.ctx, _lib.ptr(pose_bad), _lib.ptr(path_start), n_paths,
                                  _lib.ptr(out), _lib.stream_ptr()), "hl_path_reduce")
    return out


def ypark_paths(cand, step):
    torch = _torch()
    lib = _lib.load_library()
    if torch.is_tensor(cand) and cand.is_cuda:
        dev = _device(None, cand)
        d_cand = cand.to(torch.float64).reshape(-1, 8).contiguous()
        n = d_cand.shape[0]
        counts = (torch.round(d_cand[:, 0] / step) + torch.round(d_cand[:, 1] / step) + 2).to(torch.int64)
        d_off = torch.zeros(n + 1, dtype=torch.int64, device=dev)
        if n:
            d_off[1:] = torch.cumsum(counts, 0)
        total = int(d_off[-1].item()) if n else 0
        poses = torch.empty((total, 3), dtype=torch.float64, device=dev)
        if n:
            _lib.check(lib.hl_ypark_paths(_lib.get_ctx(dev.index), _lib.ptr(d_cand), _lib.ptr(d_off), n, float(step),
                                          _lib.ptr(poses), _lib.stream_ptr()), "hl_ypark_paths")
        return poses, d_off
    dev = _device()
    cand = np.ascontiguousarray(np.asarray(cand, dtype=np.float64).reshape(-1, 8))
    n = cand.shape[0]
    counts = (np.rint(cand[:, 0] / step) + np.rint(cand[:, 1] / step) + 2).astype(np.int64)
    offsets = np.concatenate([[0], np.cumsum(counts)]).astype(np.int64)
    poses = torch.empty((int(offsets[-1]), 3), dtype=torch.float64, device=dev)
    if n == 0:
        return poses, offsets
    d_cand = torch.from_numpy(cand).to(dev)
    d_off = torch.from_numpy(offsets).to(dev)
    _lib.check(lib.hl_ypark_paths(_lib.get_ctx(dev.index), _lib.ptr(d_cand), _lib.ptr(d_off), n, float(step),
                                  _lib.ptr(poses), _lib.stream_ptr()), "hl_ypark_paths")
    return poses, offsets


def arc_paths(cand, step):
    torch = _torch()
    lib = _lib.load_library()
    dev = _device()
    cand = np.ascontiguousarray(np.asarray(cand, dtype=np.float64).reshape(-1, 8))
    n = cand.shape[0]
    counts = (np.rint(cand[:, 5] / step) + 1).astype(np.int64)
    offsets = np.concatenate([[0], np.cumsum(counts)]).astype(np.int64)
    poses = torch.empty((int(offsets[-1]), 3), dtype=torch.float64, device=dev)
    if n == 0:
        return poses, offsets
    d_cand = torch.from_numpy(cand).to(dev)
    d_off = torch.from_numpy(offsets).to(dev)
    _lib.check(lib.hl_arc_paths(_lib.get_ctx(dev.index), _lib.ptr(d_cand), _lib.ptr(d_off), n, float(step),
                                _lib.ptr(poses), _lib.stream_ptr()), "hl_arc_paths")
    return poses, offsets


def ref_path_batch(x, y, direction, in_offsets, wheel_base, desired_v=0.5, ds=0.1):
    torch = _torch()
    lib = _lib.load_library()
    dev = _device()
    def dev_t(a, dt):
        if torch.is_tensor(a):
            return a.to(dev).to(dt).contiguous()
        return torch.from_numpy(np.ascontiguousarray(a)).to(dev).to(dt).contiguous()
    x, y = dev_t(x, torch.float64), dev_t(y, torch.float64)
    direction = dev_t(direction, torch.int8)
    in_off = dev_t(np.asarray(in_offsets, dtype=np.int64), torch.int64)
    n = in_off.numel() - 1
    counts = torch.zeros(max(n, 1), dtype=torch.int64, device=dev)
    status = torch.zeros(max(n, 1), dtype=torch.int32, device=dev)
    ctx = _lib.get_ctx(dev.index)
    if n > 0:
        _lib.check(lib.hl_ref_path_count(ctx, _lib.ptr(x), _lib.ptr(y), _lib.ptr(direction), _lib.ptr(in_off), n, float(ds),
                                         _lib.ptr(counts), _lib.ptr(status), _lib.stream_ptr()), "hl_ref_path_count")
    out_off = torch.zeros(n + 1, dtype=torch.int64, device=dev)
    if n > 0:
        out_off[1:] = torch.cumsum(counts[:n], 0)
# ... 295 lines not shown
```

include/headland_b200.h:

```cpp
#ifndef HEADLAND_B200_H
#define HEADLAND_B200_H

#include <stdint.h>

#ifdef __cplusplus
extern "C" {
#endif

#define HL_ABI_VERSION 4

#define HL_MAX_PRIMS        16
#define HL_MAX_ROLLOUT      16
#define HL_CAPSULE_VERTS    66
#define HL_RS_CANDIDATES    46
#define HL_RS_MAX_SEGS       5

#define HL_CHECK_OBSTACLES  1u
#define HL_CHECK_BOUNDARY   2u
#define HL_CHECK_AUX        4u
#define HL_CHECK_LANE       8u

enum {
    HL_STATUS_OK                 = 0,
    HL_STATUS_START_GOAL_BLOCKED = 1,
    HL_STATUS_OPEN_EMPTY         = 2,
    HL_STATUS_MAX_NODES          = 3,
    HL_STATUS_CAPACITY           = 4,
    HL_STATUS_RS_ASSERT          = 5
};

typedef struct hl_ctx hl_ctx;
typedef struct hl_env_batch hl_env_batch;

typedef struct {
    int32_t n_obs;
    const double* obs_xy;
    int32_t n_field;
    const double* field_xy;
    int32_t n_seg;
    const double* seg_xy;
    const double* seg_poly;
    const double* seg_len;
    int32_t n_crit;
    const double* crit_xy;
    int32_t n_guide;
    const double* guide;
    double default_search_length;
    double body_ext[4];
    int32_t n_aux;
    const double* aux_ext;
} HlEnvHost;

typedef struct {
    double plan_resolution;
    double yaw_resolution;
    double maxc;
    double max_steer;
    double wheel_base;
    int32_t n_prims;
    double prim_steer[HL_MAX_PRIMS];
    double prim_dir[HL_MAX_PRIMS];
    double prim_yaw_step[HL_MAX_PRIMS];
    double prim_curv[HL_MAX_PRIMS];
    double prim_steer_eff[HL_MAX_PRIMS];
    int32_t steps_default;
    int32_t steps_large;
    double steer_cost, delta_steer_cost, direction_change_cost, reverse_cost, hybrid_cost;
    double min_length_to_goal;
    int32_t max_nodes;
    int32_t max_path_poses;
    int32_t motion_type;
    int32_t dubins_capacity;
} HlSearchParams;

typedef struct {
    int32_t env_id;
    int32_t reserved;
    double start[3];
    double goal[3];
} HlScenario;

typedef struct {
    int32_t status;
    int32_t counter;
    int32_t n_expanded;
    int32_t arrival;
    int32_t path_len;
    int32_t rs_word;
    int64_t path_offset;
    double  goal_cost;
    int64_t n_pose_checks;
    int64_t n_exact;
    int64_t keys_offset;
    int64_t cycles;
    int64_t n_pose_checks_ref;
} HlPlanResult;

typedef struct {
    int32_t cand;
    int32_t n_seg;
    int32_t npts;
    int32_t collide;
    double  L;
    double  cost;
    double  len[HL_RS_MAX_SEGS];
    double  nlen[HL_RS_MAX_SEGS];
} HlRsWord;

const char* hl_last_error(void);
int hl_abi_version(void);
int hl_ctx_create(hl_ctx** out, int device);
void hl_ctx_destroy(hl_ctx* ctx);
int hl_ctx_sm_count(const hl_ctx* ctx);
int hl_ctx_device(const hl_ctx* ctx);
int hl_ctx_set_astar_variant(hl_ctx* ctx, int variant);

int hl_env_upload(hl_ctx* ctx, const HlEnvHost* h_envs, int32_t n_env, hl_env_batch** out);
void hl_env_free(hl_env_batch* envs);
int32_t hl_env_count(const hl_env_batch* envs);
int hl_env_device(const hl_env_batch* envs);

int hl_collision_check(hl_ctx* ctx, const hl_env_batch* envs, const int32_t* d_env_id,
                       const double* d_poses, const int32_t* d_pose_idx, int64_t n,
                       uint32_t flags, uint8_t* d_out, unsigned long long* d_n_exact,
                       void* stream);

int hl_path_reduce(hl_ctx* ctx, const uint8_t* d_pose_bad, const int64_t* d_path_start,
                   int64_t n_paths, uint8_t* d_path_bad, void* stream);

int hl_ypark_paths(hl_ctx* ctx, const double* d_cand, const int64_t* d_offsets, int64_t n, double step,
                   double* d_poses, void* stream);

int hl_arc_paths(hl_ctx* ctx, const double* d_cand, const int64_t* d_offsets, int64_t n, double step,
                 double* d_poses, void* stream);

int hl_ref_path_count(hl_ctx* ctx, const double* d_x, const double* d_y, const int8_t* d_dir,
                      const int64_t* d_in_offsets, int64_t n_paths, double ds, int64_t* d_counts,
                      int32_t* d_status, void* stream);
int hl_ref_path_fill(hl_ctx* ctx, const double* d_x, const double* d_y, const int8_t* d_dir,
                     const int64_t* d_in_offsets, const int64_t* d_out_offsets, const int32_t* d_status,
                     int64_t n_paths, double wheel_base, double desired_v, double ds, double* d_workspace,
                     double* d_out, void* stream);

int hl_dubins_count(hl_ctx* ctx, const double* d_pairs, int64_t n, double rho, double step, double ds,
                    int32_t append_goal, int64_t* d_slots, int32_t* d_word, double* d_length, void* stream);
int hl_dubins_knots(hl_ctx* ctx, const double* d_pairs, int64_t n, double rho, double step, double ds,
                    int32_t append_goal, const int64_t* d_slot_offsets, double* d_workspace,
                    int32_t* d_n_knots, int64_t* d_n_rows, double* d_samples , void* stream);
int hl_dubins_fill(hl_ctx* ctx, int64_t n, double ds, const int64_t* d_slot_offsets, const int64_t* d_row_offsets,
                   const int32_t* d_n_knots, double* d_workspace, double* d_out, void* stream);

int hl_min_boundary_distance(hl_ctx* ctx, const hl_env_batch* envs, const int32_t* d_env_id, const double* d_poses,
                             const int64_t* d_path_start, int64_t n_paths, int32_t with_aux, double* d_out, void* stream);

int hl_corridor_hits(hl_ctx* ctx, const hl_env_batch* envs, const int32_t* d_env_id, const double* d_points,
                     const int64_t* d_line_start, int64_t n_lines, double radius, uint8_t* d_out, void* stream);

int hl_rs_all_paths(hl_ctx* ctx, const hl_env_batch* envs, const int32_t* d_env_id,
                    const double* d_start_goal, int64_t n, double maxc, double step,
                    double max_steer, uint32_t flags, HlRsWord* d_words, int32_t* d_count,
                    int32_t* d_order, void* stream);

int hl_rs_sample(hl_ctx* ctx, const double* d_start, const HlRsWord* d_words, int64_t m,
                 double maxc, double step, const int64_t* d_offset, double* d_x, double* d_y,
                 double* d_yaw, double* d_cs, int8_t* d_dir, void* stream);

int hl_hybrid_astar_batch(hl_ctx* ctx, const hl_env_batch* envs, const HlScenario* d_scen,
                          int32_t n_scen, const HlSearchParams* h_params,
                          HlPlanResult* d_results, int32_t* d_expanded_keys, int64_t keys_capacity,
                          unsigned long long* d_keys_cursor, double* d_path_x, double* d_path_y, double* d_path_yaw,
                          double* d_path_k, int8_t* d_path_dir, int64_t path_capacity,
                          unsigned long long* d_path_cursor, void* stream);
int64_t hl_hybrid_astar_workspace_bytes(const hl_ctx* ctx, const HlSearchParams* h_params);
#define HL_ASTAR_N_PHASES 13
int hl_astar_phase_cycles(hl_ctx* ctx, uint64_t* h_out, int32_t n, int32_t reset);

int hl_distance_field(hl_ctx* ctx, const uint8_t* d_occ, int32_t w, int32_t h, int32_t gi,
                      int32_t gj, int32_t motion_type, double* d_out, int32_t* h_sweeps,
                      void* stream);

typedef struct {
    int64_t occ_offset;
    int64_t out_offset;
    int32_t w, h;
    int32_t gi, gj;
} HlGridField;

int hl_distance_field_batch(hl_ctx* ctx, const uint8_t* d_occ, int64_t occ_bytes,
                            const HlGridField* h_fields, int32_t n_fields, int32_t motion_type,
                            double* d_out, int64_t out_elems, int32_t* h_sweeps, void* stream);

int hl_grid_pack(hl_ctx* ctx, const uint8_t* d_occ, int32_t w, int32_t h, uint32_t* d_bits,
                 void* stream);
int hl_grid_footprint_check(hl_ctx* ctx, const uint32_t* d_occ_bits, int32_t w, int32_t h,
                            double res, const double* d_poses, int64_t n,
                            const double body_ext[4], uint8_t* d_out, void* stream);

int hl_measure_fp32_peak(hl_ctx* ctx, double* h_tflops);

#ifdef __cplusplus
}
#endif
#endif
// ... 1 lines not shown
```

Baseline: 204,600.

## Add per-environment uniform cell grid to prune obstacle, field and lane collision tests

```diff
diff --git a/headland_trajectory_planning_b200/_lib.py b/headland_trajectory_planning_b200/_lib.py
--- a/headland_trajectory_planning_b200/_lib.py
+++ b/headland_trajectory_planning_b200/_lib.py
@@ -7,7 +7,7 @@
 HERE = os.path.dirname(os.path.abspath(__file__))
 _LIB_NAME = "libheadland_b200.so"
 
-ABI_VERSION = 4
+ABI_VERSION = 5
 HL_MAX_PRIMS = 16
 HL_CAPSULE_VERTS = 66
 HL_RS_CANDIDATES = 46
@@ -78,7 +78,7 @@
 
 EXPORTS = [
     "hl_last_error", "hl_abi_version", "hl_ctx_create", "hl_ctx_destroy", "hl_ctx_sm_count", "hl_ctx_device",
-    "hl_ctx_set_astar_variant", "hl_env_upload", "hl_env_free", "hl_env_count", "hl_env_device", "hl_collision_check", "hl_path_reduce",
+    "hl_ctx_set_astar_variant", "hl_env_upload", "hl_env_free", "hl_env_count", "hl_env_device", "hl_env_cells", "hl_collision_check", "hl_path_reduce",
     "hl_rs_all_paths", "hl_rs_sample", "hl_hybrid_astar_batch", "hl_hybrid_astar_workspace_bytes", "hl_astar_phase_cycles",
     "hl_distance_field", "hl_distance_field_batch", "hl_grid_pack", "hl_grid_footprint_check", "hl_measure_fp32_peak", "hl_ypark_paths", "hl_arc_paths", "hl_ref_path_count", "hl_ref_path_fill",
     "hl_dubins_count", "hl_dubins_knots", "hl_dubins_fill", "hl_min_boundary_distance", "hl_corridor_hits",
@@ -144,6 +144,7 @@
         lib.hl_env_free.restype = None
         lib.hl_env_count.argtypes = [vp]
         lib.hl_env_count.restype = i32
+        lib.hl_env_cells.argtypes = [vp, i32, vp, vp, vp, i64]
         lib.hl_collision_check.argtypes = [vp, vp, vp, vp, vp, i64, u32, vp, vp, vp]
         lib.hl_path_reduce.argtypes = [vp, vp, vp, i64, vp, vp]
         lib.hl_rs_all_paths.argtypes = [vp, vp, vp, vp, i64, dbl, dbl, dbl, u32, vp, vp, vp, vp]
diff --git a/headland_trajectory_planning_b200/csrc/hl_astar.cu b/headland_trajectory_planning_b200/csrc/hl_astar.cu
--- a/headland_trajectory_planning_b200/csrc/hl_astar.cu
+++ b/headland_trajectory_planning_b200/csrc/hl_astar.cu
@@ -112,7 +112,7 @@
         const long long i = base + lane;
         int st = HL_FREE;
         unsigned amb = 0;
-        if (i < cnt) st = pose_filter(D, E, rx[i], ry[i], ryaw[i], FLAGS, &amb);
+        if (i < cnt) st = pose_filter(eb, D, E, rx[i], ry[i], ryaw[i], FLAGS, &amb);
         const unsigned livem = __ballot_sync(FULL, i < cnt);
         const unsigned hitm = __ballot_sync(FULL, st == HL_HIT);
         const unsigned ambm = __ballot_sync(FULL, st == HL_AMBIG);
@@ -299,7 +299,7 @@
                         rs_sample_world32(plan, j, inv_maxc, fx, fy, fc, fs);
                         if (fabsf(fx) > Ers.reach || fabsf(fy) > Ers.reach) st = far_status(FLAGS, Ers.n_seg);
                         else if (!(fx == fx) || !(fy == fy) || !(fc == fc)) { st = HL_AMBIG; amb = FLAGS; }
-                        else st = filter_part(Ers, fx, fy, fc, fs, Ers.ext, FLAGS, &amb);
+                        else st = filter_body(Ers, env_table(eb, D), fx, fy, fc, fs, FLAGS, &amb);
                     }
                     const unsigned livem = __ballot_sync(FULL, j < npts);
                     const unsigned hitm = __ballot_sync(FULL, st == HL_HIT);
@@ -376,7 +376,7 @@
             for (int idx = lane; idx < total; idx += 32) {
                 const int p = idx / np1, j = idx - p * np1;
                 unsigned amb = 0;
-                int st = pose_filter(D, E, S.tx[p][j], S.ty[p][j], S.pyaw[p][j], FLAGS, &amb);
+                int st = pose_filter(eb, D, E, S.tx[p][j], S.ty[p][j], S.pyaw[p][j], FLAGS, &amb);
                 S.pamb[p][j] = (st == HL_AMBIG) ? (unsigned char)amb : 0;
                 if (st == HL_HIT) atomicOr(&S.phit[p], 1);
             }
diff --git a/headland_trajectory_planning_b200/csrc/hl_astar_common.cuh b/headland_trajectory_planning_b200/csrc/hl_astar_common.cuh
--- a/headland_trajectory_planning_b200/csrc/hl_astar_common.cuh
+++ b/headland_trajectory_planning_b200/csrc/hl_astar_common.cuh
@@ -181,14 +181,14 @@
     heap_set_t<0>(H, n, slot, prio);
 }
 
-__device__ HL_CODE int pose_filter(const EnvDesc& D, const EnvSmem& E, double x, double y, double yaw,
+__device__ HL_CODE int pose_filter(const EnvBatchDev& eb, const EnvDesc& D, const EnvSmem& E, double x, double y, double yaw,
                                            unsigned flags, unsigned* amb) {
     float px = (float)(x - D.origin[0]), py = (float)(y - D.origin[1]);
     if (fabsf(px) > E.reach || fabsf(py) > E.reach) return far_status(flags, E.n_seg);
     if (!(fabs(yaw) < 1e6) || !(px == px) || !(py == py)) { *amb = flags; return HL_AMBIG; }
     float sf, cf;
     sincosf((float)yaw, &sf, &cf);
-    return filter_part(E, px, py, cf, sf, E.ext, flags, amb);
+    return filter_body(E, env_table(eb, D), px, py, cf, sf, flags, amb);
 }
 
 __device__ __noinline__ bool pose_exact(const EnvBatchDev& eb, const EnvDesc& D, double x, double y, double yaw,
@@ -275,7 +275,7 @@
     if (lane < 2) {
         const double* q = lane == 0 ? start : goal;
         unsigned amb = flags;
-        int r = pose_filter(D, E, q[0], q[1], q[2], flags, &amb);
+        int r = pose_filter(eb, D, E, q[0], q[1], q[2], flags, &amb);
         bad = (r == HL_HIT) || (r == HL_AMBIG && pose_exact(eb, D, q[0], q[1], q[2], amb));
     }
     bad = __any_sync(FULL, bad);
diff --git a/headland_trajectory_planning_b200/csrc/hl_astar_level.cuh b/headland_trajectory_planning_b200/csrc/hl_astar_level.cuh
--- a/headland_trajectory_planning_b200/csrc/hl_astar_level.cuh
+++ b/headland_trajectory_planning_b200/csrc/hl_astar_level.cuh
@@ -308,7 +308,7 @@
                 rs_sample_world32(plan, j, inv_maxc, fx, fy, fc, fs);
                 if (fabsf(fx) > E.reach || fabsf(fy) > E.reach) st2 = far_status(LS_FLAGS, E.n_seg);
                 else if (!(fx == fx) || !(fy == fy) || !(fc == fc)) { st2 = HL_AMBIG; amb = LS_FLAGS; }
-                else st2 = filter_part(E, fx, fy, fc, fs, E.ext, LS_FLAGS, &amb);
+                else st2 = filter_body(E, env_table(C.eb, D), fx, fy, fc, fs, LS_FLAGS, &amb);
             }
             const unsigned livem = __ballot_sync(FULL, j < npts);
             const unsigned hitm = __ballot_sync(FULL, st2 == HL_HIT);
@@ -392,7 +392,7 @@
         EnvSmem E;
         global_env(C.eb, D, E);
         unsigned amb = 0;
-        const int st = pose_filter(D, E, x, y, R.pyaw[j], LS_FLAGS, &amb);
+        const int st = pose_filter(C.eb, D, E, x, y, R.pyaw[j], LS_FLAGS, &amb);
         R.pamb[j] = (st == HL_AMBIG) ? (unsigned char)amb : 0;
         if (st == HL_HIT) atomicOr(&R.phit, 1);
         if (j == 0 && p == 0) atomicAdd(&S.checks, (unsigned long long)(P.n_prims * np1));
diff --git a/headland_trajectory_planning_b200/csrc/hl_astar_spec.cuh b/headland_trajectory_planning_b200/csrc/hl_astar_spec.cuh
--- a/headland_trajectory_planning_b200/csrc/hl_astar_spec.cuh
+++ b/headland_trajectory_planning_b200/csrc/hl_astar_spec.cuh
@@ -245,7 +245,7 @@
             rs_sample_world32(plan, j, inv_maxc, fx, fy, fc, fs);
             if (fabsf(fx) > Ers.reach || fabsf(fy) > Ers.reach) st2 = far_status(FLAGS, Ers.n_seg);
             else if (!(fx == fx) || !(fy == fy) || !(fc == fc)) { st2 = HL_AMBIG; amb = FLAGS; }
-            else st2 = filter_part(Ers, fx, fy, fc, fs, Ers.ext, FLAGS, &amb);
+            else st2 = filter_body(Ers, env_table(eb, D), fx, fy, fc, fs, FLAGS, &amb);
         }
         const unsigned livem = __ballot_sync(FULL, j < npts);
         const unsigned hitm = __ballot_sync(FULL, st2 == HL_HIT);
@@ -467,7 +467,7 @@
                                 rs_sample_world32(plan, j, inv_maxc, fx, fy, fc, fs);
                                 if (fabsf(fx) > Ers.reach || fabsf(fy) > Ers.reach) st2 = far_status(FLAGS, Ers.n_seg);
                                 else if (!(fx == fx) || !(fy == fy) || !(fc == fc)) st2 = HL_AMBIG;
-                                else st2 = filter_part(Ers, fx, fy, fc, fs, Ers.ext, FLAGS, &amb);
+                                else st2 = filter_body(Ers, env_table(eb, D), fx, fy, fc, fs, FLAGS, &amb);
                             }
                         }
                         const unsigned hitm = __ballot_sync(FULL, st2 == HL_HIT);
@@ -715,7 +715,7 @@
                 for (int idx = tl; idx < P.n_prims * far_cnt; idx += AQ_TEAM) {
                     const int p = idx / far_cnt, j = n - (idx - p * far_cnt);
                     unsigned amb = 0;
-                    int st = pose_filter(D, E, S.tx[p][j], S.ty[p][j], S.pyaw[p][j], FLAGS, &amb);
+                    int st = pose_filter(eb, D, E, S.tx[p][j], S.ty[p][j], S.pyaw[p][j], FLAGS, &amb);
                     S.pamb[p][j] = (st == HL_AMBIG) ? (unsigned char)amb : 0;
                     if (st == HL_HIT) atomicOr(&S.phit[p], 1);
                 }
@@ -728,7 +728,7 @@
                     const int q = idx / rem, j = idx - q * rem;
                     const int p = __fns(live, 0, q + 1);
                     unsigned amb = 0;
-                    int st = pose_filter(D, E, S.tx[p][j], S.ty[p][j], S.pyaw[p][j], FLAGS, &amb);
+                    int st = pose_filter(eb, D, E, S.tx[p][j], S.ty[p][j], S.pyaw[p][j], FLAGS, &amb);
                     S.pamb[p][j] = (st == HL_AMBIG) ? (unsigned char)amb : 0;
                     if (st == HL_HIT) atomicOr(&S.phit[p], 1);
                 }
diff --git a/headland_trajectory_planning_b200/csrc/hl_collision.cu b/headland_trajectory_planning_b200/csrc/hl_collision.cu
--- a/headland_trajectory_planning_b200/csrc/hl_collision.cu
+++ b/headland_trajectory_planning_b200/csrc/hl_collision.cu
@@ -370,7 +370,7 @@
         bool bad = false;
         unsigned amb = flags;
         int r = HL_FREE;
-        if (active) r = beyond ? far_status(flags, E.n_seg) : (far ? HL_AMBIG : filter_part(E, px, py, cf, sf, E.ext, flags, &amb));
+        if (active) r = beyond ? far_status(flags, E.n_seg) : (far ? HL_AMBIG : filter_body(E, env_table(eb, D), px, py, cf, sf, flags, &amb));
         if (r == HL_HIT) bad = true;
         warp_resolve(r == HL_AMBIG, x, y, yaw, e, D.body_ext, amb, bad, eb, n_exact, lane);
         if (flags & HL_CHECK_AUX) {
diff --git a/headland_trajectory_planning_b200/csrc/hl_common.cuh b/headland_trajectory_planning_b200/csrc/hl_common.cuh
--- a/headland_trajectory_planning_b200/csrc/hl_common.cuh
+++ b/headland_trajectory_planning_b200/csrc/hl_common.cuh
@@ -8,6 +8,10 @@
 #define HL_OBS32_STRIDE 28
 #define HL_FIELD32_STRIDE 12
 #define HL_PI 3.141592653589793
+#define HL_CELL 1.0f
+#define HL_MAX_CELLS 65536
+enum { HL_FC_CROSS = 0, HL_FC_INSIDE_CLEAR = 1, HL_FC_INSIDE_NEAR = 2, HL_FC_OUTSIDE = 3 };
+enum { HL_LC_CHECK = 0, HL_LC_FREE = 1, HL_LC_HIT = 2 };
 
 struct EnvDesc {
     int n_obs, obs_off;
@@ -19,6 +23,10 @@
     int all_rect, pad0;
     float eps;
     float reach;
+    int cell_off;
+    int cell_nx, cell_ny;
+    float cell_x0, cell_y0;
+    int pad1;
     double origin[2];
     double default_len;
     double body_ext[4];
@@ -40,6 +48,7 @@
     const double* guide_yaw;
     const double* guide_s;
     const double* aux64;
+    const uint4* cells;
     int n_env;
 };
 
diff --git a/headland_trajectory_planning_b200/csrc/hl_ctx.cu b/headland_trajectory_planning_b200/csrc/hl_ctx.cu
--- a/headland_trajectory_planning_b200/csrc/hl_ctx.cu
+++ b/headland_trajectory_planning_b200/csrc/hl_ctx.cu
@@ -7,6 +7,7 @@
 #include <mutex>
 #include <cmath>
 #include "hl_common.cuh"
+#include "hl_geom.cuh"
 
 static thread_local char g_err[512] = "";
 
@@ -165,7 +166,7 @@
 extern "C" int32_t hl_env_count(const hl_env_batch* envs) { return envs ? envs->dev.n_env : 0; }
 
 enum { P_DESC = 0, P_OBS64, P_FIELD64, P_SEG64, P_SEGLEN, P_SEGPOLY, P_CRIT64, P_AUX64, P_GUIDE_AOS,
-       P_OBS32, P_FIELD32, P_SEG32, P_GX, P_GY, P_GYAW, P_GS, P_COUNT };
+       P_OBS32, P_FIELD32, P_SEG32, P_GX, P_GY, P_GYAW, P_GS, P_CELLS, P_COUNT };
 #define P_HOST_POOLS P_OBS32
 struct PoolLayout {
     size_t off[P_COUNT];
@@ -289,12 +290,141 @@
     if (t == 0) { D.all_rect = s_all_rect; D.pad0 = 0; }
 }
 
+__device__ __forceinline__ double seg_dist2(double px, double py, double ax, double ay, double bx, double by) {
+    const double ex = bx - ax, ey = by - ay, l2 = ex * ex + ey * ey;
+    const double t = l2 > 0.0 ? fmin(fmax(((px - ax) * ex + (py - ay) * ey) / l2, 0.0), 1.0) : 0.0;
+    const double dx = px - (ax + t * ex), dy = py - (ay + t * ey);
+    return dx * dx + dy * dy;
+}
+__device__ __forceinline__ double box_dist2(double px, double py, double lx, double ly, double hx, double hy) {
+    const double dx = fmax(fmax(lx - px, px - hx), 0.0), dy = fmax(fmax(ly - py, py - hy), 0.0);
+    return dx * dx + dy * dy;
+}
+__device__ double square_seg_dist2(double qx, double qy, double a, double ax, double ay, double bx, double by) {
+    const double p[2] = {ax - qx, ay - qy}, d[2] = {bx - ax, by - ay};
+    double t0 = 0.0, t1 = 1.0;
+    bool meets = true;
+    for (int k = 0; k < 2; ++k) {
+        if (d[k] == 0.0) { if (fabs(p[k]) > a) meets = false; }
+        else {
+            const double ta = (-a - p[k]) / d[k], tb = (a - p[k]) / d[k];
+            t0 = fmax(t0, fmin(ta, tb)); t1 = fmin(t1, fmax(ta, tb));
+        }
+    }
+    if (meets && t0 <= t1) return 0.0;
+    double d2 = fmin(box_dist2(ax, ay, qx - a, qy - a, qx + a, qy + a), box_dist2(bx, by, qx - a, qy - a, qx + a, qy + a));
+    for (int k = 0; k < 4; ++k) d2 = fmin(d2, seg_dist2(qx + ((k & 1) ? a : -a), qy + ((k & 2) ? a : -a), ax, ay, bx, by));
+    return d2;
+}
+
+__global__ void __launch_bounds__(256) k_env_cells(EnvDesc* desc, const double* obs64, const double* field64,
+                                                   const double* seg64, uint4* cells, int n_env) {
+    const int e = blockIdx.x;
+    if (e >= n_env) return;
+    EnvDesc& D = desc[e];
+    const int nx = D.cell_nx, ny = D.cell_ny;
+    const int t = threadIdx.x, nt = blockDim.x;
+    if (nx <= 0 || ny <= 0) {
+        if (t == 0) cells[D.cell_off] = make_uint4(0u, 0u, 0u, 0u);
+        return;
+    }
+    __shared__ double s_obs[32][8], s_fld[32][2], s_seg[HL_MAX_SEGS][4];
+    __shared__ int s_ccw[32];
+    __shared__ double s_x0, s_y0;
+    const double ox = D.origin[0], oy = D.origin[1];
+    const int n_obs = D.n_obs, n_fld = D.n_field, n_seg = D.n_seg;
+    for (int i = t; i < 8 * n_obs; i += nt) s_obs[i >> 3][i & 7] = obs64[8 * (size_t)D.obs_off + i] - ((i & 1) ? oy : ox);
+    for (int i = t; i < 2 * n_fld; i += nt) s_fld[i >> 1][i & 1] = field64[2 * (size_t)D.field_off + i] - ((i & 1) ? oy : ox);
+    for (int i = t; i < 4 * n_seg; i += nt) s_seg[i >> 2][i & 3] = seg64[4 * (size_t)D.seg_off + i] - ((i & 1) ? oy : ox);
+    __syncthreads();
+    const double hx = 0.5 * (D.body_ext[1] - D.body_ext[0]), hy = 0.5 * (D.body_ext[3] - D.body_ext[2]);
+    const double rho = sqrt(hx * hx + hy * hy);
+    if (t < n_obs) {
+        int ccw = 1;
+        for (int i = 0; i < 4; ++i) {
+            const int j = (i + 1) & 3, k = (i + 2) & 3;
+            const double cr = (s_obs[t][2 * j] - s_obs[t][2 * i]) * (s_obs[t][2 * k + 1] - s_obs[t][2 * j + 1]) -
+                              (s_obs[t][2 * j + 1] - s_obs[t][2 * i + 1]) * (s_obs[t][2 * k] - s_obs[t][2 * j]);
+            if (!(cr > 0.0)) ccw = 0;
+        }
+        s_ccw[t] = ccw;
+    }
+    if (t == 0) {
+        double lx = INFINITY, ly = INFINITY;
+        for (int i = 0; i < n_fld; ++i) { lx = fmin(lx, s_fld[i][0]); ly = fmin(ly, s_fld[i][1]); }
+        const float x0 = (float)(lx - rho - (double)HL_CELL), y0 = (float)(ly - rho - (double)HL_CELL);
+        s_x0 = x0; s_y0 = y0;
+        D.cell_x0 = x0; D.cell_y0 = y0;
+        cells[D.cell_off] = make_uint4(__float_as_uint(x0), __float_as_uint(y0), (unsigned)nx, (unsigned)ny);
+    }
+    __syncthreads();
+    const double cell = (double)HL_CELL, a = 0.5 * cell, h = 0.7071067811865476 * cell;
+    const double m = 4.0 * ((double)D.eps + 6e-5);
+    const double r = rho + m, r2 = r * r, rh2 = (r + h) * (r + h);
+    const double lane_in = (double)HL_LANE_RIN - m - rho, lane_out = (double)HL_LANE_R + m + rho;
+    uint4* out = cells + (size_t)D.cell_off + 1;
+    for (int c = t; c < nx * ny; c += nt) {
+        const double qx = s_x0 + ((c % nx) + 0.5) * cell, qy = s_y0 + ((c / nx) + 0.5) * cell;
+        unsigned om = 0;
+        for (int k = 0; k < n_obs; ++k) {
+            const double* V = s_obs[k];
+            if (s_ccw[k]) {
+                const double lx = fmin(fmin(V[0], V[2]), fmin(V[4], V[6])), hx2 = fmax(fmax(V[0], V[2]), fmax(V[4], V[6]));
+                const double ly = fmin(fmin(V[1], V[3]), fmin(V[5], V[7])), hy2 = fmax(fmax(V[1], V[3]), fmax(V[5], V[7]));
+                if (box_dist2(qx, qy, lx, ly, hx2, hy2) > rh2) continue;
+                bool in = true;
+                double d2 = INFINITY;
+                for (int i = 0; i < 4; ++i) {
+                    const int j = (i + 1) & 3;
+                    const double cr = (V[2 * j] - V[2 * i]) * (qy - V[2 * i + 1]) - (V[2 * j + 1] - V[2 * i + 1]) * (qx - V[2 * i]);
+                    if (cr < 0.0) in = false;
+                    d2 = fmin(d2, square_seg_dist2(qx, qy, a, V[2 * i], V[2 * i + 1], V[2 * j], V[2 * j + 1]));
+                }
+                if (!in && d2 > r2) continue;
+            }
+            om |= 1u << k;
+        }
+        unsigned fm = 0, fc = HL_FC_CROSS;
+        {
+            double dmin2 = INFINITY;
+            bool inside = false;
+            for (int i = 0; i < n_fld; ++i) {
+                const int j = (i + 1 == n_fld) ? 0 : i + 1;
+                const double ax = s_fld[i][0], ay = s_fld[i][1], bx = s_fld[j][0], by = s_fld[j][1];
+                if ((ay > qy) != (by > qy) && qx < ax + (bx - ax) * (qy - ay) / (by - ay)) inside = !inside;
+                if (box_dist2(qx, qy, fmin(ax, bx), fmin(ay, by), fmax(ax, bx), fmax(ay, by)) > rh2) continue;
+                const double d2 = square_seg_dist2(qx, qy, a, ax, ay, bx, by);
+                dmin2 = fmin(dmin2, d2);
+                if (d2 <= r2) fm |= 1u << i;
+            }
+            if (dmin2 > m * m) fc = !inside ? HL_FC_OUTSIDE : (fm ? HL_FC_INSIDE_NEAR : HL_FC_INSIDE_CLEAR);
+            if (fc == HL_FC_OUTSIDE) fm = 0;
+            if (fc == HL_FC_CROSS) fm = n_fld >= 32 ? ~0u : (1u << n_fld) - 1u;
+        }
+        unsigned lc = HL_LC_CHECK;
+        if (n_seg > 0) {
+            bool any_in = false, all_out = true;
+            for (int i = 0; i < n_seg; ++i) {
+                const double* g = s_seg[i];
+                double far2 = 0.0;
+                for (int k = 0; k < 4; ++k)
+                    far2 = fmax(far2, seg_dist2(qx + ((k & 1) ? a : -a), qy + ((k & 2) ? a : -a), g[0], g[1], g[2], g[3]));
+                if (lane_in > 0.0 && far2 < lane_in * lane_in) any_in = true;
+                if (!(square_seg_dist2(qx, qy, a, g[0], g[1], g[2], g[3]) > lane_out * lane_out)) all_out = false;
+            }
+            lc = any_in ? HL_LC_FREE : (all_out ? HL_LC_HIT : HL_LC_CHECK);
+        }
+        out[c] = make_uint4(om, fm, fc | (lc << 2), 0u);
+    }
+}
+
 extern "C" int hl_env_upload(hl_ctx* ctx, const HlEnvHost* h, int32_t n_env, hl_env_batch** out) {
     if (!ctx || !h || !out || n_env <= 0) { hl_set_error("hl_env_upload: bad arguments"); return 1; }
     if (hl_enter(ctx, nullptr, nullptr, "hl_env_upload")) return 1;
     std::lock_guard<std::recursive_mutex> lock(*(std::recursive_mutex*)ctx->mu);
-    size_t n_obs = 0, n_field = 0, n_seg = 0, n_crit = 0, n_guide = 0, n_aux = 0;
+    size_t n_obs = 0, n_field = 0, n_seg = 0, n_crit = 0, n_guide = 0, n_aux = 0, n_cells = 0;
     std::vector<size_t> offs(6 * (size_t)n_env);
+    std::vector<int> cell_dims(3 * (size_t)n_env);
     for (int e = 0; e < n_env; ++e) {
         const HlEnvHost& E = h[e];
         size_t* o6 = &offs[6 * (size_t)e];
@@ -304,6 +434,21 @@
             hl_set_error("hl_env_upload: env %d has a negative count", e); return 1;
         }
         n_obs += E.n_obs; n_field += E.n_field; n_seg += E.n_seg; n_crit += E.n_crit; n_guide += E.n_guide; n_aux += E.n_aux;
+        int* cd = &cell_dims[3 * (size_t)e];
+        cd[0] = (int)n_cells; cd[1] = cd[2] = 0;
+        n_cells += 1;
+        if (E.n_obs <= 32 && E.n_field >= 3 && E.n_field <= 32) {
+            double lo[2] = {INFINITY, INFINITY}, hi[2] = {-INFINITY, -INFINITY};
+            for (int i = 0; i < E.n_field; ++i)
+                for (int c = 0; c < 2; ++c) { lo[c] = fmin(lo[c], E.field_xy[2 * i + c]); hi[c] = fmax(hi[c], E.field_xy[2 * i + c]); }
+            const double hx = 0.5 * (E.body_ext[1] - E.body_ext[0]), hy = 0.5 * (E.body_ext[3] - E.body_ext[2]);
+            const double span = 2.0 * (sqrt(hx * hx + hy * hy) + (double)HL_CELL);
+            const double wx = (hi[0] - lo[0] + span) / (double)HL_CELL + 2.0, wy = (hi[1] - lo[1] + span) / (double)HL_CELL + 2.0;
+            if (wx > 0.0 && wy > 0.0 && wx * wy <= (double)HL_MAX_CELLS) {
+                cd[1] = (int)wx; cd[2] = (int)wy;
+                n_cells += (size_t)cd[1] * cd[2];
+            }
+        }
     }
     size_t bytes[P_COUNT];
     bytes[P_DESC] = sizeof(EnvDesc) * (size_t)n_env;
@@ -316,6 +461,8 @@
     bytes[P_FIELD32] = sizeof(float) * HL_FIELD32_STRIDE * n_field;
     bytes[P_SEG32] = sizeof(float) * 4 * n_seg;
     bytes[P_GX] = bytes[P_GY] = bytes[P_GYAW] = bytes[P_GS] = sizeof(double) * n_guide;
+    bytes[P_CELLS] = sizeof(uint4) * n_cells;
+    if (n_cells > (size_t)INT32_MAX) { hl_set_error("hl_env_upload: %zu cells exceed the 32-bit cell offsets", n_cells); return 1; }
     PoolLayout L;
     L.total = 0;
     for (int k = 0; k < P_COUNT; ++k) {
@@ -349,6 +496,9 @@
         D.default_len = E.default_search_length;
         for (int k = 0; k < 4; ++k) D.body_ext[k] = E.body_ext[k];
         D.origin[0] = D.origin[1] = 0.0; D.reach = 0.f; D.eps = 0.f; D.all_rect = 1; D.pad0 = 0;
+        const int* cd = &cell_dims[3 * (size_t)e];
+        D.cell_off = cd[0]; D.cell_nx = cd[1]; D.cell_ny = cd[2];
+        D.cell_x0 = D.cell_y0 = 0.f; D.pad1 = 0;
         if (E.n_obs) memcpy(obs64 + 8 * c_obs, E.obs_xy, sizeof(double) * 8 * E.n_obs);
         if (E.n_field) memcpy(field64 + 2 * c_field, E.field_xy, sizeof(double) * 2 * E.n_field);
         if (E.n_seg) {
@@ -400,6 +550,7 @@
     cudaError_t ce = cudaMemcpyAsync(d, S, L.host_bytes, cudaMemcpyHostToDevice, cs);
     if (ce == cudaSuccess) {
         k_env_derive<<<n_env, 128, 0, cs>>>(A, n_env);
+        k_env_cells<<<n_env, 256, 0, cs>>>(A.desc, A.obs64, A.field64, A.seg64, (uint4*)(d + L.off[P_CELLS]), n_env);
         ce = cudaGetLastError();
     }
     if (ce == cudaSuccess) ce = cudaStreamSynchronize(cs);
@@ -414,6 +565,29 @@
     b->dev.crit64 = (const double*)(d + L.off[P_CRIT64]);
     b->dev.guide_x = A.gx; b->dev.guide_y = A.gy; b->dev.guide_yaw = A.gyaw; b->dev.guide_s = A.gs;
     b->dev.aux64 = A.aux64;
+    b->dev.cells = (const uint4*)(d + L.off[P_CELLS]);
     *out = b;
     return 0;
 }
+
+extern "C" int hl_env_cells(const hl_env_batch* envs, int32_t env, int32_t* dims, double* info, uint32_t* records,
+                            int64_t cap_records) {
+    if (!envs || !dims || !info || env < 0 || env >= envs->dev.n_env) { hl_set_error("hl_env_cells: bad arguments"); return 1; }
+    int prev = 0;
+    HL_CUDA_OK(cudaGetDevice(&prev));
+    HL_CUDA_OK(cudaSetDevice(envs->device));
+    EnvDesc D;
+    cudaError_t ce = cudaMemcpy(&D, envs->dev.desc + env, sizeof(EnvDesc), cudaMemcpyDeviceToHost);
+    const int64_t n = (int64_t)D.cell_nx * D.cell_ny;
+    if (ce == cudaSuccess) {
+        dims[0] = D.cell_nx; dims[1] = D.cell_ny;
+        info[0] = D.origin[0]; info[1] = D.origin[1]; info[2] = D.cell_x0; info[3] = D.cell_y0; info[4] = D.eps;
+        if (records && n > 0) {
+            if (cap_records < n) { cudaSetDevice(prev); hl_set_error("hl_env_cells: %lld records do not fit in %lld", (long long)n, (long long)cap_records); return 1; }
+            ce = cudaMemcpy(records, envs->dev.cells + D.cell_off + 1, sizeof(uint4) * (size_t)n, cudaMemcpyDeviceToHost);
+        }
+    }
+    cudaSetDevice(prev);
+    if (ce != cudaSuccess) { hl_set_error("hl_env_cells: %s", cudaGetErrorString(ce)); return 1; }
+    return 0;
+}
diff --git a/headland_trajectory_planning_b200/csrc/hl_geom.cuh b/headland_trajectory_planning_b200/csrc/hl_geom.cuh
--- a/headland_trajectory_planning_b200/csrc/hl_geom.cuh
+++ b/headland_trajectory_planning_b200/csrc/hl_geom.cuh
@@ -349,6 +349,17 @@
     const float* field;
     const float* seg;
 };
+
+__device__ __forceinline__ const uint4* env_table(const EnvBatchDev& eb, const EnvDesc& D) { return eb.cells + D.cell_off; }
+
+__device__ __forceinline__ uint4 cell_lookup(const uint4* cells, float Cx, float Cy) {
+    const uint4 hd = __ldg(cells);
+    const float gx = (Cx - __uint_as_float(hd.x)) * (1.0f / HL_CELL), gy = (Cy - __uint_as_float(hd.y)) * (1.0f / HL_CELL);
+    if (gx >= 0.f && gy >= 0.f && gx < (float)hd.z && gy < (float)hd.w)
+        return __ldg(cells + 1 + (int)gy * (int)hd.z + (int)gx);
+    return make_uint4(~0u, ~0u, HL_FC_CROSS | (HL_LC_CHECK << 2), 0u);
+}
+__device__ __forceinline__ unsigned low_bits(int n) { return n >= 32 ? ~0u : (1u << n) - 1u; }
 
 __device__ __forceinline__ float f_rcp(float x) { return __fdividef(1.0f, x); }
 __device__ __forceinline__ float f_sqrt(float x) { return x > 0.0f ? x * rsqrtf(x) : 0.0f; }
@@ -387,7 +398,7 @@
 };
 
 static __device__ __forceinline__ void filt_stage1(const EnvSmem& E, float px, float py, float c, float s,
-                                                   const float* ext, unsigned flags, FiltState& F) {
+                                                   const float* ext, unsigned flags, const uint4& cell, FiltState& F) {
     const float eps = E.eps;
     const float hx = 0.5f * (ext[1] - ext[0]), hy = 0.5f * (ext[3] - ext[2]);
     const float mx = 0.5f * (ext[1] + ext[0]), my = 0.5f * (ext[3] + ext[2]);
@@ -398,7 +409,9 @@
         bool a_obs = false;
         if (E.all_rect) {
             HL_LOOP
-            for (int k = 0; k < E.n_obs; ++k) {
+            for (int base = 0; base < E.n_obs; base += 32)
+            for (unsigned bits = cell.x & low_bits(E.n_obs - base); bits; bits &= bits - 1) {
+                const int k = base + __ffs(bits) - 1;
                 const float* o = E.obs + HL_OBS32_STRIDE * k;
                 const float4 b0 = *reinterpret_cast<const float4*>(o + 20);
                 const float4 b1 = *reinterpret_cast<const float4*>(o + 24);
@@ -422,7 +435,9 @@
                 ry[j] = fmaf(s, lx[j], fmaf(c, ly[j], py));
             }
             HL_LOOP
-            for (int k = 0; k < E.n_obs; ++k) {
+            for (int base = 0; base < E.n_obs; base += 32)
+            for (unsigned bits = cell.x & low_bits(E.n_obs - base); bits; bits &= bits - 1) {
+                const int k = base + __ffs(bits) - 1;
                 const float* o = E.obs + HL_OBS32_STRIDE * k;
                 float sep = -INFINITY;
 #pragma unroll
@@ -453,7 +468,9 @@
         const int n = E.n_field;
         const float rho_eps = sqrtf(fmaf(hx, hx, hy * hy)) + eps;
         HL_LOOP
-        for (int i = 0; i < n; ++i) {
+        for (int base = 0; base < n; base += 32)
+        for (unsigned bits = cell.y & low_bits(n - base); bits; bits &= bits - 1) {
+            const int i = base + __ffs(bits) - 1;
             const float* e = E.field + HL_FIELD32_STRIDE * i;
             const float4 r0 = *reinterpret_cast<const float4*>(e);
             const float4 r1 = *reinterpret_cast<const float4*>(e + 4);
@@ -468,6 +485,8 @@
                 if (!(fabsf(sd) > rn + eps)) { if (i < 32) near_mask |= 1u << i; else overflow = true; }
             }
         }
+        const unsigned fc = cell.z & 3u;
+        if (fc != HL_FC_CROSS) inside = fc != HL_FC_OUTSIDE;
     }
     F.near_mask = near_mask; F.amb = amb; F.hit = hit; F.inside = inside; F.overflow = overflow;
 }
@@ -518,12 +537,14 @@
 }
 
 static __device__ __forceinline__ int filt_lane(const EnvSmem& E, float px, float py, float c, float s,
-                                                const float* ext, bool* lane_amb) {
+                                                const float* ext, unsigned lane_cls, bool* lane_amb) {
     const float eps = E.eps;
     const float hx = 0.5f * (ext[1] - ext[0]), hy = 0.5f * (ext[3] - ext[2]);
     const float mx = 0.5f * (ext[1] + ext[0]), my = 0.5f * (ext[3] + ext[2]);
     const float Cx = fmaf(c, mx, fmaf(-s, my, px)), Cy = fmaf(s, mx, fmaf(c, my, py));
     *lane_amb = false;
+    if (lane_cls == HL_LC_FREE) return HL_FREE;
+    if (lane_cls == HL_LC_HIT) return HL_HIT;
     const float rho = sqrtf(fmaf(hx, hx, hy * hy));
     const float rin = (float)HL_LANE_RIN - eps, rout = (float)HL_LANE_R + eps;
     bool accepted = false, need_corners = false;
@@ -595,20 +616,34 @@
     return HL_FREE;
 }
 
-static __device__ HL_CODE int filter_part(const EnvSmem& E, float px, float py, float c, float s,
-                                           const float* ext, unsigned flags, unsigned* which_ambig) {
+template <bool CELLS>
+static __device__ HL_CODE int filter_part_t(const EnvSmem& E, const uint4* cells, float px, float py, float c, float s,
+                                             const float* ext, unsigned flags, unsigned* which_ambig) {
+    uint4 cell = make_uint4(~0u, ~0u, HL_FC_CROSS | (HL_LC_CHECK << 2), 0u);
+    if (CELLS) {
+        const float mx = 0.5f * (ext[1] + ext[0]), my = 0.5f * (ext[3] + ext[2]);
+        cell = cell_lookup(cells, fmaf(c, mx, fmaf(-s, my, px)), fmaf(s, mx, fmaf(c, my, py)));
+    }
     FiltState F;
-    filt_stage1(E, px, py, c, s, ext, flags, F);
+    filt_stage1(E, px, py, c, s, ext, flags, cell, F);
     if (flags & HL_CHECK_BOUNDARY) filt_field2(E, px, py, c, s, ext, F);
     if (F.hit) return HL_HIT;
     unsigned amb = F.amb;
     if ((flags & HL_CHECK_LANE) && E.n_seg > 0) {
         bool lane_amb;
-        if (filt_lane(E, px, py, c, s, ext, &lane_amb) == HL_HIT) return HL_HIT;
+        if (filt_lane(E, px, py, c, s, ext, (cell.z >> 2) & 3u, &lane_amb) == HL_HIT) return HL_HIT;
         if (lane_amb) amb |= HL_CHECK_LANE;
     }
     if (amb) { if (which_ambig) *which_ambig = amb; return HL_AMBIG; }
     return HL_FREE;
+}
+static __device__ __forceinline__ int filter_part(const EnvSmem& E, float px, float py, float c, float s,
+                                                  const float* ext, unsigned flags, unsigned* which_ambig) {
+    return filter_part_t<false>(E, nullptr, px, py, c, s, ext, flags, which_ambig);
+}
+static __device__ __forceinline__ int filter_body(const EnvSmem& E, const uint4* cells, float px, float py, float c,
+                                                  float s, unsigned flags, unsigned* which_ambig) {
+    return filter_part_t<true>(E, cells, px, py, c, s, E.ext, flags, which_ambig);
 }
 
 static __device__ bool pose_infeasible(const EnvBatchDev& eb, const EnvDesc& D, const EnvSmem& E,
@@ -620,7 +655,7 @@
     float sf, cf;
     sincosf((float)yaw, &sf, &cf);
     unsigned amb = flags;
-    int r = far ? HL_AMBIG : filter_part(E, px, py, cf, sf, E.ext, flags, &amb);
+    int r = far ? HL_AMBIG : filter_body(E, env_table(eb, D), px, py, cf, sf, flags, &amb);
     if (r == HL_HIT) return true;
     bool bad = false;
     Pose64 p;
diff --git a/headland_trajectory_planning_b200/csrc/hl_rs.cu b/headland_trajectory_planning_b200/csrc/hl_rs.cu
--- a/headland_trajectory_planning_b200/csrc/hl_rs.cu
+++ b/headland_trajectory_planning_b200/csrc/hl_rs.cu
@@ -17,7 +17,7 @@
     RsPlan plans[RS_PLANS];
 };
 
-__global__ void __launch_bounds__(RS_WARPS * 32)
+__global__ void __launch_bounds__(RS_WARPS * 32, 4)
 k_rs_all_paths(EnvBatchDev eb, int have_env, const int32_t* __restrict__ env_id,
                const double* __restrict__ sg, long long n, double maxc, double step, double max_steer,
                unsigned flags, HlRsWord* __restrict__ words, int32_t* __restrict__ count,
@@ -128,7 +128,7 @@
                             rs_sample_world32(plan, j, inv_maxc, fx, fy, fc, fs);
                             if (fabsf(fx) > E.reach || fabsf(fy) > E.reach) st = far_status(flags, E.n_seg);
                             else if (!(fx == fx) || !(fy == fy) || !(fc == fc)) { st = HL_AMBIG; amb = flags; }
-                            else st = filter_part(E, fx, fy, fc, fs, E.ext, flags, &amb);
+                            else st = filter_body(E, env_table(eb, D), fx, fy, fc, fs, flags, &amb);
                         }
                         hit = __any_sync(0xffffffffu, st == HL_HIT);
                         if (!hit && __any_sync(0xffffffffu, st == HL_AMBIG)) {
@@ -168,7 +168,7 @@
     }
 }
 
-__global__ void __launch_bounds__(RS_WARPS * 32)
+__global__ void __launch_bounds__(RS_WARPS * 32, 4)
 k_rs_sample(const double* __restrict__ start, const HlRsWord* __restrict__ words, long long m, double maxc,
             double step, const long long* __restrict__ offset, double* __restrict__ ox, double* __restrict__ oy,
             double* __restrict__ oyaw, double* __restrict__ ocs, int8_t* __restrict__ odir) {
diff --git a/headland_trajectory_planning_b200/ops.py b/headland_trajectory_planning_b200/ops.py
--- a/headland_trajectory_planning_b200/ops.py
+++ b/headland_trajectory_planning_b200/ops.py
@@ -48,6 +48,19 @@
     if count_exact:
         return out, n_exact
     return out
+
+
+def env_cells(envs, env):
+    lib = _lib.load_library()
+    dims = np.zeros(2, dtype=np.int32)
+    info = np.zeros(5, dtype=np.float64)
+    _lib.check(lib.hl_env_cells(envs.handle, int(env), dims.ctypes.data, info.ctypes.data, None, 0), "hl_env_cells")
+    nx, ny = int(dims[0]), int(dims[1])
+    rec = np.zeros((ny, nx, 4), dtype=np.uint32)
+    if nx * ny:
+        _lib.check(lib.hl_env_cells(envs.handle, int(env), dims.ctypes.data, info.ctypes.data, rec.ctypes.data,
+                                    nx * ny), "hl_env_cells")
+    return {"records": rec, "origin": info[0:2].copy(), "corner": info[2:4].copy(), "eps": float(info[4])}
 
 
 def path_reduce(envs, pose_bad, path_start):
diff --git a/include/headland_b200.h b/include/headland_b200.h
--- a/include/headland_b200.h
+++ b/include/headland_b200.h
@@ -7,7 +7,7 @@
 extern "C" {
 #endif
 
-#define HL_ABI_VERSION 4
+#define HL_ABI_VERSION 5
 
 #define HL_MAX_PRIMS        16
 #define HL_MAX_ROLLOUT      16
@@ -119,6 +119,8 @@
 void hl_env_free(hl_env_batch* envs);
 int32_t hl_env_count(const hl_env_batch* envs);
 int hl_env_device(const hl_env_batch* envs);
+int hl_env_cells(const hl_env_batch* envs, int32_t env, int32_t* dims, double* info, uint32_t* records,
+                 int64_t cap_records);
 
 int hl_collision_check(hl_ctx* ctx, const hl_env_batch* envs, const int32_t* d_env_id,
                        const double* d_poses, const int32_t* d_pose_idx, int64_t n,
```

New measurement: 222,500 (median of 6 runs). 1.09x the previous value.
